# facebookresearch/EgoT2

Measured on AMD Instinct MI355X. Metric: clips/sec fwd+bwd, 3-task TTM translator (B=256,T=15,d=128), higher is better.
Workload: dtype f32 (operands split exactly into 3 bf16 parts; 6 bf16 MFMA products per K-block, f32 accumulate); 1 GPU; configs[1]: TTM 3-task translator, 1 layer d=128 h=4 d_ff=2048, B=256/GPU T=15 S=45, synthetic N(0,1) features, random-init weights, train mode dropout=0.5 (+0.1 on PE), weighted CE (evaluated in the forward's head epilogue), fwd+bwd; global_batch=256, parallelism=dp1, impl=auto, workgroups_per_clip=1, launch=one hipGraph replay per step, deterministic=False, compute_is_module_default=True, loss=weighted CE in the forward's head epilogue (egx_ce)

## Files before the change

egot2_amd/_lib.py:

```python
from __future__ import annotations

import ctypes as C
import os

_PKG = os.path.dirname(os.path.abspath(__file__))
LIB_PATH = os.environ.get("EGX_LIB") or os.path.join(_PKG, "libegot2x.so")

EGX_ABI_VERSION = 18
EGX_MAX_SEGMENTS = 8
EGX_F32, EGX_BF16, EGX_F32_SPLIT = 0, 1, 2
EGX_IMPL_AUTO, EGX_IMPL_GENERIC, EGX_IMPL_FUSED, EGX_IMPL_WIDE, EGX_IMPL_TILED = 0, 1, 2, 3, 4

_fp = C.c_void_p


class Segment(C.Structure):
    _fields_ = [("feat", _fp), ("T", C.c_int), ("d_in", C.c_int), ("proj_w", _fp), ("proj_b", _fp),
                ("add_vec", _fp), ("pos", _fp), ("pos_stride", C.c_int), ("feat_bf16", C.c_int), ("pool", C.c_int)]


class SegmentGrads(C.Structure):
    _fields_ = [("proj_w", _fp), ("proj_b", _fp), ("add_vec", _fp), ("pos", _fp), ("feat", _fp)]


# ... 67 lines not shown
    _fields_ = [(n, _fp) for n in _DEC_LAYER_FIELDS]


class DecLayerGrads(C.Structure):
    _fields_ = [(n, _fp) for n in _DEC_LAYER_FIELDS]


SIGNATURES = {
    "egx_abi_version": (C.c_int, []),
    "egx_last_error": (C.c_char_p, []),
    "egx_launch_count": (C.c_longlong, [C.c_int]),
    "egx_tuning_reload": (None, []),
    "egx_weight_cache_bytes": (C.c_size_t, [C.POINTER(Config), C.POINTER(Segment)]),
    "egx_encoder_workspace": (C.c_int, [C.POINTER(Config), C.POINTER(Segment), C.c_int,
                                        C.POINTER(C.c_size_t), C.POINTER(C.c_size_t)]),
    "egx_encoder_uses_fused": (C.c_int, [C.POINTER(Config), C.POINTER(Segment), C.c_int]),
    "egx_encoder_token_ce_ok": (C.c_int, [C.POINTER(Config), C.POINTER(Segment), C.c_int]),
    "egx_encoder_impl": (C.c_int, [C.POINTER(Config), C.POINTER(Segment), C.c_int]),
    "egx_encoder_slices": (C.c_int, [C.POINTER(Config), C.POINTER(Segment), C.c_int]),
    "egx_wide_gemm_scratch": (C.c_size_t, [C.c_int, C.c_int, C.c_int, C.c_int]),
    "egx_wide_gemm": (C.c_int, [C.c_int, _fp, _fp, _fp, _fp, C.c_int, C.c_int, C.c_int, _fp, C.c_int, _fp, _fp, _fp]),
    "egx_wide_attention_fwd": (C.c_int, [_fp, _fp, _fp, C.c_int, C.c_int, C.c_int, C.c_int, C.c_float, C.c_uint64, _fp]),
    "egx_wide_attention_bwd": (C.c_int, [_fp, _fp, _fp, _fp, _fp, _fp, C.c_int, C.c_int, C.c_int, C.c_int, C.c_float, C.c_uint64, _fp]),
    "egx_encoder_fwd": (C.c_int, [C.POINTER(Config), C.POINTER(Segment), _fp, _fp, C.POINTER(Layer), C.c_int,
                                  _fp, _fp, _fp, C.c_int, C.c_uint64, _fp]),
    "egx_encoder_bwd": (C.c_int, [C.POINTER(Config), C.POINTER(Segment), _fp, _fp, C.POINTER(Layer), C.c_int,
                                  _fp, _fp, _fp, C.POINTER(SegmentGrads), _fp, _fp, C.POINTER(LayerGrads),
                                  C.c_int, C.c_uint64, _fp]),
    "egx_translator_workspace": (C.c_int, [C.POINTER(Config), C.POINTER(Segment), C.c_int,
                                           C.POINTER(C.c_size_t), C.POINTER(C.c_size_t)]),
    "egx_translator_fwd": (C.c_int, [C.POINTER(Config), C.POINTER(Segment), _fp, _fp, C.POINTER(Layer), C.POINTER(Head),
                                     C.c_int, _fp, _fp, _fp, _fp, C.c_int, C.c_uint64, _fp]),
    "egx_ragged_workspace": (C.c_int, [C.POINTER(Config), C.POINTER(Segment), C.c_int, _fp, C.POINTER(C.c_size_t)]),
    "egx_ragged_fwd": (C.c_int, [C.POINTER(Config), C.POINTER(Segment), _fp, _fp, _fp, C.POINTER(Layer), C.POINTER(Head), C.c_int,
                                 _fp, _fp, _fp, _fp]),
    "egx_ragged_train_workspace": (C.c_int, [C.POINTER(Config), C.POINTER(Segment), C.c_int, _fp, C.POINTER(C.c_size_t),
                                             C.POINTER(C.c_size_t)]),
    "egx_ragged_train_fwd": (C.c_int, [C.POINTER(Config), C.POINTER(Segment), _fp, _fp, _fp, C.POINTER(Layer), C.POINTER(Head), C.c_int,
                                       _fp, _fp, _fp, _fp, C.c_int, C.c_uint64, _fp]),
    "egx_ragged_bwd": (C.c_int, [C.POINTER(Config), C.POINTER(Segment), _fp, _fp, _fp, C.POINTER(Layer), C.POINTER(Head), C.c_int,
                                 _fp, _fp, _fp, _fp, C.POINTER(SegmentGrads), _fp, _fp, C.POINTER(LayerGrads), C.POINTER(HeadGrads),
                                 C.c_int, C.c_uint64, _fp]),
    "egx_ragged_encode_workspace": (C.c_int, [C.POINTER(Config), C.POINTER(Segment), C.c_int, _fp, C.POINTER(C.c_size_t)]),
    "egx_ragged_encode": (C.c_int, [C.POINTER(Config), C.POINTER(Segment), _fp, _fp, _fp, C.POINTER(Layer), C.c_int, _fp, C.c_int, _fp, _fp]),
    "egx_ragged_encode_train_workspace": (C.c_int, [C.POINTER(Config), C.POINTER(Segment), C.c_int, _fp, C.POINTER(C.c_size_t),
                                                    C.POINTER(C.c_size_t)]),
    "egx_ragged_encode_train_fwd": (C.c_int, [C.POINTER(Config), C.POINTER(Segment), _fp, _fp, _fp, C.POINTER(Layer), C.c_int, _fp, C.c_int, _fp,
                                              C.c_int, C.c_uint64, _fp]),
    "egx_ragged_encode_bwd": (C.c_int, [C.POINTER(Config), C.POINTER(Segment), _fp, _fp, C.POINTER(Layer), C.c_int, _fp, C.c_int, _fp, _fp,
                                        C.POINTER(SegmentGrads), _fp, _fp, C.POINTER(LayerGrads), C.c_int, C.c_uint64, _fp]),
    "egx_translator_bwd": (C.c_int, [C.POINTER(Config), C.POINTER(Segment), _fp, _fp, C.POINTER(Layer), C.POINTER(Head),
                                     C.c_int, _fp, _fp, _fp, C.POINTER(SegmentGrads), _fp, _fp, C.POINTER(LayerGrads),
                                     C.POINTER(HeadGrads), C.c_int, C.c_uint64, _fp]),
    "egx_small_attention_fwd": (C.c_int, [_fp, C.c_int, _fp, C.c_int, _fp, C.c_int, _fp, C.c_int, C.c_int, C.c_int, C.c_int,
                                          C.c_int, C.c_int, C.c_int, C.c_float, C.c_uint64, C.c_uint32, _fp]),
    "egx_small_attention_bwd": (C.c_int, [_fp, C.c_int, _fp, C.c_int, _fp, C.c_int, _fp, C.c_int, _fp, _fp, _fp, C.c_int,
                                          C.c_int, C.c_int, C.c_int, C.c_int, C.c_int, C.c_float, C.c_uint64, C.c_uint32, _fp]),
    "egx_target_attention_fwd": (C.c_int, [_fp, C.c_int, _fp, C.c_int, _fp, C.c_int, _fp, C.c_int, C.c_int, C.c_int, C.c_int,
                                           C.c_int, C.c_int, C.c_int, C.c_float, C.c_uint64, C.c_uint32, _fp]),
    "egx_target_attention_bwd": (C.c_int, [_fp, C.c_int, _fp, C.c_int, _fp, C.c_int, _fp, C.c_int, _fp, _fp, _fp, C.c_int,
                                           C.c_int, C.c_int, C.c_int, C.c_int, C.c_int, C.c_float, C.c_uint64, C.c_uint32, _fp]),
    "egx_embed_pos_fwd": (C.c_int, [_fp, _fp, _fp, C.c_int, C.c_float, _fp, C.c_int, C.c_int, C.c_int, C.c_int, C.c_float,
                                    C.c_uint64, _fp]),
    "egx_embed_pos_bwd": (C.c_int, [_fp, _fp, _fp, C.c_float, C.c_int, C.c_int, C.c_int, C.c_int, C.c_float, C.c_uint64, _fp]),
    "egx_decoder_workspace": (C.c_int, [C.POINTER(DecConfig), C.c_int, C.POINTER(C.c_size_t), C.POINTER(C.c_size_t)]),
    "egx_decoder_fwd": (C.c_int, [C.POINTER(DecConfig), _fp, _fp, _fp, _fp, C.c_int, C.POINTER(DecLayer), _fp, _fp, C.c_int, _fp, _fp,
                                  _fp, C.c_int, C.c_uint64, _fp]),
    "egx_decoder_ragged_workspace": (C.c_int, [C.POINTER(DecConfig), C.c_int, _fp, C.POINTER(C.c_size_t)]),
    "egx_decoder_ragged_fwd": (C.c_int, [C.POINTER(DecConfig), _fp, _fp, _fp, _fp, _fp, C.c_int, C.POINTER(DecLayer), _fp, _fp, C.c_int, _fp,
                                         _fp, _fp]),
    "egx_decoder_ragged_train_workspace": (C.c_int, [C.POINTER(DecConfig), C.c_int, _fp, C.POINTER(C.c_size_t), C.POINTER(C.c_size_t)]),
    "egx_decoder_ragged_train_fwd": (C.c_int, [C.POINTER(DecConfig), _fp, _fp, _fp, _fp, _fp, C.c_int, C.POINTER(DecLayer), _fp, _fp, C.c_int,
                                               _fp, _fp, _fp, C.c_int, C.c_uint64, _fp]),
    "egx_decoder_ragged_bwd": (C.c_int, [C.POINTER(DecConfig), _fp, _fp, C.POINTER(DecLayer), _fp, C.c_int, _fp, _fp, _fp, _fp, _fp,
                                         C.POINTER(DecLayerGrads), _fp, _fp, _fp, C.c_size_t, C.c_int, C.c_uint64, _fp]),
    "egx_decoder_generate_workspace": (C.c_int, [C.POINTER(DecConfig), C.c_int, C.c_int, C.POINTER(C.c_size_t)]),
    "egx_decoder_generate": (C.c_int, [C.POINTER(DecConfig), _fp, _fp, _fp, _fp, C.c_int, C.POINTER(DecLayer), _fp, _fp, C.c_int, C.c_int, _fp,
                                       _fp, _fp, _fp]),
    "egx_decoder_beam_workspace": (C.c_int, [C.POINTER(DecConfig), C.c_int, C.c_int, C.c_int, C.POINTER(C.c_size_t)]),
    "egx_decoder_beam": (C.c_int, [C.POINTER(DecConfig), _fp, _fp, _fp, _fp, C.c_int, C.POINTER(DecLayer), _fp, _fp, C.c_int, C.c_int, C.c_int,
                                   _fp, _fp, _fp, _fp, _fp, _fp, _fp, _fp]),
    "egx_decoder_generate_sched": (C.c_int, [C.POINTER(DecConfig), _fp, _fp, _fp, _fp, C.c_int, C.POINTER(DecLayer), _fp, _fp, C.c_int, C.c_int,
                                             _fp, _fp, _fp, _fp, C.c_int, C.POINTER(C.c_int), _fp]),
    "egx_decoder_beam_sched": (C.c_int, [C.POINTER(DecConfig), _fp, _fp, _fp, _fp, C.c_int, C.POINTER(DecLayer), _fp, _fp, C.c_int, C.c_int,
                                         C.c_int, _fp, _fp, _fp, _fp, _fp, _fp, _fp, _fp, C.c_int, C.POINTER(C.c_int), _fp]),
    "egx_cross_attention_weights": (C.c_int, [_fp, C.c_int, _fp, C.c_int, C.c_int, _fp, C.c_int, C.c_int, C.c_int, C.c_int, C.c_int, _fp, C.c_int,
                                              _fp]),
    "egx_decoder_cross_weights": (C.c_int, [C.POINTER(DecConfig), C.c_int, _fp, _fp, _fp, _fp]),
    "egx_decoder_generate_attn": (C.c_int, [C.POINTER(DecConfig), _fp, _fp, _fp, _fp, C.c_int, C.POINTER(DecLayer), _fp, _fp, C.c_int, C.c_int,
                                            _fp, _fp, _fp, _fp, C.c_int, C.POINTER(C.c_int), _fp, _fp]),
    "egx_decoder_forced_workspace": (C.c_int, [C.POINTER(DecConfig), C.c_int, C.c_int, C.c_int, C.POINTER(C.c_size_t)]),
    "egx_decoder_forced": (C.c_int, [C.POINTER(DecConfig), _fp, _fp, _fp, _fp, _fp, C.c_int, C.POINTER(DecLayer), _fp, _fp, C.c_int, C.c_int,
                                     C.c_int, _fp, _fp, _fp, _fp]),
    "egx_decoder_bwd": (C.c_int, [C.POINTER(DecConfig), _fp, C.POINTER(DecLayer), _fp, C.c_int, _fp, _fp, _fp, _fp, _fp,
                                  C.POINTER(DecLayerGrads), _fp, _fp, _fp, C.c_size_t, C.c_int, C.c_uint64, _fp]),
    "egx_comm_unique_id": (C.c_int, [_fp]),
    "egx_comm_create": (C.c_int, [_fp, C.c_int, C.c_int, C.POINTER(C.c_void_p)]),
    "egx_comm_size": (C.c_int, [_fp]),
    "egx_allreduce": (C.c_int, [_fp, _fp, C.c_size_t, C.c_int, C.c_int, _fp]),
    "egx_comm_destroy": (C.c_int, [_fp]),
    "egx_comm_library": (C.c_char_p, []),
    "egx_relu_mask": (C.c_int, [_fp, _fp, C.c_size_t, _fp]),
    "egx_dropout": (C.c_int, [_fp, C.c_int, C.c_int, C.c_float, C.c_uint64, C.c_uint32, _fp]),
    "egx_pool_pack": (C.c_int, [_fp, C.c_int, C.c_int, C.c_int, C.c_int, C.c_int, C.c_int, C.c_int, C.c_int, C.c_int, C.c_int,
                                _fp, C.c_int, C.c_longlong, _fp]),
    "egx_weighted_ce": (C.c_int, [_fp, _fp, _fp, C.c_int, C.c_int, _fp, _fp, _fp]),
# ... 104 lines not shown
```

egot2_amd/csrc/common.h:

```cpp
#pragma once
#include <hip/hip_runtime.h>
#include <stdint.h>
#include <stdio.h>
#include <string>

namespace egx {

typedef float f32x4 __attribute__((ext_vector_type(4)));
typedef short bf16x8 __attribute__((ext_vector_type(8)));

void set_error(const char* fmt, ...);
void count_launch();

#define EGX_CHECK(cond, ...)                         \
    do {                                             \
        if (!(cond)) {                               \
            ::egx::set_error(__VA_ARGS__);           \
            return 1;                                \
        }                                            \
    } while (0)

#define EGX_HIP(expr)                                                                    \
    do {                                                                                 \
        hipError_t _e = (expr);                                                          \
        if (_e != hipSuccess) {                                                          \
            ::egx::set_error("%s failed: %s (%s:%d)", #expr, hipGetErrorString(_e),      \
                             __FILE__, __LINE__);                                        \
            return 1;                                                                    \
        }                                                                                \
    } while (0)

#define EGX_LAUNCH_CHECK()                                                               \
    do {                                                                                 \
        ::egx::count_launch();                                                           \
        hipError_t _e = hipGetLastError();                                               \
        if (_e != hipSuccess) {                                                          \
            ::egx::set_error("kernel launch failed: %s (%s:%d)", hipGetErrorString(_e),  \
                             __FILE__, __LINE__);                                        \
            return 1;                                                                    \
        }                                                                                \
    } while (0)

struct Tuning {
    int ffn_cut = -1;
    bool has_slices = false; int slices_cap = 0;
    bool has_drop = false; long slice_drop = 0;
    int dec_group = -1;
    int wide_tile = 0;
    int dec_side = 1;
};
const Tuning& tuning();

static inline int cdiv(int a, int b) { return (a + b - 1) / b; }
static inline size_t align_up(size_t x, size_t a) { return (x + a - 1) / a * a; }

__device__ __forceinline__ unsigned short f2bf(float x) {
    __bf16 h = (__bf16)x;
    return __builtin_bit_cast(unsigned short, h);
}

__device__ __forceinline__ uint32_t pack_bf16x2(float a, float b) {
    typedef float f32x2_ __attribute__((ext_vector_type(2)));
    typedef __bf16 bf16x2_ __attribute__((ext_vector_type(2)));
    f32x2_ v = {a, b};
    return __builtin_bit_cast(uint32_t, __builtin_convertvector(v, bf16x2_));
}

template <typename T>
__device__ __forceinline__ T wave_sum(T v) {
#pragma unroll
    for (int o = 32; o > 0; o >>= 1) v += __shfl_xor(v, o, 64);
    return v;
}
__device__ __forceinline__ float wave_max(float v) {
#pragma unroll
    for (int o = 32; o > 0; o >>= 1) v = fmaxf(v, __shfl_xor(v, o, 64));
    return v;
}
__device__ __forceinline__ int wave_max(int v) {
#pragma unroll
    for (int o = 32; o > 0; o >>= 1) v = max(v, __shfl_xor(v, o, 64));
    return v;
}
struct WaveBest { float v; int i; };
__device__ __forceinline__ bool argmax_better(float va, int ia, float vb, int ib) {
    const bool na = va != va, nb = vb != vb;
    if (na != nb) return na;
    if (na || va == vb) return ia < ib;
    return va > vb;
}
__device__ __forceinline__ WaveBest wave_argmax(float v, int i) {
#pragma unroll
    for (int o = 32; o > 0; o >>= 1) {
        const float vo = __shfl_xor(v, o, 64);
        const int io = __shfl_xor(i, o, 64);
        if (argmax_better(vo, io, v, i)) { v = vo; i = io; }
    }
    WaveBest b;
    b.v = v; b.i = i;
    return b;
}
// ... 63 lines not shown
```

egot2_amd/csrc/encoder.hip:

```cpp
#include <stdarg.h>
#include <string.h>
#include <stdlib.h>
#include <vector>

#include "../../include/egot2x.h"
#include "common.h"
#include "kernels.h"
#include "fused.h"
#include "fused_host.h"
#include "wide.h"
#include "wide_host.h"

namespace egx {

static thread_local char g_err[1024] = "";

static long long g_launches = 0;
void count_launch() { ++g_launches; }
void set_error(const char* fmt, ...) {
    va_list ap;
    va_start(ap, fmt);
    vsnprintf(g_err, sizeof(g_err), fmt, ap);
    va_end(ap);
}
// ... 33 lines not shown
    }
    size_t d = pl.d, N = pl.N;
    size_t cur = 0;
    for (int i = 0; i < pl.nseg; ++i) {
        size_t rows = (size_t)B * segs[i].T;
        pl.seg_pre[i] = take(cur, rows * d * 4);
        pl.seg_stats[i] = take(cur, rows * 2 * 4);
    }
    for (int l = 0; l < pl.L; ++l) {
        LayerOff& o = pl.layer[l];
        o.x_in = take(cur, N * d * 4);
        o.qkv = take(cur, N * 3 * d * 4);
        o.lse = take(cur, (size_t)B * pl.H * S * 4);
        o.attn_o = take(cur, N * d * 4);
        o.res1 = take(cur, N * d * 4);
        o.stats1 = take(cur, N * 2 * 4);
        o.x1 = take(cur, N * d * 4);
        o.hid = take(cur, N * (size_t)pl.dff * 4);
        o.res2 = take(cur, N * d * 4);
        o.stats2 = take(cur, N * 2 * 4);
    }
    pl.saved_bytes = cur;

    size_t sc = 0;
    pl.s_dA = take(sc, N * d * 4);
    pl.s_dB = take(sc, N * d * 4);
    pl.s_dqkv = take(sc, N * 3 * d * 4);
    pl.s_dhid = take(sc, N * (size_t)pl.dff * 4);
    size_t slab = 0;
    auto upd = [&](int M, int Nn, int K) { slab = size_max(slab, gemm_scratch_bytes(2, M, Nn, K)); };
    upd(3 * pl.d, pl.d, (int)N);
    upd(pl.d, pl.d, (int)N);
    upd(pl.dff, pl.d, (int)N);
    upd(pl.d, pl.dff, (int)N);
    for (int i = 0; i < pl.nseg; ++i)
        if (segs[i].proj_w) upd(pl.d, segs[i].d_in, B * segs[i].T);
    pl.slab_bytes = slab;
    pl.s_slab = take(sc, slab);
    pl.det_bytes = cfg->deterministic ? generic_det_scratch_bytes(B, pl.d, pl.dff) : 0;
    pl.s_det = take(sc, pl.det_bytes);
    pl.scratch_bytes = sc;
    return 0;
}

static Tuning g_tuning;
static bool g_tuning_loaded = false;
static void tuning_load() {
    Tuning t;
    if (const char* e = getenv("EGX_FFN_CUT")) t.ffn_cut = e[0] != '0' ? 1 : 0;
    if (const char* e = getenv("EGX_FFN_SLICES")) { t.has_slices = true; t.slices_cap = atoi(e); }
    if (const char* e = getenv("EGX_SLICE_DROP")) { t.has_drop = true; t.slice_drop = strtol(e, nullptr, 16); }
    if (const char* e = getenv("EGX_DEC_GROUP")) t.dec_group = atoi(e);
    if (const char* e = getenv("EGX_WIDE_TILE")) t.wide_tile = atoi(e);
    if (const char* e = getenv("EGX_DEC_SIDE")) t.dec_side = e[0] == '0' ? 0 : e[0] == '2' ? 2 : 1;
    g_tuning = t;
    g_tuning_loaded = true;
}
const Tuning& tuning() { if (!g_tuning_loaded) tuning_load(); return g_tuning; }

static bool use_tiled(const egx_config* cfg, const egx_segment* segs, const Plan& pl, bool* err) {
    *err = false;
    const bool ok = tiled_ok(cfg, segs, pl);
    if (cfg->impl == EGX_IMPL_TILED) {
        if (!ok) { set_error("tiled implementation does not support this configuration (needs d=128, h=4, 48 < S <= %d, compute bf16 or f32s, d_ff%%128==0, projected segments, <=4 layers)", TILED_MAX_S); *err = true; }
        return ok;
    }
    return cfg->impl == EGX_IMPL_AUTO && ok;
}

static bool use_fused(const egx_config* cfg, const egx_segment* segs, const Plan& pl, bool* err) {
    *err = false;
    bool ok = fused_ok(cfg, segs, pl);
    if (cfg->impl == EGX_IMPL_FUSED) {
        if (!ok) { set_error("fused implementation does not support this configuration (needs d=128, h=4 or 8, S<=48, d_ff%%128==0, projected segments, <=%d layers)", FUSED_MAX_LAYERS); *err = true; }
        return ok;
    }
    return cfg->impl == EGX_IMPL_AUTO && ok;
}

static bool use_wide(const egx_config* cfg, const egx_segment* segs, const Plan& pl, bool* err) {
    *err = false;
    const bool ok = wide_ok(cfg, segs, pl.B);
    if (cfg->impl == EGX_IMPL_WIDE) {
        if (!ok) { set_error("wide implementation does not support this configuration (needs compute = bf16, d_model >= 256, d_model / d_ff / projected d_in multiples of 128, S <= 128 with head dim 32 / 64 / 96 / 128, S <= 480 with head dim 32 / 64 or S <= 16 with head dim 256 / 512; d_model <= 2048)"); *err = true; }
        return ok;
    }
    return cfg->impl == EGX_IMPL_AUTO && ok && !fused_ok(cfg, segs, pl);
}

static int linear_nt(const float* x, const float* W, const float* bias, float* y, int M, int N, int K, int relu,
                     const Drop& dr, const float* residual, int compute, hipStream_t st) {
    GemmParams g;
    g.A = x; g.B = W; g.C = y;
    g.M = M; g.N = N; g.K = K;
    g.lda = K; g.ldb = K; g.ldc = N;
    g.bias = bias;
    g.relu = relu;
    g.drop_key = dr.key; g.drop_thresh = dr.thresh; g.drop_inv_keep = dr.inv_keep;
    g.residual = residual; g.ldr = N;
    return gemm(0, g, compute, 0, nullptr, 0, st);
}

int linear_dx(const float* dy, const float* W, float* dx, int M, int N, int K, const float* mask, float mask_scale,
              const float* residual, int compute, hipStream_t st, void* slab, size_t slab_bytes) {
    GemmParams g;
    g.A = dy; g.B = W; g.C = dx;
// ... 197 lines not shown
        const float* pre = sg.feat;
        if (sg.proj_w) {
            float* po = fptr(saved, pl.seg_pre[i]);
            Drop df = make_drop(training, cfg->p_feat, seed, (uint32_t)i, SITE_FEAT);
            if (linear_nt(sg.feat, sg.proj_w, sg.proj_b, po, rows, d, sg.d_in, 0, df, nullptr, comp, st)) return 1;
            pre = po;
        }
        LnFwdParams lp;
        lp.x = pre; lp.w = ln_w; lp.b = ln_b; lp.eps = cfg->ln_eps;
        lp.stats = fptr(saved, pl.seg_stats[i]);
        lp.y = x0; lp.rows = rows; lp.d = d;
        lp.T = sg.T; lp.S = S; lp.off = pl.seg_off[i];
        lp.add_vec = sg.add_vec; lp.pos = sg.pos; lp.pos_stride = sg.pos_stride;
        Drop dp = make_drop(training, cfg->p_pos, seed, 0, SITE_POS);
        lp.drop_key = dp.key; lp.drop_thresh = dp.thresh; lp.drop_inv_keep = dp.inv_keep;
        if (layernorm_fwd(lp, st)) return 1;
    }

    for (int l = 0; l < pl.L; ++l) {
        const LayerOff& o = pl.layer[l];
        const egx_layer& w = layers[l];
        const float* x_in = cfptr(saved, o.x_in);
        float* x_out = (l + 1 < pl.L) ? fptr(saved, pl.layer[l + 1].x_in) : tokens_out;
        Drop none;
        if (linear_nt(x_in, w.in_proj_w, w.in_proj_b, fptr(saved, o.qkv), N, 3 * d, d, 0, none, nullptr, comp, st)) return 1;
        Drop da = make_drop(training, cfg->p_drop, seed, (uint32_t)l, SITE_ATTN);
        if (attention_fwd(cfptr(saved, o.qkv), fptr(saved, o.attn_o), fptr(saved, o.lse), B, S, pl.H, d, da.key, da.thresh,
                          da.inv_keep, st)) return 1;
        Drop d1 = make_drop(training, cfg->p_drop, seed, (uint32_t)l, SITE_RES1);
        if (linear_nt(cfptr(saved, o.attn_o), w.out_proj_w, w.out_proj_b, fptr(saved, o.res1), N, d, d, 0, d1, x_in, comp, st)) return 1;
        LnFwdParams l1;
        l1.x = cfptr(saved, o.res1); l1.w = w.norm1_w; l1.b = w.norm1_b; l1.eps = cfg->ln_eps;
        l1.stats = fptr(saved, o.stats1); l1.y = fptr(saved, o.x1); l1.rows = N; l1.d = d;
        if (layernorm_fwd(l1, st)) return 1;
        Drop dh = make_drop(training, cfg->p_drop, seed, (uint32_t)l, SITE_FFN);
        if (linear_nt(cfptr(saved, o.x1), w.lin1_w, w.lin1_b, fptr(saved, o.hid), N, pl.dff, d, 1, dh, nullptr, comp, st)) return 1;
        Drop d2 = make_drop(training, cfg->p_drop, seed, (uint32_t)l, SITE_RES2);
        if (linear_nt(cfptr(saved, o.hid), w.lin2_w, w.lin2_b, fptr(saved, o.res2), N, d, pl.dff, 0, d2, cfptr(saved, o.x1), comp, st)) return 1;
        LnFwdParams l2;
        l2.x = cfptr(saved, o.res2); l2.w = w.norm2_w; l2.b = w.norm2_b; l2.eps = cfg->ln_eps;
        l2.stats = fptr(saved, o.stats2); l2.y = x_out; l2.rows = N; l2.d = d;
        if (layernorm_fwd(l2, st)) return 1;
    }
    if (with_head) {
        if (pool_head_fwd(tokens_out, B, S, d, head->ln_w, head->ln_b, cfg->ln_eps, head->W, head->b, head->n_out,
                          head_pooled, logits_out, st)) return 1;
        if (ce) return weighted_ce(logits_out, ce->target, ce->class_weight, B, head->n_out, ce->loss, ce->d_logits, st);
    }
    return 0;
}

static int encoder_fwd_impl(const egx_config* cfg, const egx_segment* segs, const float* ln_w, const float* ln_b,
                            const egx_layer* layers, const egx_head* head, int B, float* tokens_out, float* logits_out,
                            void* saved, void* scratch, int training, uint64_t seed, void* stream) {
    (void)scratch;
    Plan pl;
    if (make_plan(cfg, segs, B, pl)) return 1;
    EGX_CHECK(saved && ln_w && ln_b, "null pointer argument");
    EGX_CHECK(pl.L == 0 || layers, "null layers");
    hipStream_t st = (hipStream_t)stream;
    const bool with_head = head && head->W;
    EGX_CHECK(with_head ? (logits_out != nullptr) : (tokens_out != nullptr), "null output pointer");
    if (check_ce(cfg->ce, with_head, " (egx_translator_fwd)")) return 1;
    EGX_CHECK(!cfg->weight_cache_valid || cfg->weight_cache, "weight_cache_valid without a weight_cache");
    const egx_token_ce* tce = cfg->token_ce;
    if (tce) {
        EGX_CHECK(!with_head && token_ce_ok(cfg, segs, pl), "egx_config.token_ce: not on this configuration (egx_encoder_token_ce_ok)");
        EGX_CHECK(tce->W && tce->target && tce->logits && tce->loss && tce->d_logits && tce->C >= 1 && tce->C <= 8,
                  "egx_config.token_ce: W, target, logits, loss, d_logits and 1 <= C <= 8 must be set");
    }
    if (check_head(head)) return 1;
    if (training && !cfg->seed_ptr && (cfg->p_drop > 0.f || cfg->p_pos > 0.f || cfg->p_feat > 0.f)) {
        hipStreamCaptureStatus cs = hipStreamCaptureStatusNone;
        if (hipStreamIsCapturing(st, &cs) != hipSuccess) (void)hipGetLastError();
        EGX_CHECK(cs == hipStreamCaptureStatusNone, "training-mode dropout (p > 0) with a host seed cannot be captured in a hipGraph: every replay would "
                  "repeat the same masks; pass egx_config.seed_ptr (model.enable_device_seed()), capture with p = 0, or launch eagerly");
    }
    bool ferr, terr = false, werr;
    const bool fused = use_fused(cfg, segs, pl, &ferr);
    const bool tiled = !fused && !ferr && use_tiled(cfg, segs, pl, &terr);
    if (fused || tiled) return fused_path_fwd(cfg, segs, pl, tiled, ln_w, ln_b, layers, head, tokens_out, logits_out, saved, training, seed, st);
    if (ferr || terr) return 1;
    EGX_CHECK(cfg->out_tokens == 0 || cfg->out_tokens == pl.S, "out_tokens is implemented by the fused per-clip kernels only (egx_encoder_impl() == EGX_IMPL_FUSED)");
    if (use_wide(cfg, segs, pl, &werr)) return wide_path_fwd(cfg, segs, pl, ln_w, ln_b, layers, head, tokens_out, logits_out, saved, training, seed, st);
    if (werr) return 1;
    return generic_fwd(cfg, segs, pl, ln_w, ln_b, layers, head, tokens_out, logits_out, saved, training, seed, st);
}

static int wide_path_bwd(const egx_config* cfg, const egx_segment* segs, const Plan& pl, const float* ln_w, const egx_layer* layers, const egx_head* head,
                         const float* d_tokens, const float* d_logits, const void* saved, void* scratch, const egx_segment_grads* seg_grads, float* d_ln_w,
                         float* d_ln_b, const egx_layer_grads* layer_grads, const egx_head_grads* head_grads, int training, uint64_t seed, hipStream_t st) {
    const int B = pl.B;
    const bool with_head = head && head->W;
    EGX_CHECK(layers && layer_grads, "null layers / layer_grads");
    if (cfg->bwd_stage == 2) return 0;
    size_t wsv = 0, wsc = 0;
    wide_workspace(cfg, segs, B, &wsv, &wsc);
    const float* dtok = d_tokens;
    bool zeroed = false;
    if (with_head) {
        const float* extra = cfptr(saved, align_up(wsv, 256));
        const float* pooled = extra + (size_t)pl.N * pl.d;
        float* dt = fptr(scratch, align_up(wsc, 256));
        if (cfg->zero_buf && cfg->zero_bytes) { EGX_HIP(hipMemsetAsync(cfg->zero_buf, 0, cfg->zero_bytes, st)); zeroed = true; }
        if (pool_head_bwd(d_logits, pooled, B, pl.S, pl.d, head->ln_w, head->ln_b, cfg->ln_eps, head->W, head->n_out, dt,
                          head_grads ? head_grads->ln_w : nullptr, head_grads ? head_grads->ln_b : nullptr,
                          head_grads ? head_grads->W : nullptr, head_grads ? head_grads->b : nullptr, st)) return 1;
        dtok = dt;
    }
    egx_config c2 = *cfg;
    if (zeroed) { c2.zero_buf = nullptr; c2.zero_bytes = 0; }
    return wide_encoder_bwd(&c2, segs, ln_w, layers, B, dtok, saved, scratch, seg_grads, d_ln_w, d_ln_b, layer_grads, training, seed, st);
}

static int generic_bwd(const egx_config* cfg, const egx_segment* segs, const Plan& pl, const float* ln_w, const egx_layer* layers, const egx_head* head,
                       float* d_tokens, const float* d_logits, const void* saved, void* scratch, const egx_segment_grads* seg_grads, float* d_ln_w,
                       float* d_ln_b, const egx_layer_grads* layer_grads, const egx_head_grads* head_grads, int training, uint64_t seed, hipStream_t st) {
    const int B = pl.B;
    const bool with_head = head && head->W;
    EGX_CHECK(pl.L == 0 || (layers && layer_grads), "null layers / layer_grads");
    if (cfg->bwd_stage == 2) return 0;
    const int d = pl.d, S = pl.S, comp = cfg->compute, dff = pl.dff;
    const int N = (int)pl.N;
    if (cfg->zero_buf && cfg->zero_bytes) EGX_HIP(hipMemsetAsync(cfg->zero_buf, 0, cfg->zero_bytes, st));
    DetScope det_scope(cfg->deterministic ? (char*)scratch + pl.s_det : nullptr, pl.det_bytes);
    if (with_head) {
        const float* tk = cfptr(saved, align_up(pl.saved_bytes, 256));
        const float* pooled = tk + (size_t)N * d;
        d_tokens = fptr(scratch, align_up(pl.scratch_bytes, 256));
        if (pool_head_bwd(d_logits, pooled, B, S, d, head->ln_w, head->ln_b, cfg->ln_eps, head->W, head->n_out, d_tokens,
                          head_grads ? head_grads->ln_w : nullptr, head_grads ? head_grads->ln_b : nullptr,
                          head_grads ? head_grads->W : nullptr, head_grads ? head_grads->b : nullptr, st)) return 1;
    }
    float* dA = fptr(scratch, pl.s_dA);
// ... 34 lines not shown
        if (d1.thresh) {
            EGX_HIP(hipMemcpyAsync(dBm, dA, (size_t)N * d * 4, hipMemcpyDeviceToDevice, st));
            if (apply_dropout_mask(dBm, N, d, d1.key, d1.thresh, d1.inv_keep, st)) return 1;
            dbr = dBm;
        }
        if (gw.out_proj_b && colsum_accum(dbr, N, d, d, gw.out_proj_b, st)) return 1;
        if (gw.out_proj_w && linear_dw(dbr, cfptr(saved, o.attn_o), gw.out_proj_w, N, d, d, comp, slab, pl.slab_bytes, st)) return 1;
        if (linear_dx(dbr, w.out_proj_w, g, N, d, d, nullptr, 1.f, nullptr, comp, st)) return 1;
        Drop da = make_drop(training, cfg->p_drop, seed, (uint32_t)l, SITE_ATTN);
        if (attention_bwd(cfptr(saved, o.qkv), cfptr(saved, o.attn_o), cfptr(saved, o.lse), g, dqkv, B, S, pl.H, d, da.key,
                          da.thresh, da.inv_keep, st)) return 1;
        if (gw.in_proj_b && colsum_accum(dqkv, N, 3 * d, 3 * d, gw.in_proj_b, st)) return 1;
        if (gw.in_proj_w && linear_dw(dqkv, cfptr(saved, o.x_in), gw.in_proj_w, N, 3 * d, d, comp, slab, pl.slab_bytes, st)) return 1;
        if (linear_dx(dqkv, w.in_proj_w, g, N, 3 * d, d, nullptr, 1.f, dA, comp, st)) return 1;
    }

    Drop dp = make_drop(training, cfg->p_pos, seed, 0, SITE_POS);
    for (int i = 0; i < pl.nseg; ++i) {
        const egx_segment& sg = segs[i];
        egx_segment_grads sgr;
        memset(&sgr, 0, sizeof(sgr));
        if (seg_grads) sgr = seg_grads[i];
        int rows = B * sg.T;
        if (sgr.pos && pos_grad_accum(g, B, S, pl.seg_off[i], sg.T, d, sgr.pos, sg.pos_stride, dp.key, dp.thresh, dp.inv_keep, st)) return 1;
        bool need_dx = (sg.proj_w && (sgr.proj_w || sgr.proj_b || sgr.feat)) || (!sg.proj_w && sgr.feat);
        bool need_any = need_dx || d_ln_w || d_ln_b || sgr.add_vec;
        if (!need_any) continue;
        float* dseg = (!sg.proj_w && sgr.feat) ? sgr.feat : dA;
        LnBwdParams bp;
        bp.dy = g;
        bp.pre = sg.proj_w ? cfptr(saved, pl.seg_pre[i]) : sg.feat;
        bp.stats = cfptr(saved, pl.seg_stats[i]);
        bp.w = ln_w; bp.dx = dseg; bp.dw = d_ln_w; bp.db = d_ln_b; bp.dadd = sgr.add_vec;
        bp.rows = rows; bp.d = d; bp.T = sg.T; bp.S = S; bp.off = pl.seg_off[i];
        bp.drop_key = dp.key; bp.drop_thresh = dp.thresh; bp.drop_inv_keep = dp.inv_keep;
        if (sg.proj_w) {
            Drop df = make_drop(training, cfg->p_feat, seed, (uint32_t)i, SITE_FEAT);
            bp.out_drop_key = df.key; bp.out_drop_thresh = df.thresh; bp.out_drop_inv_keep = df.inv_keep;
        }
        if (layernorm_bwd(bp, st)) return 1;
        if (sg.proj_w) {
            if (sgr.proj_b && colsum_accum(dseg, rows, d, d, sgr.proj_b, st)) return 1;
            if (sgr.proj_w && linear_dw(dseg, sg.feat, sgr.proj_w, rows, d, sg.d_in, comp, slab, pl.slab_bytes, st)) return 1;
            if (sgr.feat && linear_dx(dseg, sg.proj_w, sgr.feat, rows, d, sg.d_in, nullptr, 1.f, nullptr, comp, st)) return 1;
        }
    }
    return 0;
}

static int encoder_bwd_impl(const egx_config* cfg, const egx_segment* segs, const float* ln_w, const float* ln_b,
                            const egx_layer* layers, const egx_head* head, int B, float* d_tokens, const float* d_logits,
                            const void* saved, void* scratch, const egx_segment_grads* seg_grads, float* d_ln_w,
                            float* d_ln_b, const egx_layer_grads* layer_grads, const egx_head_grads* head_grads,
                            int training, uint64_t seed, void* stream) {
    (void)ln_b;
    Plan pl;
    if (make_plan(cfg, segs, B, pl)) return 1;
    const bool with_head = head && head->W;
    EGX_CHECK((with_head ? (const void*)d_logits : cfg->token_ce ? (const void*)cfg->token_ce->d_logits : (const void*)d_tokens) && saved && scratch && ln_w, "null pointer argument");
    hipStream_t st = (hipStream_t)stream;
    bool ferr, terr = false, werr;
    const bool fused = use_fused(cfg, segs, pl, &ferr);
    const bool tiled = !fused && !ferr && use_tiled(cfg, segs, pl, &terr);
    if (fused || tiled) return fused_path_bwd(cfg, segs, pl, tiled, ln_w, ln_b, layers, head, d_tokens, d_logits, saved, scratch, seg_grads, d_ln_w, d_ln_b,
                                              layer_grads, head_grads, training, seed, st);
    if (ferr || terr) return 1;
    if (use_wide(cfg, segs, pl, &werr)) return wide_path_bwd(cfg, segs, pl, ln_w, layers, head, d_tokens, d_logits, saved, scratch, seg_grads, d_ln_w, d_ln_b,
                                                             layer_grads, head_grads, training, seed, st);
    if (werr) return 1;
    return generic_bwd(cfg, segs, pl, ln_w, layers, head, d_tokens, d_logits, saved, scratch, seg_grads, d_ln_w, d_ln_b, layer_grads, head_grads, training, seed, st);
}

extern "C" {

int egx_encoder_fwd(const egx_config* cfg, const egx_segment* segs, const float* ln_w, const float* ln_b,
                    const egx_layer* layers, int B, float* tokens_out, void* saved, void* scratch, int training,
                    uint64_t seed, void* stream) {
    return encoder_fwd_impl(cfg, segs, ln_w, ln_b, layers, nullptr, B, tokens_out, nullptr, saved, scratch, training, seed, stream);
}

int egx_encoder_bwd(const egx_config* cfg, const egx_segment* segs, const float* ln_w, const float* ln_b,
                    const egx_layer* layers, int B, float* d_tokens, const void* saved, void* scratch,
                    const egx_segment_grads* seg_grads, float* d_ln_w, float* d_ln_b,
                    const egx_layer_grads* layer_grads, int training, uint64_t seed, void* stream) {
    return encoder_bwd_impl(cfg, segs, ln_w, ln_b, layers, nullptr, B, d_tokens, nullptr, saved, scratch, seg_grads, d_ln_w,
                            d_ln_b, layer_grads, nullptr, training, seed, stream);
}

int egx_translator_workspace(const egx_config* cfg, const egx_segment* segs, int B, size_t* saved_bytes, size_t* scratch_bytes) {
    Plan pl;
    if (make_plan(cfg, segs, B, pl)) return 1;
    size_t sv = 0, sc = 0;
    if (egx_encoder_workspace(cfg, segs, B, &sv, &sc)) return 1;
    size_t wsv = 0, wsc = 0;
    if (wide_ok(cfg, segs, B)) wide_workspace(cfg, segs, B, &wsv, &wsc);
    size_t extra_sv = align_up(size_max(pl.saved_bytes, wsv), 256) + (pl.N + (size_t)B) * pl.d * 4 + 256;
    size_t extra_sc = align_up(size_max(pl.scratch_bytes, wsc), 256) + pl.N * pl.d * 4 + 256;
    if (saved_bytes) *saved_bytes = size_max(sv, extra_sv);
    if (scratch_bytes) *scratch_bytes = size_max(sc, extra_sc);
    return 0;
}

int egx_translator_fwd(const egx_config* cfg, const egx_segment* segs, const float* ln_w, const float* ln_b,
                       const egx_layer* layers, const egx_head* head, int B, float* logits_out, float* tokens_out,
                       void* saved, void* scratch, int training, uint64_t seed, void* stream) {
    EGX_CHECK(head && head->W, "egx_translator_fwd needs a head (use egx_encoder_fwd otherwise)");
    return encoder_fwd_impl(cfg, segs, ln_w, ln_b, layers, head, B, tokens_out, logits_out, saved, scratch, training, seed, stream);
}

int egx_translator_bwd(const egx_config* cfg, const egx_segment* segs, const float* ln_w, const float* ln_b,
                       const egx_layer* layers, const egx_head* head, int B, const float* d_logits, const void* saved,
                       void* scratch, const egx_segment_grads* seg_grads, float* d_ln_w, float* d_ln_b,
                       const egx_layer_grads* layer_grads, const egx_head_grads* head_grads, int training,
                       uint64_t seed, void* stream) {
    EGX_CHECK(head && head->W, "egx_translator_bwd needs a head (use egx_encoder_bwd otherwise)");
    return encoder_bwd_impl(cfg, segs, ln_w, ln_b, layers, head, B, nullptr, d_logits, saved, scratch, seg_grads, d_ln_w,
                            d_ln_b, layer_grads, head_grads, training, seed, stream);
}

int egx_pool_head_fwd(const float* tokens, int B, int S, int d, const float* ln_w, const float* ln_b, float ln_eps,
                      const float* W, const float* b, int n_out, float* pooled_saved, float* out, void* stream) {
    EGX_CHECK(tokens && pooled_saved && out, "null pointer argument");
    return pool_head_fwd(tokens, B, S, d, ln_w, ln_b, ln_eps, W, b, n_out, pooled_saved, out, (hipStream_t)stream);
}

int egx_pool_head_bwd(const float* d_out, const float* pooled_saved, int B, int S, int d, const float* ln_w,
                      const float* ln_b, float ln_eps, const float* W, int n_out, float* d_tokens, float* d_ln_w,
                      float* d_ln_b, float* d_W, float* d_b, void* stream) {
    EGX_CHECK(d_out && pooled_saved && d_tokens, "null pointer argument");
    return pool_head_bwd(d_out, pooled_saved, B, S, d, ln_w, ln_b, ln_eps, W, n_out, d_tokens, d_ln_w, d_ln_b, d_W, d_b,
                         (hipStream_t)stream);
}

int egx_linear_fwd(const float* x, const float* W, const float* b, float* y, int M, int N, int K, int relu, int compute,
                   void* stream) {
    EGX_CHECK(x && W && y, "null pointer argument");
    Drop none;
    return linear_nt(x, W, b, y, M, N, K, relu, none, nullptr, compute, (hipStream_t)stream);
}
int egx_linear_residual_fwd(const float* x, const float* W, const float* b, const float* residual, float* y, int M, int N, int K,
                            int compute, void* stream) {
    EGX_CHECK(x && W && y && residual, "null pointer argument");
    Drop none;
    return linear_nt(x, W, b, y, M, N, K, 0, none, residual, compute, (hipStream_t)stream);
}
int egx_gelu_fwd(const float* z, float* h, size_t n, void* stream) { return gelu_fwd(z, h, n, (hipStream_t)stream); }
int egx_gelu_bwd(const float* z, const float* dh, float* dz, size_t n, void* stream) { return gelu_bwd(z, dh, dz, n, (hipStream_t)stream); }

size_t egx_colsum_ordered_scratch(int M, int N) { return colsum_part_bytes(M, N); }
int egx_colsum_ordered(const float* dy, int M, int N, float* db, void* scratch, size_t scratch_bytes, void* stream) {
    EGX_CHECK(dy && db, "egx_colsum_ordered: null pointer argument");
    EGX_CHECK(scratch_bytes >= colsum_part_bytes(M, N) && (scratch || !colsum_part_bytes(M, N)),
              "egx_colsum_ordered: scratch of %zu bytes, egx_colsum_ordered_scratch(%d, %d) = %zu", scratch_bytes, M, N, colsum_part_bytes(M, N));
    return colsum_accum_ordered(dy, M, N, N, db, scratch, scratch_bytes, (hipStream_t)stream);
}

size_t egx_linear_bwd_scratch(int M, int N, int K) { return size_max(gemm_scratch_bytes(2, N, K, M), gemm_scratch_bytes(1, M, K, N)); }

int egx_linear_bwd(const float* dy, const float* x, const float* W, float* dx, float* dW, float* db, int M, int N, int K,
                   int compute, void* scratch, void* stream) {
    hipStream_t st = (hipStream_t)stream;
    EGX_CHECK(dy, "null dy");
    if (db && colsum_accum(dy, M, N, N, db, st)) return 1;
    if (dW) {
        EGX_CHECK(x && scratch, "linear_bwd: dW needs x and scratch");
        if (linear_dw(dy, x, dW, M, N, K, compute, scratch, gemm_scratch_bytes(2, N, K, M), st)) return 1;
    }
    if (dx) {
        EGX_CHECK(W, "linear_bwd: dx needs W");
        if (linear_dx(dy, W, dx, M, N, K, nullptr, 1.f, nullptr, compute, st, scratch, scratch ? egx_linear_bwd_scratch(M, N, K) : 0)) return 1;
    }
    return 0;
// ... 191 lines not shown
```

egot2_amd/csrc/ffn_cut.hip:

```cpp
#include <stdlib.h>
#include "common.h"
#include "kernels.h"
#include "fused.h"
#include "fused_dev.h"

namespace egx {

__device__ unsigned long long g_cstamps[32];
#ifdef EGX_STAMPS
#define CSTAMP_INIT() unsigned long long ct_prev = __builtin_amdgcn_s_memtime(), ct_acc[8] = {0, 0, 0, 0, 0, 0, 0, 0}
#define CSTAMP(k) do { __builtin_amdgcn_sched_barrier(0); unsigned long long t_ = __builtin_amdgcn_s_memtime(); ct_acc[k] += t_ - ct_prev; ct_prev = t_; __builtin_amdgcn_sched_barrier(0); } while (0)
#define CSTAMP_FLUSH(base) do { if (blockIdx.x == 0 && (threadIdx.x == 0 || threadIdx.x == 256)) for (int k_ = 0; k_ < 8; ++k_) g_cstamps[(base) + (threadIdx.x >> 8) * 8 + k_] = ct_acc[k_]; } while (0)
#define ASTAMP(i) do { if (blockIdx.x == 0 && threadIdx.x == 0) g_cstamps[i] = __builtin_amdgcn_s_memtime(); } while (0)
#else
#define ASTAMP(i) do { } while (0)
#define CSTAMP_INIT() do { } while (0)
#define CSTAMP(k) do { } while (0)
#define CSTAMP_FLUSH(base) do { } while (0)
#endif
int debug_read_cstamps(unsigned long long* out) {
    return hipMemcpyFromSymbol(out, HIP_SYMBOL(g_cstamps), sizeof(unsigned long long) * 32) == hipSuccess ? 0 : 1;
}
#ifdef EGX_DIAG_NOLOAD
#define RING_REFILL(slot, k, hb, hbn) do { } while (0)
#else
#define RING_REFILL(slot, k, hb, hbn) ring[slot] = frag_load(((k) + D) & 15, (k) + D < 16 ? (hb) : (hbn))
#endif

namespace {
constexpr int CT = 512;
constexpr int CNT = 3;
constexpr int CSP = CNT * 16;
constexpr int CBLK = CSP * LDX;
constexpr int CPS = CSP * LDXH;

template <int CM> struct RingDepth { static constexpr int v = 4; };
template <> struct RingDepth<CM_BF16> { static constexpr int v = 16; };

template <int CM>
__device__ __forceinline__ Frag<CM> operand_frag(const unsigned short* planes, const float* xf, int row, int k0, int q) {
    if constexpr (CM == CM_SPLIT) {
        return load_split_frag(planes, CPS, row, k0, q);
    } else if constexpr (CM == CM_BF16) {
        const unsigned short* b = planes + row * LDXH + k0 + 4 * q;
        const uint2 lo = *reinterpret_cast<const uint2*>(b), hi = *reinterpret_cast<const uint2*>(b + 16);
        Frag<CM_BF16> f;
        f.v = __builtin_bit_cast(bf16x8, (u32x4){lo.x, lo.y, hi.x, hi.y});
        return f;
    } else {
        return load_frag<CM>(xf + row * LDX + k0, q);
    }
}

// ... 38 lines not shown
        *reinterpret_cast<uint2*>(plane + row * LDXH + c) = make_uint2(pack_bf16x2(v[0], v[1]), pack_bf16x2(v[2], v[3]));
    }
}
__device__ __forceinline__ void block_to_split_planes(unsigned short* planes, const float* blk) {
    const int row = threadIdx.x >> 2, c0 = (threadIdx.x & 3) * 32;
    if (row < CSP) {
        float g[32];
        uint32_t h[16], m[16], lo[16];
        load32(blk + row * LDX + c0, g);
        split32(g, h, m, lo);
        store_parts32(planes + row * LDXH + c0, (size_t)CPS, h, m, lo);
    }
}

template <int CM, bool FWD>
__device__ __forceinline__ void cut_walk(int wave, int nit, int& j_begin, int& n_mine, int shift_code = 0) {
    const int shift = shift_code ? shift_code - 1 : (CM == CM_BF16 ? 0 : (FWD ? nit / 4 : nit / 8));
    const int n_old = nit + shift;
    j_begin = wave < 4 ? 0 : n_old;
    n_mine = wave < 4 ? n_old : 2 * nit - n_old;
}
constexpr int CP_FLOATS = 1024 + 8 * FD;
constexpr int CP_HEAD_ROWS = 8;
__device__ __forceinline__ int cut_rot(int rot_mode, int clip, int nit) {
    return rot_mode == 0 ? (int)((clip * 11u + (clip >> 3) * 5u) % (unsigned)nit)
         : rot_mode == 4 ? (int)(((unsigned)(clip >> 3) & 3u) % (unsigned)nit)
         : rot_mode == 5 ? (int)(((unsigned)(clip >> 3) & 7u) % (unsigned)nit) : 0;
}

__device__ __forceinline__ void reduce_partials8(f32x4 (&y)[8][CNT], float* blk0, int wave, int r, int q) {
    if (wave >= 4) {
        float* mine = blk0 + (wave - 4) * CBLK;
#pragma unroll
        for (int i = 0; i < 8; ++i)
#pragma unroll
            for (int t = 0; t < CNT; ++t)
                *reinterpret_cast<f32x4*>(mine + (t * 16 + r) * LDX + i * 16 + 4 * q) = y[i][t];
    }
    __syncthreads();
    if (wave < 4) {
        float* mine = blk0 + wave * CBLK;
#pragma unroll
        for (int i = 0; i < 8; ++i)
#pragma unroll
            for (int t = 0; t < CNT; ++t) {
                f32x4* a = reinterpret_cast<f32x4*>(mine + (t * 16 + r) * LDX + i * 16 + 4 * q);
                *a = y[i][t] + *a;
            }
    }
    __syncthreads();
}
}

template <int CM>
__global__ __launch_bounds__(CT) void ffn_fwd_kernel(FusedFwdParams p, int l) {
    extern __shared__ __attribute__((aligned(16))) float lds[];
    float* X1 = lds;
    float* R = lds + CBLK;
    unsigned short* XP = reinterpret_cast<unsigned short*>(R);
    constexpr int NPL = CM == CM_SPLIT ? 3 : 1;
    constexpr int D = RingDepth<CM>::v;
    const int tid = threadIdx.x, wave = tid >> 6, lane = tid & 63, r = lane & 15, q = lane >> 4;
    const int clip = blockIdx.x, S = p.S;
    const size_t tokbase = (size_t)clip * S;
    const FusedLayer& w = p.layer[l];
    const bool dev_seed = p.seed_ptr != nullptr;
    const uint64_t seed_dev = dev_seed ? *p.seed_ptr : 0ull;
    const uint64_t k_ffn = dev_seed ? site_key(seed_dev, l, SITE_FFN) : w.ffn_key;
    const uint64_t k_res2 = dev_seed ? site_key(seed_dev, l, SITE_RES2) : w.res2_key;

    ASTAMP(16);
    Touched tch = {{0, 0, 0, 0}};
    if (p.touch.n) tch = touch_lines<CT>(p.touch, blockIdx.x, gridDim.x, tid);
    const int nhb = p.d_ff / 32;
    int j_begin_, n_mine_;
    cut_walk<CM, true>(wave, nhb / 8, j_begin_, n_mine_, p.rot_mode >> 8);
    const int nit = __builtin_amdgcn_readfirstlane(n_mine_), j_begin = __builtin_amdgcn_readfirstlane(j_begin_);
    const int pair_s = __builtin_amdgcn_readfirstlane(wave & 3);
    const int rot = cut_rot(p.rot_mode & 255, clip, nit);
    auto hb_of = [&](int it) { int j = it + rot; if (j >= nit) j -= nit; return pair_s + 4 * (j_begin + j); };
    float* CP = lds + 5 * CBLK;
    const bool cp_hd = p.head.n_out > 0 && l + 1 == p.n_layers;
    const int cp_g = tid >> 5, cp_c4 = (tid & 31) << 2;
    f32x4 cp_v, cp_w;
    float cp_b;
    {
        const float* src = cp_g == 0 ? w.norm2_w : cp_g == 1 ? w.norm2_b : (cp_g == 3 && cp_hd) ? p.head.ln_w : (cp_g == 4 && cp_hd) ? p.head.ln_b : w.lin2_b;
        cp_v = *reinterpret_cast<const f32x4*>(src + cp_c4);
        const int nb = cp_hd ? p.head.n_out : 0, nw = cp_hd && p.head.n_out <= CP_HEAD_ROWS ? p.head.n_out * 32 : 0;
        cp_b = nb ? p.head.b[min(max(tid - 160, 0), nb - 1)] : 0.f;
        cp_w = *reinterpret_cast<const f32x4*>(nw ? p.head.W + (size_t)min(max(tid - 256, 0), nw - 1) * 4 : w.lin2_b);
    }
    auto cp_store = [&] {
        if (cp_g < 3 || (cp_g < 5 && cp_hd)) *reinterpret_cast<f32x4*>(CP + cp_g * FD + cp_c4) = cp_v;
        if (cp_hd) {
            if (tid >= 160 && tid < 160 + p.head.n_out) CP[5 * FD + (tid - 160)] = cp_b;
            if (p.head.n_out <= CP_HEAD_ROWS && tid >= 256 && tid < 256 + p.head.n_out * 32) *reinterpret_cast<f32x4*>(CP + 1024 + (tid - 256) * 4) = cp_w;
        }
    };
    auto frag_load = [&](int k, int hb) -> WRaw<CM> {
        return k < 8 ? load_w<CM>(w.lin1_wp, hb * 2 + (k & 1), FD / 32, k >> 1, lane) : load_w<CM>(w.lin2_wp, k - 8, nhb, hb, lane);
    };
    WRaw<CM> ring[D];
    float4 b1r[2];
    {
        const int hb0 = hb_of(0);
#pragma unroll
        for (int k = 0; k < D; ++k) ring[k] = frag_load(k, hb0);
// ... 130 lines not shown
                    for (int e = 0; e < 4; ++e) hacc[i][t][e] += bv[i][e];
        }
        uint32_t dead = 0;
#pragma unroll
        for (int k = 2 * CNT * 4 - 1; k >= 0; --k) {
            const int i = k / (CNT * 4), t = (k / 4) % CNT, e = k & 3;
            dead = __builtin_amdgcn_alignbit(dead, __float_as_uint(hacc[i][t][e]), 31);
        }
        p.relu_bits[bits_base + (size_t)hb * 64] = ~dead & ((1u << (2 * CNT * 4)) - 1u);
#pragma unroll
        for (int i = 0; i < 2; ++i)
#pragma unroll
            for (int t = 0; t < CNT; ++t)
#pragma unroll
                for (int e = 0; e < 4; ++e) hacc[i][t][e] = __int_as_float(max(__float_as_int(hacc[i][t][e]), 0));
        Frag<CM> hbq[CNT];
#pragma unroll
        for (int t = 0; t < CNT; ++t) hbq[t] = chain_frag<CM>(hacc[0][t], hacc[1][t]);
#ifndef EGX_DIAG_NOSTORE
        {
            char* hb_base = hid_base + (size_t)hb * 2 * (HTILE_ELEMS * ESZ);
#pragma unroll
            for (int t = 0; t < CNT; ++t) {
                if constexpr (CM == CM_BF16) {
                    const u32x4 u = __builtin_bit_cast(u32x4, hbq[t].v);
                    store_hid_tile_bf16(hb_base + (size_t)t * nht * (HTILE_ELEMS * ESZ), u, lane, S - t * 16);
                } else {
#pragma unroll
                    for (int i = 0; i < 2; ++i)
                        store_hid_tile<CM>(hb_base + ((size_t)t * nht + i) * (HTILE_ELEMS * ESZ), hacc[i][t], lane, S - t * 16);
                }
            }
        }
#endif
        __builtin_amdgcn_sched_barrier(0);
        CSTAMP(3);
#pragma unroll
        for (int k = 8; k < 16; ++k) {
            pin(ring[k % D]);
            if (k == 8) { CSTAMP(4); }
            Frag<CM> a = w_frag<CM>(ring[k % D]);
#pragma unroll
            for (int t = 0; t < CNT; ++t) mma<CM>(y[k - 8][t], a, hbq[t]);
            __builtin_amdgcn_sched_barrier(0);
            RING_REFILL(k % D, k, hb, hbn);
            __builtin_amdgcn_sched_barrier(0);
        }
    }
    CSTAMP(5);
    CSTAMP_FLUSH(0);
    ASTAMP(18);
    __syncthreads();
    ASTAMP(19);
    reduce_partials8(y, R, wave, r, q);
    ASTAMP(20);

    for (int i = tid; i < S * (FD / 4); i += CT) {
        const int row = i >> 5, c = (i & 31) << 2, o = row * LDX + c;
        const f32x4 a0 = *reinterpret_cast<const f32x4*>(R + o), a1 = *reinterpret_cast<const f32x4*>(R + CBLK + o);
        const f32x4 a2 = *reinterpret_cast<const f32x4*>(R + 2 * CBLK + o), a3 = *reinterpret_cast<const f32x4*>(R + 3 * CBLK + o);
        f32x4 f = ((a0 + a1) + (a2 + a3)) + *reinterpret_cast<const f32x4*>(CP + 2 * FD + c);
        if (w.res_thresh) {
            float m4[4];
            drop_scale4(k_res2, (uint32_t)(tokbase + row), (uint32_t)c, w.res_thresh, w.drop_inv, m4);
            f = f * f32x4{m4[0], m4[1], m4[2], m4[3]};
        }
        *reinterpret_cast<f32x4*>(X1 + o) = f + *reinterpret_cast<const f32x4*>(X1 + o);
    }
    __syncthreads();
    ASTAMP(21);
    const bool last = l + 1 == p.n_layers;
    float* Y = R;
    ln_rows(X1, S, CP, CP + FD, p.eps, [&](int row, int c0, float (&x)[32], float (&yv)[32]) {
        if (last && p.tokens_out && row < p.out_T) store32(p.tokens_out + ((size_t)clip * p.out_T + row) * FD + c0, yv);
        store32(Y + row * LDX + c0, yv);
    }, [&] { rows_from_lds(p.saved_res + ((size_t)(2 * l + 1) * p.B + clip) * S * FD, X1, S); });
    __syncthreads();
    ASTAMP(22);
    if (!last) {
        rows_from_lds(p.xin_out + ((size_t)(l + 1) * p.B + clip) * S * FD, Y, S);
        return;
    }
    if (p.head.n_out > 0) {
        float* pooled = X1;
        const FusedCe ce{p.ce_target, p.ce_weight, p.ce_loss, p.ce_dlogits, p.ce_B, nullptr};
        CeReq rq;
        if (ce.target) { ce_request_labels<CT>(ce, tid, rq); ce_request_weights(ce, p.head.n_out, rq); }
        if (tid < FD) pooled[tid] = colsum_lds(Y, 0, S, tid) * (1.f / (float)S);
        if (ce.target) ce_weight_partials<CT>(ce, p.head.n_out, tid, rq, pooled + 256);
        __syncthreads();
        if (wave == 0) {
            float2 x = *reinterpret_cast<float2*>(pooled + 2 * lane);
            float mean = wave_sum(x.x + x.y) * (1.f / FD);
            float dx = x.x - mean, dy = x.y - mean;
            float rstd = rsqrtf(wave_sum(dx * dx + dy * dy) * (1.f / FD) + p.eps);
            float2 lw = *reinterpret_cast<const float2*>(CP + 3 * FD + 2 * lane);
            float2 lb = *reinterpret_cast<const float2*>(CP + 4 * FD + 2 * lane);
            float y0 = dx * rstd * lw.x + lb.x, y1 = dy * rstd * lw.y + lb.y;
            const bool w_lds = p.head.n_out <= CP_HEAD_ROWS;
            float zmine = 0.f;
            for (int o = 0; o < p.head.n_out; ++o) {
                float2 wv = w_lds ? *reinterpret_cast<const float2*>(CP + 1024 + o * FD + 2 * lane) : *reinterpret_cast<const float2*>(p.head.W + (size_t)o * FD + 2 * lane);
                float sdot = wave_sum(y0 * wv.x + y1 * wv.y) + CP[5 * FD + o];
                if (lane == 0) p.logits_out[(size_t)clip * p.head.n_out + o] = sdot;
                zmine = lane == o ? sdot : zmine;
            }
            if (ce.target) ce_clip<CT>(ce, p.head.n_out, clip, lane, zmine, pooled + 256, true);
        }
    }
    ASTAMP(23);
}

template <int CM>
__global__ __launch_bounds__(CT) void ffn_bwd_kernel(FusedBwdParams p, int l) {
    extern __shared__ __attribute__((aligned(16))) float lds[];
    float* B1 = lds;
    float* Gs = lds + 1 * CBLK;
    float* B2 = lds + 2 * CBLK;
    float* B3 = lds + 3 * CBLK;
    float* B4 = lds + 4 * CBLK;
    unsigned short* GP = reinterpret_cast<unsigned short*>(B3);
    constexpr int D = RingDepth<CM>::v;
    const int tid = threadIdx.x, wave = tid >> 6, lane = tid & 63, r = lane & 15, q = lane >> 4;
    const int clip = blockIdx.x, S = p.S;
    const size_t tok0 = (size_t)clip * S;
    const FusedBwdLayer& w = p.layer[l];
    const bool dev_seed = p.seed_ptr != nullptr;
    const uint64_t seed_dev = dev_seed ? *p.seed_ptr : 0ull;
    const uint64_t k_res2 = dev_seed ? site_key(seed_dev, l, SITE_RES2) : w.res2_key;
    const bool last = l + 1 == p.n_layers;

    ASTAMP(24);
    Touched tch = {{0, 0, 0, 0}};
    if (p.touch.n) tch = touch_lines<CT>(p.touch, blockIdx.x, gridDim.x, tid);
    if (p.zero_buf) {
        const size_t n4 = p.zero_n / 4, per = (n4 + gridDim.x - 1) / gridDim.x;
        const size_t b0 = (size_t)blockIdx.x * per, b1 = b0 + per < n4 ? b0 + per : n4;
        for (size_t k = b0 + threadIdx.x; k < b1; k += CT) reinterpret_cast<float4*>(p.zero_buf)[k] = make_float4(0, 0, 0, 0);
    }
    float* part = p.partials + (size_t)clip * p.P;
    float* pl = part + l * FUSED_P_LAYER;

    const int nhb = p.d_ff / 32;
    int j_begin_, n_mine_;
    cut_walk<CM, false>(wave, nhb / 8, j_begin_, n_mine_, p.rot_mode >> 8);
    const int nit = __builtin_amdgcn_readfirstlane(n_mine_), j_begin = __builtin_amdgcn_readfirstlane(j_begin_);
    const int pair_s = __builtin_amdgcn_readfirstlane(wave & 3);
    const int rot = cut_rot(p.rot_mode & 255, clip, nit);
    auto hb_of = [&](int it) { int j = it + rot; if (j >= nit) j -= nit; return pair_s + 4 * (j_begin + j); };
    float* CP = lds + 5 * CBLK;
    const bool cp_hd = p.head.n_out > 0 && last;
    const int cp_g = tid >> 5, cp_c4 = (tid & 31) << 2;
    f32x4 cp_v, cp_w;
    float cp_b;
    {
        const float* src = cp_g == 1 ? w.norm2_b : (cp_g == 3 && cp_hd) ? p.head.ln_w : (cp_g == 4 && cp_hd) ? p.head.ln_b : w.norm2_w;
        cp_v = *reinterpret_cast<const f32x4*>(src + cp_c4);
        const int nb = cp_hd ? p.head.n_out : 0, nw = cp_hd && p.head.n_out <= CP_HEAD_ROWS ? p.head.n_out * 32 : 0;
        cp_b = nb ? p.d_logits[(size_t)clip * p.head.n_out + min(max(tid - 160, 0), nb - 1)] : 0.f;
        if (nb && p.d_logits_scale) cp_b *= *p.d_logits_scale;
        cp_w = *reinterpret_cast<const f32x4*>(nw ? p.head.W + (size_t)min(max(tid - 256, 0), nw - 1) * 4 : w.norm2_w);
    }
    auto cp_store = [&] {
        if (cp_g < 2 || ((cp_g == 3 || cp_g == 4) && cp_hd)) *reinterpret_cast<f32x4*>(CP + cp_g * FD + cp_c4) = cp_v;
        if (cp_hd) {
            if (tid >= 160 && tid < 160 + p.head.n_out) CP[5 * FD + 64 + (tid - 160)] = cp_b;
            if (p.head.n_out <= CP_HEAD_ROWS && tid >= 256 && tid < 256 + p.head.n_out * 32) *reinterpret_cast<f32x4*>(CP + 1024 + (tid - 256) * 4) = cp_w;
        }
    };
    auto frag_load = [&](int k, int hb) -> WRaw<CM> {
        return k < 8 ? load_w<CM>(w.lin2_wtp, hb * 2 + (k & 1), FD / 32, k >> 1, lane) : load_w<CM>(w.lin1_wtp, k - 8, nhb, hb, lane);
    };
    const uint32_t* relu_bits = p.relu_bits + ((size_t)l * p.B + clip) * (size_t)nhb * 64 + lane;
    WRaw<CM> ring[D];
    uint32_t relu_word;
    {
        const int hb0 = hb_of(0);
#pragma unroll
        for (int k = 0; k < D; ++k) ring[k] = frag_load(k, hb0);
        relu_word = relu_bits[(size_t)hb0 * 64];
    }
    const float* res2 = p.saved_res + ((size_t)(2 * l + 1) * p.B + clip) * S * FD;
    const bool head_bwd = last && p.head.n_out > 0;
    {
        constexpr int XR = CSP * (FD / 4) / CT;
        f32x4 rr[XR], dr[XR];
        const f32x4* rs = reinterpret_cast<const f32x4*>(res2);
        const int ndy_rows = head_bwd ? 0 : (last ? p.out_T : S);
        const f32x4* ds = head_bwd ? rs : reinterpret_cast<const f32x4*>(last ? p.d_tokens + (size_t)clip * p.out_T * FD : p.dxin + tok0 * FD);
        const int nx = S * (FD / 4), nd = ndy_rows * (FD / 4);
#pragma unroll
        for (int k = 0; k < XR; ++k) {
            const int i = tid + CT * k;
            rr[k] = rs[i < nx ? i : nx - 1];
            dr[k] = ds[i < nd ? i : (nd > 0 ? nd - 1 : 0)];
        }
        for (int i = tid; i < 5 * CBLK / 4; i += CT) reinterpret_cast<f32x4*>(lds)[i] = f32x4{0, 0, 0, 0};
        cp_store();
        __syncthreads();
#pragma unroll
        for (int k = 0; k < XR; ++k) {
            const int i = tid + CT * k, row = i >> 5, c = (i & 31) << 2;
            if (i < nx) {
                *reinterpret_cast<f32x4*>(B1 + row * LDX + c) = rr[k];
                if (head_bwd) *reinterpret_cast<f32x4*>(Gs + row * LDX + c) = rr[k];
            }
            if (i < nd) *reinterpret_cast<f32x4*>(Gs + row * LDX + c) = dr[k];
        }
        touch_sink(tch);
    }
    ASTAMP(25);
    if (head_bwd) {
        float* hp = part + p.head_off;
        __syncthreads();
        ln_rows(Gs, S, CP, CP + FD, p.eps, [&](int row, int c0, float (&x)[32], float (&y)[32]) { store32(Gs + row * LDX + c0, y); });
        __syncthreads();
        float* pooled = B2;
        if (tid < FD) pooled[tid] = colsum_lds(Gs, 0, S, tid) * (1.f / (float)S);
        __syncthreads();
        if (wave == 0) {
            float2 x = *reinterpret_cast<float2*>(pooled + 2 * lane);
            float mean = wave_sum(x.x + x.y) * (1.f / FD);
            float xh0 = x.x - mean, xh1 = x.y - mean;
            float rstd = rsqrtf(wave_sum(xh0 * xh0 + xh1 * xh1) * (1.f / FD) + p.eps);
            xh0 *= rstd; xh1 *= rstd;
            float2 lw = *reinterpret_cast<const float2*>(CP + 3 * FD + 2 * lane);
            float2 lb = *reinterpret_cast<const float2*>(CP + 4 * FD + 2 * lane);
            float y0 = xh0 * lw.x + lb.x, y1 = xh1 * lw.y + lb.y;
            float d0 = 0.f, d1 = 0.f;
            const bool w_lds = p.head.n_out <= CP_HEAD_ROWS;
            for (int o = 0; o < p.head.n_out; ++o) {
                float go = CP[5 * FD + 64 + o];
                float2 wv = w_lds ? *reinterpret_cast<const float2*>(CP + 1024 + o * FD + 2 * lane) : *reinterpret_cast<const float2*>(p.head.W + (size_t)o * FD + 2 * lane);
                d0 += go * wv.x; d1 += go * wv.y;
                *reinterpret_cast<float2*>(hp + 256 + FUSED_HEAD_MAX_OUT + o * FD + 2 * lane) = make_float2(go * y0, go * y1);
                if (lane == 0) hp[256 + o] = go;
            }
            *reinterpret_cast<float2*>(hp + 2 * lane) = make_float2(d0 * xh0, d1 * xh1);
            *reinterpret_cast<float2*>(hp + 128 + 2 * lane) = make_float2(d0, d1);
            float g0 = d0 * lw.x, g1 = d1 * lw.y;
            float s1 = wave_sum(g0 + g1) * (1.f / FD);
            float s2 = wave_sum(g0 * xh0 + g1 * xh1) * (1.f / FD);
            float inv_s = 1.f / (float)S;
            *reinterpret_cast<float2*>(pooled + 128 + 2 * lane) =
                make_float2(rstd * (g0 - s1 - xh0 * s2) * inv_s, rstd * (g1 - s1 - xh1 * s2) * inv_s);
        }
        __syncthreads();
        f32x4 dp[1];
        {
            const int c = (tid & 31) << 2;
            dp[0] = *reinterpret_cast<const f32x4*>(pooled + 128 + c);
        }
        __syncthreads();
        for (int i = tid; i < S * (FD / 4); i += CT) {
            const int row = i >> 5, c = (i & 31) << 2;
            *reinterpret_cast<f32x4*>(Gs + row * LDX + c) = dp[0];
        }
        if (tid < 64) *reinterpret_cast<f32x4*>(B2 + 4 * tid) = f32x4{0, 0, 0, 0};
    }
    __syncthreads();
    ASTAMP(26);
    ln_bwd_rows(S, CP, p.eps,
        [&](int row, int c0, float (&dy)[32], float (&x)[32]) { load32(Gs + row * LDX + c0, dy); load32(B1 + row * LDX + c0, x); },
        [&](int row, int c0, float (&dy)[32], float (&dx)[32], float (&dyx)[32]) {
            store32(B1 + row * LDX + c0, dx);
            store32(B3 + row * LDX + c0, dyx);
            if (w.res_thresh) {
                const uint32_t orow = (uint32_t)(tok0 + row);
#pragma unroll
                for (int j = 0; j < 32; ++j) dx[j] *= drop_scale(k_res2, orow, (uint32_t)(c0 + j), w.res_thresh, w.drop_inv);
            }
            store32(B2 + row * LDX + c0, dx);
        });
    __syncthreads();
    if (tid < 128) pl[0 + tid] = colsum_lds(B3, 0, S, tid);
    else if (tid < 256) pl[128 + (tid - 128)] = colsum_lds(Gs, 0, S, tid - 128);
    else if (tid < 384) pl[256 + (tid - 256)] = colsum_lds(B2, 0, S, tid - 256);
    if (!(CM != CM_F32 && p.xg_planes)) rows_from_lds(w.g2_out + tok0 * FD, B2, S);
    __syncthreads();
    if constexpr (CM == CM_SPLIT) block_to_split_planes(GP, B2);
    else if constexpr (CM == CM_BF16) block_to_plane(GP, B2);
    __syncthreads();
    if (CM != CM_F32 && p.xg_planes) {
        if constexpr (CM == CM_SPLIT) {
            const size_t plane = (size_t)p.B * CSP * FD;
            planes_from_lds<3>(reinterpret_cast<unsigned short*>(w.g2_out) + (size_t)clip * CSP * FD, plane, GP);
        } else {
            planes_from_lds<1>(reinterpret_cast<unsigned short*>(w.g2_out) + (size_t)clip * CSP * FD, 0, GP);
        }
    }

    ASTAMP(27);
    f32x4 dxa[8][CNT];
#pragma unroll
    for (int i = 0; i < 8; ++i)
#pragma unroll
        for (int t = 0; t < CNT; ++t) dxa[i][t] = f32x4{0, 0, 0, 0};
    constexpr int ESZ = CM == CM_BF16 ? 2 : 4;
    const int nht = p.d_ff / 16;
    char* const dhid_base = (char*)p.dhid_out + ((size_t)l * p.B + clip) * CNT * nht * (size_t)(HTILE_ELEMS * ESZ);
    for (int it = 0; it < nit; ++it) {
        const int hb = hb_of(it);
        const int hbn = hb_of(it + 1 < nit ? it + 1 : it);
        __builtin_amdgcn_sched_barrier(0);
        f32x4 dacc[2][CNT];
#pragma unroll
        for (int i = 0; i < 2; ++i)
#pragma unroll
            for (int t = 0; t < CNT; ++t) dacc[i][t] = f32x4{0, 0, 0, 0};
        Frag<CM> gb[CNT];
#pragma unroll
        for (int k = 0; k < 8; ++k) {
// ... 19 lines not shown
#pragma unroll
            for (int t = 0; t < CNT; ++t)
#pragma unroll
                for (int e = 0; e < 4; ++e) {
                    const int k = (i * CNT + t) * 4 + e;
                    const int32_t m = ((int32_t)(bits << (31 - k))) >> 31;
                    dacc[i][t][e] = __uint_as_float(__float_as_uint(dacc[i][t][e]) & (uint32_t)m);
                }
        Frag<CM> dq_[CNT];
#pragma unroll
        for (int t = 0; t < CNT; ++t) dq_[t] = chain_frag<CM>(dacc[0][t], dacc[1][t]);
        {
            char* hb_base = dhid_base + (size_t)hb * 2 * (HTILE_ELEMS * ESZ);
#pragma unroll
            for (int t = 0; t < CNT; ++t) {
                if constexpr (CM == CM_BF16) {
                    const u32x4 u = __builtin_bit_cast(u32x4, dq_[t].v);
                    store_hid_tile_bf16(hb_base + (size_t)t * nht * (HTILE_ELEMS * ESZ), u, lane, S - t * 16);
                } else {
#pragma unroll
                    for (int i = 0; i < 2; ++i)
                        store_hid_tile<CM>(hb_base + ((size_t)t * nht + i) * (HTILE_ELEMS * ESZ), dacc[i][t], lane, S - t * 16);
                }
            }
        }
        __builtin_amdgcn_sched_barrier(0);
#pragma unroll
        for (int k = 8; k < 16; ++k) {
            pin(ring[k % D]);
            Frag<CM> a = w_frag<CM>(ring[k % D]);
#pragma unroll
            for (int t = 0; t < CNT; ++t) mma<CM>(dxa[k - 8][t], a, dq_[t]);
            __builtin_amdgcn_sched_barrier(0);
            RING_REFILL(k % D, k, hb, hbn);
            __builtin_amdgcn_sched_barrier(0);
        }
    }
    ASTAMP(28);
    __syncthreads();
    ASTAMP(29);
    reduce_partials8(dxa, Gs, wave, r, q);
    ASTAMP(30);
    {
        f32x4* dst = reinterpret_cast<f32x4*>(p.dy1 + tok0 * FD);
        for (int i = tid; i < S * (FD / 4); i += CT) {
            const int o = (i >> 5) * LDX + ((i & 31) << 2);
            const f32x4 a0 = *reinterpret_cast<const f32x4*>(Gs + o), a1 = *reinterpret_cast<const f32x4*>(B2 + o);
            const f32x4 a2 = *reinterpret_cast<const f32x4*>(B3 + o), a3 = *reinterpret_cast<const f32x4*>(B4 + o);
            dst[i] = (((a0 + a1) + a2) + a3) + *reinterpret_cast<const f32x4*>(B1 + o);
        }
    }
    ASTAMP(31);
}

bool ffn_cut_supported(int d_ff) { return d_ff % 256 == 0 && d_ff >= 256; }
size_t ffn_cut_lds_bytes() { return (size_t)(5 * CBLK + CP_FLOATS) * sizeof(float); }

template <int CM>
static int launch_cut_fwd(const FusedFwdParams& p, int l, hipStream_t st) {
    const size_t lds = ffn_cut_lds_bytes();
    static bool attr_set = false;
    if (!attr_set) {
        EGX_HIP(hipFuncSetAttribute(reinterpret_cast<const void*>(&ffn_fwd_kernel<CM>), hipFuncAttributeMaxDynamicSharedMemorySize, (int)lds));
        attr_set = true;
    }
    timing_begin(TIMER_FFN_FWD, st);
    hipLaunchKernelGGL((ffn_fwd_kernel<CM>), dim3(p.B), dim3(CT), lds, st, p, l);
    timing_end(TIMER_FFN_FWD, st);
    EGX_LAUNCH_CHECK();
    return 0;
}
template <int CM>
static int launch_cut_bwd(const FusedBwdParams& p, int l, hipStream_t st) {
    const size_t lds = ffn_cut_lds_bytes();
    static bool attr_set = false;
    if (!attr_set) {
        EGX_HIP(hipFuncSetAttribute(reinterpret_cast<const void*>(&ffn_bwd_kernel<CM>), hipFuncAttributeMaxDynamicSharedMemorySize, (int)lds));
        attr_set = true;
    }
    timing_begin(TIMER_FFN_BWD, st);
    hipLaunchKernelGGL((ffn_bwd_kernel<CM>), dim3(p.B), dim3(CT), lds, st, p, l);
    timing_end(TIMER_FFN_BWD, st);
    EGX_LAUNCH_CHECK();
    return 0;
}

int ffn_cut_forward(const FusedFwdParams& p, int l, int compute, hipStream_t st) {
    EGX_CHECK(ffn_cut_supported(p.d_ff) && p.S <= CSP && l >= 0 && l < p.n_layers, "ffn_cut_forward: d_ff=%d S=%d layer %d", p.d_ff, p.S, l);
    EGX_CHECK(p.x1f_out && p.xin_out && p.saved_res && p.relu_bits && p.hid_out, "ffn_cut_forward: missing buffers");
    return compute == CM_BF16 ? launch_cut_fwd<CM_BF16>(p, l, st) : compute == CM_SPLIT ? launch_cut_fwd<CM_SPLIT>(p, l, st) : launch_cut_fwd<CM_F32>(p, l, st);
}
int ffn_cut_backward(const FusedBwdParams& p, int l, int compute, hipStream_t st) {
    EGX_CHECK(ffn_cut_supported(p.d_ff) && p.S <= CSP && l >= 0 && l < p.n_layers, "ffn_cut_backward: d_ff=%d S=%d layer %d", p.d_ff, p.S, l);
    EGX_CHECK(p.dy1 && p.saved_res && p.relu_bits && p.dhid_out && p.partials && (l + 1 == p.n_layers || p.dxin), "ffn_cut_backward: missing buffers");
    return compute == CM_BF16 ? launch_cut_bwd<CM_BF16>(p, l, st) : compute == CM_SPLIT ? launch_cut_bwd<CM_SPLIT>(p, l, st) : launch_cut_bwd<CM_F32>(p, l, st);
}

}
```

egot2_amd/csrc/fused.h:

```cpp
#pragma once
#include "common.h"

namespace egx {

constexpr int FUSED_MAX_SEG = 4;
constexpr int FUSED_MAX_LAYERS = 6;

constexpr int TOUCH_MAX = 4;
struct TouchList { const void* base[TOUCH_MAX]; unsigned lines[TOUCH_MAX]; int n; };
static inline void touch_add(TouchList& t, const void* base, size_t bytes) {
    if (base && bytes >= 128 && t.n < TOUCH_MAX) { t.base[t.n] = base; t.lines[t.n] = (unsigned)(bytes >> 7); ++t.n; }
}

struct FusedSeg {
    const float* feat;
    const void* proj_wp;
    const float* proj_b;
    const float* add_vec;
    const float* pos;
    int T, d_in, off, pos_stride;
    int row0, Tfull;
    int seg_id, pad_;
};

// ... 114 lines not shown
    const float* norm1_w; const float* norm1_b; const float* norm2_w; const float* norm2_b;
    uint64_t attn_key, res1_key, ffn_key, res2_key;
    uint32_t attn_thresh, res_thresh, ffn_thresh;
    float drop_inv;
    float* x1_out; float* g2_out; float* attn_o_out; float* g1_out; float* x_in_out; float* dqkv_out;
};

constexpr int FUSED_P_LAYER = 1152;
static inline int fused_partial_len(int L, int nseg) { return L * FUSED_P_LAYER + 256 + nseg * 256; }

struct FusedBwdParams {
    FusedSeg seg[FUSED_MAX_SEG];
    float* dseg_out[FUSED_MAX_SEG];
    FusedBwdLayer layer[FUSED_MAX_LAYERS];
    const float* ln_w; const float* ln_b;
    float eps;
    int nseg, n_layers, B, S, d_ff;
    int rot_mode;
    const float* d_tokens;
    int out_T;
    FusedHead head; const float* d_logits; int head_off;
    const float* pooled;
    const float* saved_pre;
    const float* saved_res;
    const float* saved_qkv;
    const uint32_t* relu_bits;
    int xg_planes;
    void* dhid_out;
    float* zero_buf; size_t zero_n;
    float* partials; int P;
    uint64_t pos_key; uint32_t pos_thresh; float pos_inv;
    const uint64_t* seed_ptr;
    uint64_t feat_key[FUSED_MAX_SEG]; uint32_t feat_thresh; float feat_inv;
    int n_heads;
    float* dx0_out;
    int tpc, S_clip; size_t Ntok;
    int tiled, l_front, l_back;
    float* datt;
    float* dres;
    int n_slices; float* xchg; unsigned* xflags; int slice_drop;
    int cut, cut_layer;
    float* dy1;
    float* dxin;
    const float* d_logits_scale;
    const float* tce_W; const float* tce_dlogits; int tce_C;
    TouchList touch;
    const int* rtab; int B_clips; const int* rseg;
};
int fused_backward(const FusedBwdParams& p, int compute, hipStream_t st);
bool ffn_cut_supported(int d_ff);
size_t ffn_cut_lds_bytes();
int ffn_cut_forward(const FusedFwdParams& p, int l, int compute, hipStream_t st);
int ffn_cut_backward(const FusedBwdParams& p, int l, int compute, hipStream_t st);

struct SmallDwProblem {
    const float* G; const float* X; float* out;
    int R, C, K, ldg, ldx, first_block, splits;
};
constexpr int SMALL_DW_MAX = 8;
struct SmallDwParams {
    SmallDwProblem pr[SMALL_DW_MAX];
    int n, per;
    float* slabs;
};
int small_dw(SmallDwParams& p, int compute, hipStream_t st, void* slabs = nullptr, size_t slab_bytes = 0, bool reduce_here = true);
int seed_advance(uint64_t* seed, hipStream_t st);

struct PartialDst { float* dst; int off, len; };
constexpr int PARTIAL_MAX_DST = 64;
struct ReducePartialsParams {
    PartialDst d[PARTIAL_MAX_DST];
    int n, B, P;
    const float* partials;
};
int reduce_partials(const ReducePartialsParams& rp, hipStream_t st, bool deterministic = false);
struct SmallDwTail { SlabReduce red; ReducePartialsParams rp; unsigned slab_blocks; int rp_units, chunks; uint64_t* seed_advance;  TouchList touch;  };
int tail_reduce(const SmallDwParams* sp, const SlabReduce* red, const ReducePartialsParams* rp, uint64_t* seed_advance_ptr, const TouchList* touch, hipStream_t st);

enum { TIMER_FUSED_FWD = 0, TIMER_FUSED_BWD = 1, TIMER_FFN_DW = 2, TIMER_FFN_FWD = 3, TIMER_FFN_BWD = 4, TIMER_WIDE_GEMM = 5,
       TIMER_WIDE_ATTN_FWD = 6, TIMER_WIDE_ATTN_BWD = 7, TIMER_COUNT = 8 };
void timing_enable(int on);
void timing_begin(int which, hipStream_t st);
void timing_end(int which, hipStream_t st);
int timing_read(int which, double* total_ms, int* count);

struct TiledAttnParams {
    const float* qkv;
    float* attn_o;
    float* lse;
    const float* d_o;
    float* delta;
    float* dqkv;
    int B, S, tpc;
    uint64_t drop_key; uint32_t drop_thresh; float drop_inv;
    const uint64_t* seed_ptr; int layer;
    const int* rtab;
};
constexpr int TILED_MAX_S = 512;
constexpr int RAGGED_REC = 16;
enum { RG_TILE0 = 0, RG_S = 1, RG_TOK0 = 2, RG_OUT0 = 3, RG_OUTN = 4, RG_T = 5 , RG_OFF = 9  };
static_assert(RG_OFF + FUSED_MAX_SEG <= RAGGED_REC, "ragged clip record");
int upload_words(int* dst, const int* src, size_t n, hipStream_t st);
int ragged_rows(float* padded, float* packed, const int* rtab, const int* rseg, int B, int T_pad, int C, int k, int to_packed, hipStream_t st);
int tiled_attn_fwd(const TiledAttnParams& p, int compute, hipStream_t st);
int tiled_attn_bwd(const TiledAttnParams& p, int compute, hipStream_t st);

bool fused_supported(int d_model, int n_heads, int d_ff, int S, int nseg, const int* d_in, const int* T, const bool* has_proj);
size_t fused_lds_bytes(int NT);
long long slices_stolen_fwd(int reset);
long long slices_stolen_bwd(int reset);
int debug_read_stamps(unsigned long long* out, int n);
int debug_read_bstamps(unsigned long long* out, int n);
int fused_forward(const FusedFwdParams& p, int compute, hipStream_t st);

}
```

egot2_amd/csrc/fused.hip:

```cpp
#include "common.h"
#include "kernels.h"
#include "fused.h"
#include "fused_dev.h"
#include <stdlib.h>
#include <string.h>
#include <type_traits>
#include <vector>

namespace egx {

__global__ __launch_bounds__(64) void pack_weights_kernel(PackParams pp) {
    int blk = blockIdx.x;
    if (pp.seed_advance && blk == 0 && threadIdx.x == 0)
        *pp.seed_advance = *pp.seed_advance * 6364136223846793005ull + 1442695040888963407ull;
    if (pp.zero_words)
        for (int i = blk * 64 + threadIdx.x; i < pp.n_zero; i += gridDim.x * 64) pp.zero_words[i] = 0u;
    if (pp.zero_word2 && blk == 0 && threadIdx.x == 0) *pp.zero_word2 = 0.f;
    if (pp.zero_ctl && blk == 0 && threadIdx.x < 8) pp.zero_ctl[threadIdx.x] = 0u;
    if (pp.n == 0) return;
    int di = 0;
    while (di + 1 < pp.n && blk >= pp.d[di + 1].first_block) ++di;
    const PackDesc& d = pp.d[di];
    int local = blk - d.first_block;
    int nkb = d.K / 32;
// ... 1021 lines not shown
            float* tacc = reinterpret_cast<float*>(p.tce_ticket + 1);
            atomicAdd(tacc, l);
            __threadfence();
            const unsigned mine = 1u + ((unsigned)cn << 12);
            const unsigned old = atomicAdd(p.tce_ticket, mine);
            if ((old & 4095u) == (unsigned)p.B - 1u) {
                __threadfence();
                *p.tce_loss = atomicExch(tacc, 0.f);
                if (p.tce_correct) *p.tce_correct = (float)((old + mine) >> 12);
                atomicExch(p.tce_ticket, 0u);
            }
        }
        STAMP(14);
    }

    if (!TILED && p.head.n_out > 0) {
        float* pooled = X1;
        const FusedCe ce{p.ce_target, p.ce_weight, p.ce_loss, p.ce_dlogits, p.ce_B, p.ce_ticket};
        CeReq rq;
        if (ce.target) { ce_request_labels<256>(ce, tid, rq); ce_request_weights(ce, p.head.n_out, rq); }
        if (tid < FD) pooled[tid] = colsum_lds(Xs, 0, S, tid) * (1.f / (float)S);
        if (ce.target) ce_weight_partials<256>(ce, p.head.n_out, tid, rq, pooled + 256);
        __syncthreads();
        if (wave == 0) {
            float2 x = *reinterpret_cast<float2*>(pooled + 2 * lane);
            float mean = wave_sum(x.x + x.y) * (1.f / FD);
            float dx = x.x - mean, dy = x.y - mean;
            float rstd = rsqrtf(wave_sum(dx * dx + dy * dy) * (1.f / FD) + p.eps);
            float2 lw = *reinterpret_cast<const float2*>(p.head.ln_w + 2 * lane);
            float2 lb = *reinterpret_cast<const float2*>(p.head.ln_b + 2 * lane);
            float y0 = dx * rstd * lw.x + lb.x, y1 = dy * rstd * lw.y + lb.y;
            float zmine = 0.f;
            for (int o = 0; o < p.head.n_out; ++o) {
                float2 wv = *reinterpret_cast<const float2*>(p.head.W + (size_t)o * FD + 2 * lane);
                float sdot = wave_sum(y0 * wv.x + y1 * wv.y) + p.head.b[o];
                if (lane == 0) p.logits_out[(size_t)clip * p.head.n_out + o] = sdot;
                zmine = lane == o ? sdot : zmine;
            }
            if (ce.target) ce_clip<256>(ce, p.head.n_out, clip, lane, zmine, pooled + 256, slice == 0);
        }
    }
}

namespace {
struct TimerSlot { std::vector<hipEvent_t> a, b; int n = 0; };
TimerSlot g_timers[TIMER_COUNT];
int g_timing_on = 0;
constexpr int TIMER_MAX_EVENTS = 4096;
}
void timing_enable(int on) {
    g_timing_on = on;
    for (int i = 0; i < TIMER_COUNT; ++i) g_timers[i].n = 0;
}
void timing_begin(int which, hipStream_t st) {
    if (!g_timing_on) return;
    TimerSlot& t = g_timers[which];
    if (t.n >= TIMER_MAX_EVENTS) return;
    if ((int)t.a.size() <= t.n) {
        hipEvent_t ea, eb;
        (void)hipEventCreate(&ea); (void)hipEventCreate(&eb);
        t.a.push_back(ea); t.b.push_back(eb);
    }
    (void)hipEventRecord(t.a[t.n], st);
}
void timing_end(int which, hipStream_t st) {
    if (!g_timing_on) return;
    TimerSlot& t = g_timers[which];
    if (t.n < (int)t.a.size() && t.n < TIMER_MAX_EVENTS) { (void)hipEventRecord(t.b[t.n], st); ++t.n; }
}
int timing_read(int which, double* total_ms, int* count) {
    if (which < 0 || which >= TIMER_COUNT) return 1;
    TimerSlot& t = g_timers[which];
    double tot = 0;
    for (int i = 0; i < t.n; ++i) {
        float ms = 0.f;
        if (hipEventSynchronize(t.b[i]) != hipSuccess || hipEventElapsedTime(&ms, t.a[i], t.b[i]) != hipSuccess) return 1;
        tot += ms;
    }
    if (total_ms) *total_ms = tot;
    if (count) *count = t.n;
    return 0;
}

size_t fused_lds_bytes(int NT) {
    int SP = NT * 16;
    return (size_t)(4 * SP * LDX + FD * LDV) * sizeof(float) + FUSED_MAX_SEG * sizeof(FusedSeg) + 16 + 21 * FD * sizeof(float);
}

bool fused_supported(int d_model, int n_heads, int d_ff, int S, int nseg, const int* d_in, const int* T, const bool* has_proj) {
    if (d_model != FD || (n_heads != FH && n_heads != 2 * FH)) return false;
    if (d_ff % 128 != 0 || d_ff < 128) return false;
    if (S < 1 || S > 48) return false;
    for (int i = 0; i < nseg; ++i) {
        if (!has_proj[i]) return false;
        if (d_in[i] % 128 != 0) return false;
        if (T[i] < 1) return false;
    }
    return true;
}

template <int CM, bool TILED, int DH>
static int launch_fwd(const FusedFwdParams& p, hipStream_t st) {
    EGX_CHECK(p.S <= 48, "fused: S=%d unsupported", p.S);
    const size_t lds = fused_lds_bytes(3);
    static bool attr_set = false;
    if (!attr_set) {
// ... 80 lines not shown
```

egot2_amd/csrc/fused_bwd.hip:

```cpp
#include <stdlib.h>
#include <string.h>
#include <type_traits>
#include "common.h"
#include "kernels.h"
#include "fused.h"
#ifdef EGX_STAMPS
namespace egx { extern __device__ unsigned long long g_bstamps[32]; }
#define LNB_STAMP(base, k) do { if ((base) >= 0 && blockIdx.x == 0 && threadIdx.x == 0) { __builtin_amdgcn_sched_barrier(0); egx::g_bstamps[(base) + (k)] = __builtin_amdgcn_s_memtime(); __builtin_amdgcn_sched_barrier(0); } } while (0)
#endif
#include "fused_dev.h"

namespace egx {

template <int CM, int HT>
__global__ __launch_bounds__(256, HT == 1 ? 2 : 1) void ffn_dw_kernel(FfnDwParams p) {
    extern __shared__ __attribute__((aligned(16))) float lds[];
    constexpr int TILE = 32 * LDX;
    const int tid = threadIdx.x, lane = tid & 63, wave = tid >> 6;
    const int r = lane & 15, q = lane >> 4;
    const int hg = blockIdx.x, split = blockIdx.y;
    const int htile0 = (hg * 4 + wave) * HT;
    const int nkb_total = (p.N + 31) / 32;
    const int kb_beg = split * p.kb_per_split;
    const int kb_end = min(nkb_total, kb_beg + p.kb_per_split);
// ... 1110 lines not shown
}
__device__ unsigned long long g_bstamps[32];
#ifdef EGX_STAMPS
#define BSTAMP(i) do { if (blockIdx.x == 0 && threadIdx.x == 0) g_bstamps[i] = __builtin_amdgcn_s_memtime(); } while (0)
#else
#define BSTAMP(i) do { } while (0)
#endif
int debug_read_bstamps(unsigned long long* out, int n) {
    return hipMemcpyFromSymbol(out, HIP_SYMBOL(g_bstamps), sizeof(unsigned long long) * (n > 32 ? 32 : n)) == hipSuccess ? 0 : 1;
}

template <int CM, bool TILED, int DH, bool SLICED = false, bool CUT = false, bool RAGGED = false>
__global__ __launch_bounds__(256, 1) void fused_bwd_kernel(FusedBwdParams p) {
    static_assert(!(TILED && SLICED), "the tiled launches are not sliced");
    static_assert(!RAGGED || TILED, "ragged batches run the tiled launches");
    static_assert(!(CUT && (TILED || SLICED)), "the cut launches are neither tiled nor sliced");
    constexpr int HPW = FDH / DH, NHEAD = FH * HPW, NCT = DH / 16;
    constexpr int NT = 3;
    constexpr int SP = NT * 16;
    constexpr int BLK = SP * LDX;
    extern __shared__ __attribute__((aligned(16))) float lds[];
    float* Gs = lds;
    float* B1 = lds + 1 * BLK;
    float* B2 = lds + 2 * BLK;
    float* B3 = lds + 3 * BLK;
    float* B4 = lds + 4 * BLK;
    float* B5 = lds + 5 * BLK;
    float* stat = lds + 6 * BLK;
    float* PSB = stat + NHEAD * 3 * SP;

    const int tid = threadIdx.x, wave = tid >> 6;
    int lane = tid & 63, r = lane & 15, q = lane >> 4;
    int clip_ = blockIdx.x, slice_ = 0;
    if constexpr (SLICED) slice_map(p.n_slices, clip_, slice_);
    const int clip = clip_, slice = slice_;
    const int n_slices = SLICED ? p.n_slices : 1;
    int S, c_real, t0;
    size_t tok0;
    const int* rrec = nullptr;
    if constexpr (RAGGED) {
        c_real = p.rtab[(size_t)p.B_clips * RAGGED_REC + clip];
        rrec = p.rtab + (size_t)c_real * RAGGED_REC;
        t0 = (clip - rrec[RG_TILE0]) * 48;
        S = min(48, rrec[RG_S] - t0);
        tok0 = (size_t)rrec[RG_TOK0] + t0;
    } else if constexpr (TILED) {
        c_real = clip / p.tpc;
        t0 = (clip - c_real * p.tpc) * 48;
        S = min(48, p.S_clip - t0);
        tok0 = (size_t)c_real * p.S_clip + t0;
    } else {
        c_real = clip; t0 = 0; S = p.S; tok0 = (size_t)clip * S;
    }
    if (!CUT && p.zero_buf) {
        const size_t n4 = p.zero_n / 4, per = (n4 + gridDim.x - 1) / gridDim.x;
        const size_t b0 = (size_t)blockIdx.x * per, b1 = b0 + per < n4 ? b0 + per : n4;
        for (size_t k = b0 + threadIdx.x; k < b1; k += 256) reinterpret_cast<float4*>(p.zero_buf)[k] = make_float4(0, 0, 0, 0);
    }
    if constexpr (SLICED) { if (clip >= p.B || ((p.slice_drop >> slice) & 1)) return; }

    BSTAMP(12);
    float* part = p.partials + (size_t)clip * p.P;
#define EGX_PHASE()                                              \
    do {                                                         \
        int t_ = threadIdx.x;                                    \
        asm volatile("" : "+v"(t_));                             \
        lane = t_ & 63; r = lane & 15; q = lane >> 4;            \
    } while (0)

    const bool dev_seed = p.seed_ptr != nullptr;
    const uint64_t seed_dev = dev_seed ? *p.seed_ptr : 0ull;
    const uint64_t pos_key = dev_seed ? site_key(seed_dev, 0, SITE_POS) : p.pos_key;
    constexpr int BPF = SP * (FD / 4) / 256;
    static_assert(SP * (FD / 4) % 256 == 0, "a block must divide among the threads");
    auto blk_request = [&](f32x4 (&v)[BPF], const float* src) {
        int t_ = threadIdx.x;
        asm volatile("" : "+v"(t_));
        const f32x4* s4 = reinterpret_cast<const f32x4*>(src);
        const int n = S * (FD / 4);
#pragma unroll
        for (int k = 0; k < BPF; ++k) { const int i = t_ + 256 * k; v[k] = s4[i < n ? i : n - 1]; }
    };
    auto blk_store = [&](const f32x4 (&v)[BPF], float* dst, float* dst2) {
        int t_ = threadIdx.x;
        asm volatile("" : "+v"(t_));
#pragma unroll
        for (int k = 0; k < BPF; ++k) {
            const int i = t_ + 256 * k, row = i >> 5, c = (i & 31) << 2;
            if (i < S * (FD / 4)) {
                *reinterpret_cast<f32x4*>(dst + row * LDX + c) = v[k];
                if (dst2) *reinterpret_cast<f32x4*>(dst2 + row * LDX + c) = v[k];
            }
        }
    };
    f32x4 pf_a[BPF], pf_b[BPF];
    auto res_ptr = [&](int slot) -> const float* {
        return TILED ? p.saved_res + ((size_t)slot * p.Ntok + tok0) * FD : p.saved_res + ((size_t)slot * p.B + clip) * S * FD;
    };
    const int l_first = CUT ? p.cut_layer : TILED ? p.l_back : p.n_layers - 1;
    Touched tch = {{0, 0, 0, 0}};
    if constexpr (!TILED) { if (p.touch.n) tch = touch_lines<256>(p.touch, blockIdx.x, gridDim.x, tid); }
    blk_request(pf_a, CUT ? p.dy1 + tok0 * FD : l_first >= 0 ? res_ptr(2 * l_first + 1) : p.saved_pre + tok0 * FD);
    blk_request(pf_b, l_first >= 0 ? res_ptr(2 * l_first) : p.saved_pre + tok0 * FD);
    const int ps_g = tid >> 5, ps_c = (tid & 31) << 2;
    const f32x4 ln0_v = *reinterpret_cast<const f32x4*>(p.ln_w + ps_c);
    f32x4 n1_v = *reinterpret_cast<const f32x4*>(p.layer[l_first >= 0 ? l_first : 0].norm1_w + ps_c);
    static_assert((6 * BLK) % 4 == 0, "the blocks are zeroed in 16-byte pieces");
// ... 961 lines not shown
```

egot2_amd/csrc/fused_dev.h:

```cpp
#pragma once
#include "common.h"
#include "fused.h"

namespace egx {

constexpr int FD = 128;
constexpr int FH = 4;
constexpr int FDH = 32;
constexpr int LDX = FD + 4;
constexpr int LDV = 64 + 4;

enum { CM_F32 = 0, CM_BF16 = 1, CM_SPLIT = 2 };
typedef uint32_t u32x4 __attribute__((ext_vector_type(4)));

template <int CM> struct Frag { float v[8]; };
template <> struct Frag<CM_BF16> { bf16x8 v; };
template <> struct Frag<CM_SPLIT> { bf16x8 p[3]; };

__device__ __forceinline__ uint32_t pack_bf16(float a, float b) { return pack_bf16x2(a, b); }

__device__ __forceinline__ void split_pair(float x, float y, uint32_t& h, uint32_t& m, uint32_t& l) {
    typedef float f32x2 __attribute__((ext_vector_type(2)));
    h = pack_bf16(x, y);
    f32x2 v = {x, y};
// ... 247 lines not shown
#pragma unroll
    for (int k = 0; k < TOUCH_MAX; ++k) {
        const int kk = k < tl.n ? k : 0;
        const unsigned nl = tl.lines[kk], per = (nl + (unsigned)nblocks - 1) / (unsigned)nblocks;
        unsigned i = (unsigned)block * per + (unsigned)tid;
        i = (i < nl && (unsigned)tid < per) ? i : nl - 1;
        t.v[k] = *reinterpret_cast<const uint32_t*>(reinterpret_cast<const char*>(tl.base[kk]) + ((size_t)i << 7));
    }
    return t;
}
__device__ __forceinline__ void touch_sink(const Touched& t) {
#pragma unroll
    for (int k = 0; k < TOUCH_MAX; ++k) asm volatile("" :: "v"(t.v[k]));
}

struct FusedCe {
    const int64_t* target;
    const float* class_weight;
    float* loss;
    float* d_logits;
    int B;
    unsigned* ticket;
};
struct CeReq { int64_t y[2]; float w[2]; };
template <int NTHREADS>
__device__ __forceinline__ void ce_request_labels(const FusedCe& ce, int tid, CeReq& rq) {
#pragma unroll
    for (int k = 0; k < 2; ++k) { const int i = tid + k * NTHREADS; rq.y[k] = ce.target[i < ce.B ? i : ce.B - 1]; }
}
__device__ __forceinline__ void ce_request_weights(const FusedCe& ce, int n_out, CeReq& rq) {
#pragma unroll
    for (int k = 0; k < 2; ++k) {
        const int64_t y = rq.y[k];
        const int yc = (y >= 0 && y < n_out) ? (int)y : 0;
        rq.w[k] = ce.class_weight ? ce.class_weight[yc] : 1.f;
    }
}
template <int NTHREADS>
__device__ __forceinline__ void ce_weight_partials(const FusedCe& ce, int n_out, int tid, const CeReq& rq, float* red) {
    float s = 0.f;
#pragma unroll
    for (int k = 0; k < 2; ++k) {
        const int i = tid + k * NTHREADS;
        s += (i < ce.B && rq.y[k] >= 0 && rq.y[k] < n_out) ? rq.w[k] : 0.f;
    }
    for (int i = tid + 2 * NTHREADS; i < ce.B; i += NTHREADS) {
        const int64_t y = ce.target[i];
        if (y >= 0 && y < n_out) s += ce.class_weight ? ce.class_weight[y] : 1.f;
    }
    s = wave_sum(s);
    if ((tid & 63) == 0) red[tid >> 6] = s;
}
template <int NTHREADS>
__device__ __forceinline__ void ce_clip(const FusedCe& ce, int n_out, int clip, int lane, float z, const float* red, bool add_loss) {
    float wtot = 0.f;
#pragma unroll
    for (int w = 0; w < NTHREADS / 64; ++w) wtot += red[w];
    const int64_t y = ce.target[clip];
    const bool valid = y >= 0 && y < n_out;
    const float wy = valid ? (ce.class_weight ? ce.class_weight[y] : 1.f) : 0.f;
    const float zl = lane < n_out ? z : -INFINITY;
    const float m = wave_max(zl);
    const float e = lane < n_out ? __expf(zl - m) : 0.f;
    const float s = wave_sum(e);
    const float zy = __shfl(zl, valid ? (int)y : 0, 64);
    const float k = wy / wtot;
    if (lane < n_out) ce.d_logits[(size_t)clip * n_out + lane] = valid ? k * (e / s - (lane == (int)y ? 1.f : 0.f)) : 0.f;
    if (lane == 0 && add_loss) {
        float term = valid ? k * (m + __logf(s) - zy) : 0.f;
        if (wtot == 0.f && clip == 0) term = __builtin_nanf("");
        if (!ce.ticket) {
            atomicAdd(ce.loss, term);
        } else {
            float* acc = reinterpret_cast<float*>(ce.ticket + 1);
            atomicAdd(acc, term);
            __threadfence();
            if (atomicInc(ce.ticket, (unsigned)ce.B - 1u) == (unsigned)ce.B - 1u) {
                __threadfence();
                *ce.loss = atomicExch(acc, 0.f);
            }
        }
    }
}


template <class Fn, class Hook>
__device__ __forceinline__ void ln_rows(const float* buf, int S, const float* __restrict__ w, const float* __restrict__ b,
                                        float eps, Fn&& fn, Hook&& after_w) {
    const int row = threadIdx.x >> 2, part = threadIdx.x & 3;
    const int c0 = part * 32;
    f32x4 wq[8], bq[8];
#pragma unroll
    for (int j = 0; j < 8; ++j) {
        wq[j] = *reinterpret_cast<const f32x4*>(w + c0 + 4 * j);
        bq[j] = *reinterpret_cast<const f32x4*>(b + c0 + 4 * j);
    }
    after_w();
    if (row < S) {
        float x[32], y[32];
        float s = 0.f;
#pragma unroll
        for (int j = 0; j < 8; ++j) {
            float4 v = *reinterpret_cast<const float4*>(buf + row * LDX + c0 + 4 * j);
            x[4 * j] = v.x; x[4 * j + 1] = v.y; x[4 * j + 2] = v.z; x[4 * j + 3] = v.w;
            s += (v.x + v.y) + (v.z + v.w);
        }
        float mean = quad_sum(s) * (1.f / FD);
        float ss = 0.f;
#pragma unroll
        for (int j = 0; j < 32; ++j) { float t = x[j] - mean; ss += t * t; }
        float rstd = rsqrtf(quad_sum(ss) * (1.f / FD) + eps);
#pragma unroll
        for (int j = 0; j < 8; ++j) {
#pragma unroll
            for (int e = 0; e < 4; ++e) y[4 * j + e] = (x[4 * j + e] - mean) * rstd * wq[j][e] + bq[j][e];
        }
        fn(row, c0, x, y);
    } else {
        (void)quad_sum(0.f);
        (void)quad_sum(0.f);
// ... 320 lines not shown
```

egot2_amd/csrc/fused_host.h:

```cpp
#pragma once
#include "../../include/egot2x.h"
#include "common.h"

namespace egx {

struct LayerOff {
    size_t x_in, qkv, lse, attn_o, res1, stats1, x1, hid, res2, stats2;
};
struct Plan {
    int B = 0, S = 0, d = 0, H = 0, dff = 0, L = 0, nseg = 0;
    int vB = 0, tpc = 1;
    size_t N = 0;
    int seg_off[EGX_MAX_SEGMENTS];
    size_t seg_pre[EGX_MAX_SEGMENTS], seg_stats[EGX_MAX_SEGMENTS];
    LayerOff layer[64];
    size_t saved_bytes = 0;
    size_t s_dA = 0, s_dB = 0, s_dqkv = 0, s_dhid = 0, s_slab = 0, slab_bytes = 0, s_det = 0, det_bytes = 0;
    size_t scratch_bytes = 0;
};
int make_plan(const egx_config* cfg, const egx_segment* segs, int B, Plan& pl);

static inline size_t size_max(size_t a, size_t b) { return a > b ? a : b; }
static inline size_t take(size_t& cur, size_t bytes) {
    size_t o = cur;
    cur = align_up(cur + bytes, 256);
    return o;
}
static inline float* fptr(void* base, size_t off) { return (float*)((char*)base + off); }
static inline const float* cfptr(const void* base, size_t off) { return (const float*)((const char*)base + off); }

struct Drop {
    uint64_t key = 0;
    uint32_t thresh = 0;
    float inv_keep = 1.f;
};
static inline Drop make_drop(int training, float p, uint64_t seed, uint32_t layer, uint32_t site) {
    Drop dr;
    if (training && p > 0.f) {
        dr.key = site_key(seed, layer, site);
        dr.thresh = drop_threshold(p);
        dr.inv_keep = p < 1.f ? 1.f / (1.f - p) : 0.f;
    }
    return dr;
}
int linear_dx(const float* dy, const float* W, float* dx, int M, int N, int K, const float* mask, float mask_scale,
              const float* residual, int compute, hipStream_t st, void* slab = nullptr, size_t slab_bytes = 0);

bool packed_feats(const egx_segment* segs, int nseg);
bool fused_ok(const egx_config* cfg, const egx_segment* segs, const Plan& pl);
bool tiled_ok(const egx_config* cfg, const egx_segment* segs, const Plan& pl);
int fused_slices(const Plan& pl, int compute);
bool fused_token_ce_ok(const egx_config* cfg, const Plan& pl);
size_t fused_weight_cache_bytes(const egx_config* cfg, const egx_segment* segs, const Plan& pl);
void fused_workspace(const egx_config* cfg, const egx_segment* segs, const Plan& pl, size_t* saved, size_t* scratch);
int check_head(const egx_head* head);
int check_ce(const egx_ce* ce, bool with_head, const char* entry);
int fused_path_fwd(const egx_config* cfg, const egx_segment* segs, const Plan& pl, bool tiled, const float* ln_w, const float* ln_b,
                   const egx_layer* layers, const egx_head* head, float* tokens_out, float* logits_out, void* saved, int training,
                   uint64_t seed, hipStream_t st);
int fused_path_bwd(const egx_config* cfg, const egx_segment* segs, const Plan& pl, bool tiled, const float* ln_w, const float* ln_b,
                   const egx_layer* layers, const egx_head* head, float* d_tokens, const float* d_logits, const void* saved, void* scratch,
                   const egx_segment_grads* seg_grads, float* d_ln_w, float* d_ln_b, const egx_layer_grads* layer_grads,
                   const egx_head_grads* head_grads, int training, uint64_t seed, hipStream_t st);

}
```

egot2_amd/csrc/fused_host.hip:

```cpp
#include <string.h>
#include <vector>

#include "../../include/egot2x.h"
#include "common.h"
#include "kernels.h"
#include "fused.h"
#include "fused_host.h"

namespace egx {

bool packed_feats(const egx_segment* segs, int nseg) {
    for (int i = 0; i < nseg; ++i)
        if (segs[i].feat_bf16 || segs[i].pool > 1) return true;
    return false;
}
bool fused_ok(const egx_config* cfg, const egx_segment* segs, const Plan& pl) {
    if (pl.nseg > FUSED_MAX_SEG || pl.L > FUSED_MAX_LAYERS || pl.L < 1) return false;
    if (packed_feats(segs, pl.nseg)) return false;
    int d_in[EGX_MAX_SEGMENTS], T[EGX_MAX_SEGMENTS];
    bool hp[EGX_MAX_SEGMENTS];
    for (int i = 0; i < pl.nseg; ++i) { d_in[i] = segs[i].d_in; T[i] = segs[i].T; hp[i] = segs[i].proj_w != nullptr; }
    return fused_supported(pl.d, pl.H, pl.dff, pl.S, pl.nseg, d_in, T, hp);
}
static size_t fused_mask_words(const Plan& pl) { return (size_t)pl.L * pl.vB * (pl.dff / 32) * 64; }
// ... 186 lines not shown
    }
    s.bytes = cur;
    return s;
}

struct Packer {
    PackParams& pk;
    bool cache_hit;
    const void* operator()(const float* src, void* dst, int R, int K, int ld, int transpose, float scale = 1.f) {
        if (cache_hit) return dst;
        PackDesc& dsc = pk.d[pk.n++];
        dsc.src = src; dsc.dst = dst; dsc.R = R; dsc.K = K; dsc.ld = ld; dsc.transpose = transpose; dsc.scale = scale;
        return dst;
    }
};
static void fill_seg(FusedSeg& fs, const egx_segment& s, int i, const void* proj_wp = nullptr) {
    if (proj_wp) { fs.feat = s.feat; fs.proj_wp = proj_wp; fs.proj_b = s.proj_b; }
    fs.add_vec = s.add_vec; fs.pos = s.pos; fs.T = s.T; fs.d_in = s.d_in; fs.pos_stride = s.pos_stride;
    fs.Tfull = s.T; fs.seg_id = i;
}
static void fill_layer(FusedLayer& fl, const egx_layer& w, const FusedPackLayout::Layer& P, int d, int dff, float ffn_scale, Packer& pack) {
    fl.in_proj_wp = pack(w.in_proj_w, P.in_w, 3 * d, d, d, 0); fl.in_proj_b = w.in_proj_b;
    fl.out_proj_wp = pack(w.out_proj_w, P.out_w, d, d, d, 0); fl.out_proj_b = w.out_proj_b;
    fl.lin1_wp = pack(w.lin1_w, P.lin1_w, dff, d, d, 0, ffn_scale); fl.lin1_b = w.lin1_b;
    fl.lin2_wp = pack(w.lin2_w, P.lin2_w, d, dff, dff, 0); fl.lin2_b = w.lin2_b;
    pack(w.in_proj_w, P.in_wt, d, 3 * d, d, 1);
    pack(w.out_proj_w, P.out_wt, d, d, d, 1);
    pack(w.lin1_w, P.lin1_wt, d, dff, d, 1);
    pack(w.lin2_w, P.lin2_wt, dff, d, dff, 1, ffn_scale);
    fl.norm1_w = w.norm1_w; fl.norm1_b = w.norm1_b; fl.norm2_w = w.norm2_w; fl.norm2_b = w.norm2_b;
}
static void fill_bwd_layer(FusedBwdLayer& fl, const egx_layer& w, const FusedPackLayout::Layer& P) {
    fl.in_proj_wp = P.in_w; fl.in_proj_wtp = P.in_wt; fl.out_proj_wtp = P.out_wt;
    fl.lin1_wp = P.lin1_w; fl.lin2_wtp = P.lin2_wt; fl.lin1_wtp = P.lin1_wt;
    fl.in_proj_b = w.in_proj_b; fl.lin1_b = w.lin1_b;
    fl.norm1_w = w.norm1_w; fl.norm1_b = w.norm1_b; fl.norm2_w = w.norm2_w; fl.norm2_b = w.norm2_b;
}
template <class LayerT>
static void set_layer_drop(LayerT& fl, int training, float p, uint64_t seed, int l) {
    const Drop da = make_drop(training, p, seed, (uint32_t)l, SITE_ATTN);
    fl.attn_key = da.key; fl.attn_thresh = da.thresh; fl.drop_inv = da.inv_keep;
    fl.res_thresh = da.thresh; fl.ffn_thresh = da.thresh;
    fl.res1_key = make_drop(training, p, seed, (uint32_t)l, SITE_RES1).key;
    fl.ffn_key = make_drop(training, p, seed, (uint32_t)l, SITE_FFN).key;
    fl.res2_key = make_drop(training, p, seed, (uint32_t)l, SITE_RES2).key;
}

bool fused_token_ce_ok(const egx_config* cfg, const Plan& pl) {
    if (!cfg->weight_cache || cfg->deterministic) return false;
    if (pl.B > 4095) return false;
    const int ns = fused_slices(pl, cfg->compute);
    return ns == 1 && !use_cut(pl, ns, false, cfg->compute);
}
size_t fused_weight_cache_bytes(const egx_config* cfg, const egx_segment* segs, const Plan& pl) {
    if (pl.d != 128 || pl.nseg > FUSED_MAX_SEG || pl.L > FUSED_MAX_LAYERS || pl.L < 1 || pl.dff % 128 != 0) return 0;
    for (int i = 0; i < pl.nseg; ++i)
        if (!segs[i].proj_w || segs[i].d_in % 128 != 0) return 0;
    return align_up(fused_pack_layout(cfg, segs, pl, nullptr).bytes, 256) + 256;
}
void fused_workspace(const egx_config* cfg, const egx_segment* segs, const Plan& pl, size_t* saved, size_t* scratch) {
    *saved = 0; *scratch = 0;
    if (tiled_ok(cfg, segs, pl)) {
        Plan vp = pl;
        plan_tiled(vp);
        *saved = tiled_saved_bytes(cfg, segs, vp);
        *scratch = fused_bwd_scratch(cfg, segs, vp, FUSED_HEAD_MAX_OUT).bytes;
    }
    if (fused_ok(cfg, segs, pl)) {
        *saved = size_max(*saved, fused_saved_bytes(cfg, segs, pl));
        *scratch = size_max(*scratch, fused_bwd_scratch(cfg, segs, pl, FUSED_HEAD_MAX_OUT).bytes);
    }
}
int check_head(const egx_head* head) {
    EGX_CHECK(!(head && head->W) || (head->ln_w && head->ln_b && head->b && head->n_out >= 1 && head->n_out <= FUSED_HEAD_MAX_OUT),
              "head needs ln_w, ln_b, W, b and 1 <= n_out <= %d", FUSED_HEAD_MAX_OUT);
    return 0;
}
int check_ce(const egx_ce* ce, bool with_head, const char* entry) {
    EGX_CHECK(!ce || with_head, "egx_config.ce: the fused cross entropy needs the pooled head%s", entry);
    EGX_CHECK(!ce || (ce->target && ce->loss && ce->d_logits), "egx_config.ce: target, loss and d_logits must be set");
    return 0;
}

struct TiledView {
    char* base;
    size_t off_attn, off_lse, off_tokens;
    const int* rtab;
    int B_clips, tpc, S_clip;
    bool tiled;
    int rot_mode;
    bool keys;
};
static TiledView uniform_view(const egx_config* cfg, const egx_segment* segs, const Plan& vp, const void* saved, bool tiled) {
    TiledView v;
    memset(&v, 0, sizeof(v));
    v.base = (char*)const_cast<void*>(saved);
    if (tiled) { v.off_attn = tiled_attn_offset(cfg, segs, vp); v.off_lse = tiled_lse_offset(cfg, segs, vp); v.off_tokens = tiled_tokens_offset(cfg, segs, vp); }
    v.B_clips = vp.B; v.tpc = vp.tpc; v.S_clip = vp.S; v.tiled = tiled;
    v.rot_mode = FFN_ROT_XCD_STAGGER;
    v.keys = true;
    return v;
}

static void fill_fwd(FusedFwdParams& fp, PackParams& pk, const FusedPackLayout& PL, const TiledView& v, const egx_config* cfg, const egx_segment* segs,
                     const Plan& vp, const float* ln_w, const float* ln_b, const egx_layer* layers, int training, uint64_t seed) {
    const int d = vp.d;
// ... 174 lines not shown
    fp.w1p = PL.layer[l].lin1_w; fp.w2tp = PL.layer[l].lin2_wt; fp.b1 = layers[l].lin1_b;
    fp.N = (int)vp.N; fp.S = vp.S; fp.d_ff = vp.dff;
    fp.drop_key = bp.layer[l].ffn_key; fp.drop_thresh = bp.layer[l].ffn_thresh; fp.drop_inv = bp.layer[l].drop_inv;
    fp.seed_ptr = cfg->seed_ptr; fp.layer = l;
    const size_t lo = (size_t)l * fused_hid_bytes(vp.vB, vp.dff, comp == EGX_BF16);
    fp.hs = v.base + fused_hid_offset(cfg, segs, vp) + lo;
    fp.dhs = (const char*)scratch + SC.dhid + lo;
    fp.B = vp.vB;
    fp.xg_planes = bp.xg_planes;
    if (fp.xg_planes) fp.x1 = (const float*)(v.base + fused_x1p_offset(cfg, segs, vp) + (size_t)l * vp.vB * FUSED_TOK_PAD * vp.d * plane_elem_bytes(cfg));
    return ffn_dw(fp, comp, gw.lin1_w, gw.lin1_b, gw.lin2_w, (char*)scratch + SC.ffn_slab[l], st, nullptr, cfg->deterministic != 0, &red);
}

struct TailArgs { const SlabReduce* red; const ReducePartialsParams* rp; uint64_t* adv; const TouchList* tl; };
struct SmallDwQueue {
    int comp; hipStream_t st;
    void* slabs; size_t slab_bytes;
    const TailArgs* tail;
    SmallDwParams sp;
    bool first;
    SmallDwQueue(int comp_, hipStream_t st_, void* slabs_, size_t slab_bytes_, const TailArgs* tail_)
        : comp(comp_), st(st_), slabs(slabs_), slab_bytes(slab_bytes_), tail(tail_), first(true) { memset(&sp, 0, sizeof(sp)); }
    int flush() {
        if (sp.n && small_dw(sp, comp, st, slabs, slab_bytes, !tail)) return 1;
        const int rc = (tail && (sp.n || first)) ? tail_reduce(sp.n ? &sp : nullptr, first ? tail->red : nullptr, first ? tail->rp : nullptr,
                                                               first ? tail->adv : nullptr, first ? tail->tl : nullptr, st) : 0;
        first = false;
        memset(&sp, 0, sizeof(sp));
        return rc;
    }
    int add(const float* G, int ldg, const float* X, int ldx, float* out, int R, int Cc, int K) {
        if (!out || K <= 0) return 0;
        if (sp.n == SMALL_DW_MAX && flush()) return 1;
        SmallDwProblem& q = sp.pr[sp.n++];
        q.G = G; q.X = X; q.out = out; q.R = R; q.C = Cc; q.K = K; q.ldg = ldg; q.ldx = ldx;
        return 0;
    }
};
static int small_dw_all(SmallDwQueue& q, const FusedBwdParams& bp, const Plan& vp, const egx_layer_grads* layer_grads, const egx_segment* segs,
                        const egx_segment_grads* seg_grads, const float* const* feat, const size_t* seg_rows) {
    const int d = vp.d, N = (int)vp.N;
    for (int l = 0; l < vp.L; ++l) {
        const egx_layer_grads& gw = layer_grads[l];
        if (q.add(bp.layer[l].g1_out, d, bp.layer[l].attn_o_out, d, gw.out_proj_w, d, d, N)) return 1;
        if (q.add(bp.layer[l].dqkv_out, 3 * d, bp.layer[l].x_in_out, d, gw.in_proj_w, 3 * d, d, N)) return 1;
    }
    for (int i = 0; i < vp.nseg && seg_grads; ++i)
        if (q.add(bp.dseg_out[i], d, feat[i], segs[i].d_in, seg_grads[i].proj_w, d, segs[i].d_in, (int)seg_rows[i])) return 1;
    return q.flush();
}

int fused_path_fwd(const egx_config* cfg, const egx_segment* segs, const Plan& pl, bool tiled, const float* ln_w, const float* ln_b,
                   const egx_layer* layers, const egx_head* head, float* tokens_out, float* logits_out, void* saved, int training,
                   uint64_t seed, hipStream_t st) {
    const int d = pl.d, S = pl.S, B = pl.B, comp = cfg->compute;
    const bool with_head = head && head->W;
    const egx_ce* ce = cfg->ce;
    const egx_token_ce* tce = cfg->token_ce;
    Plan vp = pl;
    if (tiled) plan_tiled(vp);
    const TiledView v = uniform_view(cfg, segs, vp, saved, tiled);
    FusedPackLayout PL = fused_pack_layout(cfg, segs, vp, fused_pack_base(cfg, saved, vp));
    FusedFwdParams fp;
    PackParams pk;
    fill_fwd(fp, pk, PL, v, cfg, segs, vp, ln_w, ln_b, layers, training, seed);
    for (int i = 0; i < pl.nseg; ++i) {
        fp.seg[i].off = pl.seg_off[i]; fp.seg[i].row0 = 0;
        Drop df = make_drop(training, cfg->p_feat, seed, (uint32_t)i, SITE_FEAT);
        fp.feat_key[i] = df.key; fp.feat_thresh = df.thresh; fp.feat_inv = df.inv_keep;
    }
    fp.tokens_out = tokens_out;
    fp.out_T = cfg->out_tokens > 0 ? cfg->out_tokens : S;
    if (tiled) {
        if (!fp.tokens_out) fp.tokens_out = (float*)(v.base + v.off_tokens);
        if (pack_weights(pk, st)) return 1;
        return tiled_forward(fp, v, cfg, vp, head, logits_out, st);
    }
    if (with_head) {
        fp.head.ln_w = head->ln_w; fp.head.ln_b = head->ln_b; fp.head.W = head->W; fp.head.b = head->b; fp.head.n_out = head->n_out;
        fp.logits_out = logits_out;
    }
    fp.n_slices = fused_slices(pl, comp);
    if (fp.n_slices > 1) {
        fp.xchg = (float*)((char*)saved + fused_core_bytes(cfg, segs, vp));
        fp.xflags = (unsigned*)((char*)saved + fused_core_bytes(cfg, segs, vp) + sliced_xchg_bytes(pl, fused_slices_layout(pl)));
        pk.zero_words = fp.xflags; pk.n_zero = (int)sliced_flag_words(pl);
        fp.slice_drop = slice_drop_mask(fp.n_slices);
    }
    fp.x1f_out = (float*)((char*)saved + fused_x1f_offset(cfg, segs, vp));
    const bool cut = use_cut(pl, fp.n_slices, false, comp);
    const bool ce_fused = ce && with_head && !cfg->deterministic;
    if (ce_fused) {
        fp.ce_target = ce->target; fp.ce_weight = ce->class_weight; fp.ce_loss = ce->loss; fp.ce_dlogits = ce->d_logits; fp.ce_B = B;
        if (pk.n || pk.seed_advance || pk.zero_words) pk.zero_word2 = ce->loss;
        else if (cut) fp.zero_word = ce->loss;
        else if (cfg->weight_cache) fp.ce_ticket = (unsigned*)((char*)cfg->weight_cache + align_up(PL.bytes, 256));
        else EGX_HIP(hipMemsetAsync(ce->loss, 0, sizeof(float), st));
    }
    if (tce) {
        fp.tce_W = tce->W; fp.tce_b = tce->b; fp.tce_target = tce->target; fp.tce_cw = tce->class_weight; fp.tce_C = tce->C;
        fp.tce_logits = tce->logits; fp.tce_probs = tce->probs; fp.tce_pred = tce->pred; fp.tce_loss = tce->loss; fp.tce_correct = tce->correct;
        fp.tce_dlogits = tce->d_logits;
        fp.tce_ticket = (unsigned*)((char*)cfg->weight_cache + align_up(PL.bytes, 256)) + 4;
    }
    if (pack_weights(pk, st)) return 1;
    const bool touch = cfg->weight_cache != nullptr;
    const size_t ffn_pb = packed_bytes(pl.dff, d, comp), in_pb = packed_bytes(3 * d, d, comp), out_pb = packed_bytes(d, d, comp);
    if (cut) {
        fp.mode = FUSED_MODE_ATTN;
        for (int l = 0; l < pl.L; ++l) {
            fp.l0 = l;
            memset(&fp.touch, 0, sizeof(fp.touch));
            if (touch) { touch_add(fp.touch, PL.layer[l].lin1_w, ffn_pb); touch_add(fp.touch, PL.layer[l].lin2_w, ffn_pb); }
            if (fused_forward(fp, comp, st)) return 1;
            fp.zero_word = nullptr;
            memset(&fp.touch, 0, sizeof(fp.touch));
            if (touch && l + 1 < pl.L) { touch_add(fp.touch, PL.layer[l + 1].in_w, in_pb); touch_add(fp.touch, PL.layer[l + 1].out_w, out_pb); }
            else if (touch && training) { touch_add(fp.touch, PL.layer[l].lin2_wt, ffn_pb); touch_add(fp.touch, PL.layer[l].lin1_wt, ffn_pb); }
            if (ffn_cut_forward(fp, l, comp, st)) return 1;
        }
    } else {
        if (touch) {
            touch_add(fp.touch, PL.layer[0].lin1_w, ffn_pb); touch_add(fp.touch, PL.layer[0].lin2_w, ffn_pb);
            if (training) { touch_add(fp.touch, PL.layer[pl.L - 1].lin2_wt, ffn_pb); touch_add(fp.touch, PL.layer[pl.L - 1].lin1_wt, ffn_pb); }
        }
        if (fused_forward(fp, comp, st)) return 1;
    }
    if (ce && with_head && !ce_fused) return weighted_ce(logits_out, ce->target, ce->class_weight, B, head->n_out, ce->loss, ce->d_logits, st);
    return 0;
}

int fused_path_bwd(const egx_config* cfg, const egx_segment* segs, const Plan& pl, bool tiled, const float* ln_w, const float* ln_b,
                   const egx_layer* layers, const egx_head* head, float* d_tokens, const float* d_logits, const void* saved, void* scratch,
                   const egx_segment_grads* seg_grads, float* d_ln_w, float* d_ln_b, const egx_layer_grads* layer_grads,
                   const egx_head_grads* head_grads, int training, uint64_t seed, hipStream_t st) {
    const int d = pl.d, S = pl.S, B = pl.B, comp = cfg->compute;
    const bool with_head = head && head->W;
    Plan vp = pl;
    if (tiled) plan_tiled(vp);
    const TiledView v = uniform_view(cfg, segs, vp, saved, tiled);
    FusedPackLayout PL = fused_pack_layout(cfg, segs, vp, fused_pack_base(cfg, saved, vp));
    const egx_token_ce* tce = cfg->token_ce;
    if (tce) {
        EGX_CHECK(!with_head && !tiled && fused_token_ce_ok(cfg, pl), "egx_config.token_ce: not on this configuration (egx_encoder_token_ce_ok)");
        EGX_CHECK(tce->W && tce->d_logits && tce->C >= 1 && tce->C <= 8, "egx_config.token_ce: W, d_logits and 1 <= C <= 8 must be set");
    }
    FusedBwdScratch SC = fused_bwd_scratch(cfg, segs, vp, with_head ? head->n_out : tce ? tce->C : 0);
    FusedBwdParams bp;
    if (fill_bwd(bp, PL, SC, v, cfg, segs, vp, ln_w, ln_b, layers, head, d_logits, d_tokens, scratch, training, seed)) return 1;
    const bool touch = cfg->weight_cache != nullptr && !tiled;
    const size_t ffn_pb = packed_bytes(pl.dff, d, comp), in_pb = packed_bytes(3 * d, d, comp), out_pb = packed_bytes(d, d, comp);
    for (int i = 0; i < pl.nseg; ++i) {
        bp.seg[i].off = pl.seg_off[i]; bp.seg[i].row0 = 0;
        Drop df = make_drop(training, cfg->p_feat, seed, (uint32_t)i, SITE_FEAT);
        bp.feat_key[i] = df.key; bp.feat_thresh = df.thresh; bp.feat_inv = df.inv_keep;
    }
    bool want_pos = false;
    for (int i = 0; i < pl.nseg && seg_grads; ++i) want_pos = want_pos || seg_grads[i].pos;
    bp.dx0_out = want_pos ? fptr(scratch, SC.dx0) : nullptr;
    bp.out_T = cfg->out_tokens > 0 ? cfg->out_tokens : S;
    if (tce) {
        bp.tce_W = tce->W; bp.tce_dlogits = tce->d_logits; bp.tce_C = tce->C;
        bp.d_logits_scale = cfg->d_logits_scale;
        bp.head_off = fused_partial_len(pl.L, pl.nseg);
    }
    const int stage = cfg->bwd_stage;
    EGX_CHECK(stage >= 0 && stage <= 2, "bwd_stage=%d", stage);
    if (stage == 2) bp.zero_buf = nullptr;
    if (!tiled) bp.n_slices = fused_slices(pl, comp);
    if (bp.n_slices > 1 && stage != 2) {
        bp.xchg = fptr(scratch, SC.xchg);
        bp.xflags = (unsigned*)((char*)const_cast<void*>(saved) + fused_core_bytes(cfg, segs, vp) + sliced_xchg_bytes(pl, fused_slices_layout(pl))) + sliced_flag_words(pl);
        EGX_HIP(hipMemsetAsync(bp.xflags, 0, sliced_flag_words(pl) * 4, st));
        bp.slice_drop = slice_drop_mask(bp.n_slices);
    }
    if (stage != 2 && tiled) {
        if (tiled_backward(bp, SC, v, cfg, vp, scratch, st)) return 1;
    } else if (stage != 2 && use_cut(pl, bp.n_slices, tiled, comp)) {
        bp.cut = 1; bp.dy1 = fptr(scratch, SC.dy1); bp.dxin = fptr(scratch, SC.dxin);
        for (int l = pl.L - 1; l >= 0; --l) {
            bp.cut_layer = l;
            memset(&bp.touch, 0, sizeof(bp.touch));
            if (touch) { touch_add(bp.touch, PL.layer[l].out_wt, out_pb); touch_add(bp.touch, PL.layer[l].in_wt, in_pb); }
            if (ffn_cut_backward(bp, l, comp, st)) return 1;
            bp.zero_buf = nullptr;
            memset(&bp.touch, 0, sizeof(bp.touch));
            if (touch && l > 0) { touch_add(bp.touch, PL.layer[l - 1].lin2_wt, ffn_pb); touch_add(bp.touch, PL.layer[l - 1].lin1_wt, ffn_pb); }
            if (fused_backward(bp, comp, st)) return 1;
        }
    } else if (stage != 2) {
        if (touch) { touch_add(bp.touch, PL.layer[pl.L - 1].out_wt, out_pb); touch_add(bp.touch, PL.layer[pl.L - 1].in_wt, in_pb); }
        if (fused_backward(bp, comp, st)) return 1;
    }

    for (int i = 0; i < pl.nseg && seg_grads; ++i)
        EGX_CHECK(!seg_grads[i].feat, "fused backward: feature gradients are not supported (use impl=generic)");
    ReducePartialsParams rp;
    partial_dsts(rp, bp, layer_grads, d_ln_w, d_ln_b, seg_grads, head, head_grads, tce);
    if (bp.dx0_out && stage != 2)
        for (int i = 0; i < pl.nseg; ++i)
            if (seg_grads[i].pos && pos_grad_accum(bp.dx0_out, B, S, pl.seg_off[i], segs[i].T, d, seg_grads[i].pos, segs[i].pos_stride, 0, 0, 1.f, st)) return 1;
    bool rp_pending = stage != 2;
    SlabReduce red;
    red.narr = 0; red.nslab = 0;
    for (int l = 0; l < pl.L && stage != 2; ++l)
        if (launch_ffn_dw(l, bp, PL, SC, v, cfg, segs, vp, layers, layer_grads, scratch, red, st)) return 1;
    uint64_t* adv = (cfg->advance_seed == 2 && cfg->seed_ptr && training && stage != 1) ? const_cast<uint64_t*>(cfg->seed_ptr) : nullptr;
    const float* feat[EGX_MAX_SEGMENTS];
    size_t seg_rows[EGX_MAX_SEGMENTS];
    for (int i = 0; i < pl.nseg; ++i) { feat[i] = segs[i].feat; seg_rows[i] = (size_t)(B * segs[i].T); }
    if (stage == 0) {
        TouchList tl;
        memset(&tl, 0, sizeof(tl));
        if (touch) {
            touch_add(tl, PL.proj[0], (size_t)((const char*)PL.layer[0].in_wt - (const char*)PL.proj[0]));
            touch_add(tl, PL.layer[0].out_w, out_pb);
        }
        const TailArgs tail = {&red, &rp, adv, &tl};
        SmallDwQueue q(comp, st, (char*)scratch + SC.sdw_tiles, SC.sdw_bytes, &tail);
        return small_dw_all(q, bp, vp, layer_grads, segs, seg_grads, feat, seg_rows);
    }
    if (red.narr) {
        if (ffn_dw_reduce(red, rp_pending ? &rp : nullptr, cfg->deterministic != 0, st)) return 1;
        rp_pending = false;
    }
    if (rp_pending && reduce_partials(rp, st, cfg->deterministic != 0)) return 1;
    if (stage != 1) {
        SmallDwQueue q(comp, st, cfg->deterministic ? (char*)scratch + SC.slabs : nullptr, SC.slab_bytes, nullptr);
        if (small_dw_all(q, bp, vp, layer_grads, segs, seg_grads, feat, seg_rows)) return 1;
    }
    if (adv && seed_advance(adv, st)) return 1;
    return 0;
}

}

using namespace egx;

namespace {
struct RaggedPlan {
    Plan vp;
// ... 242 lines not shown
```

egot2_amd/functional.py:

```python
from __future__ import annotations

import ctypes as C
import dataclasses
from dataclasses import dataclass, field
from typing import List, Optional, Sequence

import torch

from . import _lib
from ._lib import (Ce, Config, Head, HeadGrads, Layer, LayerGrads, Segment, SegmentGrads, check, ptr,
                   EGX_F32, EGX_BF16, EGX_F32_SPLIT, EGX_IMPL_AUTO, EGX_IMPL_GENERIC, EGX_IMPL_FUSED, EGX_IMPL_WIDE, EGX_IMPL_TILED)

COMPUTE = {"f32": EGX_F32, "fp32": EGX_F32, "float32": EGX_F32, "bf16": EGX_BF16, "bfloat16": EGX_BF16, "f32s": EGX_F32_SPLIT}
IMPL = {"auto": EGX_IMPL_AUTO, "generic": EGX_IMPL_GENERIC, "fused": EGX_IMPL_FUSED, "wide": EGX_IMPL_WIDE, "tiled": EGX_IMPL_TILED}


@dataclass
class SegmentSpec:
    T: int
    d_in: int
    has_proj: bool
    add_row: Optional[int] = None
    pos_row0: Optional[int] = None
    pool: int = 1
# ... 388 lines not shown

class EncoderFn(torch.autograd.Function):

    @staticmethod
    def forward(ctx, spec: EncoderSpec, task_embed, pos_table, ln_w, ln_b, *rest):
        lib = _load()
        nseg = len(spec.segments)
        nhead = 4 if spec.head_n_out else 0
        if spec.token_ce and (nhead or spec.ce):
            raise _lib.EgxError("EncoderSpec.token_ce cannot be combined with the pooled head")
        if spec.ce and not nhead:
            raise _lib.EgxError("EncoderSpec.ce needs the pooled head (head_n_out > 0)")
        feats, proj, layer_t, head_t, tail = _EncArgs.split(spec, rest)
        feats, proj, layer_t, head_t, ln_w, ln_b, task_embed, pos_table = _dev_params(feats, proj, layer_t, head_t, ln_w, ln_b, task_embed,
                                                                                      pos_table)
        assert len(layer_t) == 12 * spec.n_layers, "layer parameter count mismatch"
        d = spec.d_model
        B = feats[0].shape[0]
        device = feats[0].device
        segs = _segments(spec, feats, proj, task_embed, pos_table, B)
        layers = _layers(layer_t, spec.n_layers)

        nig = ctx.needs_input_grad
        if spec.impl == "auto" and (nig[2] or any(nig[5:5 + nseg])):
            feat_grad = [bool(nig[5 + i]) for i in range(nseg)]
            probe_cfg = spec.config()
            wide_ident_only = (lib.egx_encoder_impl(C.byref(probe_cfg), segs, B) == EGX_IMPL_WIDE
                               and not any(fg and ss.has_proj for fg, ss in zip(feat_grad, spec.segments)))
            if any(feat_grad) and not wide_ident_only:
                spec = dataclasses.replace(spec, impl="generic")
        py_slice = 0
        if spec.out_tokens and nhead:
            raise _lib.EgxError("out_tokens (first-tokens-only output) cannot be combined with the fused pooled head: the head pools "
                                "every token of the clip")
        if spec.out_tokens:
            full = dataclasses.replace(spec, out_tokens=0)
            probe = full.config()
            if nhead or lib.egx_encoder_impl(C.byref(probe), segs, B) != EGX_IMPL_FUSED:
                py_slice, spec = spec.out_tokens, full
        cfg = spec.config()
        sv, sc = C.c_size_t(0), C.c_size_t(0)
        ws = lib.egx_translator_workspace if nhead else lib.egx_encoder_workspace
        check(ws(C.byref(cfg), segs, B, C.byref(sv), C.byref(sc)))
        S = sum(s.T for s in spec.segments)
        saved = _saved_buffer(any(nig), "saved", device, sv.value)
        scratch = _workspace("scratch", device, sc.value)
        seed = _seed64(spec.seed)
        wc, wc_sig = _attach_weight_cache(lib, spec, cfg, segs, proj, layer_t, device)
        keep = tw = tb = None
        if spec.ce:
            loss, ctx.ce_dl, keep = _ce_attach(spec, cfg, tail[0], tail[1], B, device)
        if spec.token_ce:
            keep, tce_out, ctx.tce_dl, tw, tb = _token_ce_attach(lib, spec, cfg, segs, tail, wc is not None and not py_slice, B, S, device)
        if nhead:
            head = _head(head_t, spec.head_n_out)
            tokens = torch.empty((B, spec.head_n_out), dtype=torch.float32, device=device)
            check(lib.egx_translator_fwd(C.byref(cfg), segs, ptr(ln_w), ptr(ln_b), layers, C.byref(head), B, ptr(tokens),
                                         None, ptr(saved), ptr(scratch), int(spec.training), seed, _stream()))
        else:
            tokens = torch.empty((B, spec.out_tokens or S, d), dtype=torch.float32, device=device)
            check(lib.egx_encoder_fwd(C.byref(cfg), segs, ptr(ln_w), ptr(ln_b), layers, B, ptr(tokens), ptr(saved),
                                      ptr(scratch), int(spec.training), seed, _stream()))
            if py_slice:
                tokens = tokens[:, :py_slice].contiguous()
        del keep
        if wc is not None:
            wc.sig = wc_sig
        ctx.wcache_buf = wc.buf if wc is not None else None
        ctx.py_slice, ctx.S, ctx.B = py_slice, S, B
        ctx.spec = spec
        ctx.impl = lib.egx_encoder_impl(C.byref(cfg), segs, B)
        _last_impl[0] = ctx.impl
        _last_slices[0] = lib.egx_encoder_slices(C.byref(cfg), segs, B) if ctx.impl == EGX_IMPL_FUSED else 1
        ctx.saved_buf, ctx.scratch_bytes = saved, sc.value
        _EncArgs.save(ctx, task_embed, pos_table, ln_w, ln_b, feats, proj, layer_t, head_t, [t for t in (tw, tb) if t is not None])
        if spec.token_ce:
            ctx.mark_non_differentiable(*tce_out[1:])
            ctx.set_materialize_grads(False)
            return (tokens,) + tce_out
        if spec.ce:
            ctx.set_materialize_grads(False)
            return tokens, loss
        return tokens

    @staticmethod
    def backward(ctx, d_tokens, d_loss=None, *_aux):
        spec: EncoderSpec = ctx.spec
        dl_scale = None
        if spec.token_ce:
            if d_tokens is not None:
                raise _lib.EgxError("EncoderSpec.token_ce: a gradient through the returned tokens as well as through the fused loss is not supported "
                                    "(compose encoder() and linear_cross_entropy() instead)")
            if d_loss is None:
                return (None,) * len(ctx.needs_input_grad)
            dl_scale = _f32c(d_loss)
            d_tokens = ctx.tce_dl
        if spec.ce:
            up = _ce_upstream(ctx, d_tokens, d_loss)
            if up is None:
                return (None,) * len(ctx.needs_input_grad)
            d_tokens, dl_scale = up
        if ctx.py_slice:
            full = torch.zeros((d_tokens.shape[0], ctx.S, d_tokens.shape[2]), dtype=torch.float32, device=d_tokens.device)
            full[:, :ctx.py_slice] = d_tokens
            d_tokens = full
        lib = _load()
        tensors = _EncArgs.load(ctx)
        task_embed, pos_table, ln_w, ln_b, feats, proj, layer_t, head_t, tce_t = tensors
        B = ctx.B
        device = d_tokens.device
        hook = bucket_hook
        gr = _EncGrads(spec, ctx.needs_input_grad, 5, tensors, device, late=hook is None, bucketed=hook is not None)
        pk = gr.pk
        segs, sgr = _segments(spec, feats, proj, task_embed, pos_table, B, grads=gr.segments())
        layers, lgr = _layers(layer_t, spec.n_layers, gr.layers)

        cfg = spec.config()
        gr.attach(cfg)
        if ctx.wcache_buf is not None:
            cfg.weight_cache = ctx.wcache_buf.data_ptr()
        if dl_scale is not None:
            cfg.d_logits_scale = dl_scale.data_ptr()
        tce_keep = None
        if spec.token_ce:
            tce_keep = _lib.TokenCe(ptr(tce_t[0]), None, None, None, int(spec.token_ce), None, None, None, None, None, ptr(ctx.tce_dl),
                                    *map(ptr, (gr.tail + [None])[:2]))
            cfg.token_ce = C.cast(C.pointer(tce_keep), C.c_void_p)
        announced = set()
        cb_keep = None
        if hook is not None and ctx.impl == EGX_IMPL_WIDE:
            flat_for_cb, spans = pk.flat, dict(pk.rank_span)

            cb_error = []

            def _cb(_user, bucket):
                if cb_error or bucket not in spans or bucket in announced:
                    return
                try:
                    hook(flat_for_cb, spans[bucket][0], spans[bucket][1])
                    announced.add(bucket)
                except BaseException as e:
                    cb_error.append(e)
            cb_keep = _lib.BUCKET_CB(_cb)
            cfg.bucket_cb = C.cast(cb_keep, C.c_void_p)
        defer = bool(spec.defer_small) and ctx.impl == EGX_IMPL_FUSED
        cfg.bwd_stage = 1 if defer else 0
        scratch = _workspace("scratch", device, ctx.scratch_bytes)
        seed = _seed64(spec.seed)
        saved_buf = ctx.saved_buf
        p_lnw, p_lnb, flat_buf = ptr(gr.first[2]), ptr(gr.first[3]), pk.flat
        if head_t:
            head, hg = _head(head_t, spec.head_n_out), gr.head_grads()
            dtok = _f32c(d_tokens)

            def launch(c):
                check(lib.egx_translator_bwd(C.byref(c), segs, ptr(ln_w), ptr(ln_b), layers, C.byref(head), B, ptr(dtok),
                                             ptr(saved_buf), ptr(scratch), sgr, p_lnw, p_lnb, lgr,
                                             C.byref(hg), int(spec.training), seed, _stream()))
        else:
            if spec.token_ce:
                dtok = None
            else:
                dtok = _f32c(d_tokens)
                if dtok.data_ptr() == d_tokens.data_ptr() and ctx.impl == EGX_IMPL_GENERIC:
                    dtok = dtok.clone()

            def launch(c):
                check(lib.egx_encoder_bwd(C.byref(c), segs, ptr(ln_w), ptr(ln_b), layers, B, ptr(dtok), ptr(saved_buf),
                                          ptr(scratch), sgr, p_lnw, p_lnb, lgr, int(spec.training), seed,
                                          _stream()))
        launch(cfg)
        del tce_keep
        if cb_keep is not None and cb_error:
            raise cb_error[0]
        if hook is not None and not defer:
            done = sorted(pk.rank_span[b] for b in announced)
            cur = 0
            for lo, hi in done + [(pk.total, pk.total)]:
                if lo > cur:
                    hook(pk.flat, cur, lo)
                cur = max(cur, hi)
        last_grad_layout.update(flat=pk.flat, late_floats=pk.late_floats if defer else 0)
        if defer:
            cfg2 = spec.config()
            cfg2.bwd_stage = 2
            if ctx.wcache_buf is not None:
                cfg2.weight_cache = ctx.wcache_buf.data_ptr()
            keep = (flat_buf, tensors, dtok, scratch, saved_buf)

            def finish(_keep=keep):
                launch(cfg2)
            _deferred.append(finish)
        return gr.result(2 if spec.ce else 4 - len(gr.tail) if spec.token_ce else 0)


def encoder(spec: EncoderSpec, feats: Sequence[torch.Tensor], task_embed, pos_table, ln_w, ln_b,
            proj: Sequence[torch.Tensor], layer_params: Sequence[torch.Tensor],
            head_params: Sequence[torch.Tensor] = (), ce=None):
    if spec.ce:
        return EncoderFn.apply(spec, task_embed, pos_table, ln_w, ln_b, *feats, *proj, *layer_params, *head_params, ce[0], ce[1])
    return EncoderFn.apply(spec, task_embed, pos_table, ln_w, ln_b, *feats, *proj, *layer_params, *head_params)


def ragged_lengths(lengths, B: int, T_pad: Sequence[int], order: Optional[Sequence[int]] = None) -> torch.Tensor:
    K = len(T_pad)
    t = lengths.detach() if isinstance(lengths, torch.Tensor) else torch.as_tensor(lengths)
    if t.dtype.is_floating_point or t.dtype.is_complex or t.dtype == torch.bool:
        raise ValueError(f"lengths must be integers, got {t.dtype}")
    t = t.to("cpu", torch.int64)
    if t.dim() == 1:
        t = t[:, None].expand(t.shape[0], K)
# ... 1822 lines not shown
```

include/egot2x.h:

```cpp
#ifndef EGOT2X_H
#define EGOT2X_H

#include <stddef.h>
#include <stdint.h>

#ifdef __cplusplus
extern "C" {
#endif

#define EGX_ABI_VERSION 18
#define EGX_MAX_SEGMENTS 8

enum { EGX_F32 = 0, EGX_BF16 = 1, EGX_F32_SPLIT = 2 };
enum { EGX_IMPL_AUTO = 0, EGX_IMPL_GENERIC = 1, EGX_IMPL_FUSED = 2, EGX_IMPL_WIDE = 3, EGX_IMPL_TILED = 4 };

typedef struct egx_segment {
    const float* feat;
    int T;
    int d_in;
    const float* proj_w;
    const float* proj_b;
    const float* add_vec;
    const float* pos;
    int pos_stride;
// ... 228 lines not shown
enum { EGX_LR_CONSTANT = 0, EGX_LR_COSINE_ANNEALING = 1, EGX_LR_WARMUP_COSINE = 2, EGX_LR_WARMUP_LINEAR = 3, EGX_LR_TABLE = 4 };
#define EGX_LR_MAX_GROUPS 16
typedef struct egx_lr_schedule {
    int kind;
    int64_t warmup_steps;
    int64_t t_total;
    int64_t T_max;
    double cycles;
    const double* factors;
    int64_t n;
} egx_lr_schedule;
int egx_lr_update(const egx_lr_schedule* schedule, int64_t* step, const double* base_lr, int n_groups, float* lr_out,
                  void* stream);
int egx_adam_step_dev_lr(float* param, const float* grad, float* exp_avg, float* exp_avg_sq, size_t n, const int64_t* step,
                         const float* lr, float beta1, float beta2, float eps, float weight_decay, int decoupled,
                         float grad_scale, void* stream);
int egx_sgd_step(float* param, const float* grad, float* momentum_buf, size_t n, const int64_t* step, const float* lr_dev,
                 float lr, float momentum, float dampening, float weight_decay, int nesterov, float grad_scale,
                 void* stream);
size_t egx_segmented_ce_scratch(int B, int Z, int H, int n_ks);
int egx_segmented_ce(const float* logits, int ld, const int64_t* target, int B, int Z, int H, const int* col0, const int* C,
                     const int* ks, int n_ks, float* loss, float* loss_terms, int* n_valid, int* correct, float* d_logits,
                     void* scratch, void* stream);
int egx_lta_validate(const float* logits, int ld, const int64_t* labels, int B, int Z, int H, const int* col0, const int* C, int K,
                     uint64_t seed, const uint64_t* seed_ptr, const int64_t* preds_in, int64_t* preds, int* min_dist,
                     int64_t* dist_sum, void* stream);
enum { EGX_KF_BCE = 0, EGX_KF_CE = 1, EGX_KF_METRIC = 2 };
size_t egx_keyframe_scratch(int B);
int egx_keyframe_criterion(const float* logits, int ld, int B, int T, const int* cols, int V, int kind, const float* target,
                           const int64_t* label, const int64_t* state_change, const double* fps, const int64_t* clip_start,
                           const int64_t* clip_end, const int64_t* pnr_frame, float* loss, float* loss_rows, float* d_logits,
                           int* pred, int* label_frame, int* counts, double* dist, double* dist_sum, void* scratch, void* stream);
typedef struct egx_seq_task {
    const float* logits; long long stride_b, stride_s;
    int B, sy;
    const int64_t* target; long long target_stride_b, target_stride_s;
    float ratio;
    float* d_logits;
    const int* word_label;
    const int64_t* labels; long long labels_stride_b, labels_stride_s;
    int* pred;
} egx_seq_task;
size_t egx_sequence_ce_scratch(void);
int egx_sequence_ce(const egx_seq_task* tasks, int T, int V, void* result, void* scratch, void* stream);
size_t egx_segment_ap_scratch(int capacity);
int egx_segment_scores_update(const float* logits, int ld, int B, const int64_t* slots, int slot0, const int64_t* labels, int capacity,
                              void* scratch, void* stream);
int egx_segment_ap(int N, int capacity, void* scratch, float* score, int* order1, int* order0, void* result, void* stream);
size_t egx_view_ensemble_state(int capacity, int H, const int* C, size_t* offsets);
int egx_view_ensemble_update(const float* preds, int ld, int B, int H, const int* col0, const int* C, const int64_t* labels, const void* slots,
                             int slot_bytes, int slot0, int method, int capacity, void* state, void* stream);
int egx_view_ensemble_topk(int n, int capacity, int H, const int* C, const int* ks, int n_ks, void* state, int* rank, int* pred, void* result,
                           void* stream);
int egx_small_attention_fwd(const float* q, int ldq, const float* k, int ldk, const float* v, int ldv, float* o, int ldo,
                            int B, int Sq, int Sk, int H, int dh, int causal, float p_drop, uint64_t seed, uint32_t site,
                            void* stream);
int egx_small_attention_bwd(const float* q, int ldq, const float* k, int ldk, const float* v, int ldv, const float* d_o,
                            int ldo, float* dq, float* dk, float* dv, int B, int Sq, int Sk, int H, int dh, int causal,
                            float p_drop, uint64_t seed, uint32_t site, void* stream);
int egx_embed_pos_fwd(const int64_t* tokens, const float* emb, const float* pe, int pe_stride, float scale, float* out,
                      int B, int sy, int d, int V, float p_drop, uint64_t seed, void* stream);
int egx_embed_pos_bwd(const int64_t* tokens, const float* dy, float* d_emb, float scale, int B, int sy, int d, int V,
                      float p_drop, uint64_t seed, void* stream);
typedef struct egx_dec_config {
    int d_model, n_heads, d_ff, n_layers;
    int vocab;
    int sy, S;
    float ln_eps;
    int compute;
    float p_drop;
    float p_pos;
    const uint64_t* seed_ptr;
} egx_dec_config;
typedef struct egx_dec_layer {
    const float* sa_in_w; const float* sa_in_b; const float* sa_out_w; const float* sa_out_b; const float* norm1_w; const float* norm1_b;
    const float* ca_in_w; const float* ca_in_b; const float* ca_out_w; const float* ca_out_b; const float* norm2_w; const float* norm2_b;
    const float* lin1_w; const float* lin1_b; const float* lin2_w; const float* lin2_b; const float* norm3_w; const float* norm3_b;
} egx_dec_layer;
typedef struct egx_dec_layer_grads {
    float* sa_in_w; float* sa_in_b; float* sa_out_w; float* sa_out_b; float* norm1_w; float* norm1_b;
    float* ca_in_w; float* ca_in_b; float* ca_out_w; float* ca_out_b; float* norm2_w; float* norm2_b;
    float* lin1_w; float* lin1_b; float* lin2_w; float* lin2_b; float* norm3_w; float* norm3_b;
} egx_dec_layer_grads;
int egx_decoder_workspace(const egx_dec_config* cfg, int B, size_t* saved_bytes, size_t* scratch_bytes);
int egx_decoder_fwd(const egx_dec_config* cfg, const int64_t* tokens, const float* memory, const float* emb, const float* pe, int pe_stride,
                    const egx_dec_layer* layers, const float* fc_w, const float* fc_b, int B, float* logits, void* saved, void* scratch,
                    int training, uint64_t seed, void* stream);
int egx_decoder_bwd(const egx_dec_config* cfg, const int64_t* tokens, const egx_dec_layer* layers, const float* fc_w, int B, const float* d_logits,
                    const void* saved, void* scratch, float* d_memory, float* d_emb, const egx_dec_layer_grads* grads, float* d_fc_w,
                    float* d_fc_b, void* zero_buf, size_t zero_bytes, int training, uint64_t seed, void* stream);
int egx_decoder_ragged_workspace(const egx_dec_config* cfg, int B, const int* mem_lengths, size_t* bytes);
int egx_decoder_ragged_fwd(const egx_dec_config* cfg, const int64_t* tokens, const float* memory, const int* mem_lengths, const float* emb,
                           const float* pe, int pe_stride, const egx_dec_layer* layers, const float* fc_w, const float* fc_b, int B,
                           float* logits, void* workspace, void* stream);
int egx_decoder_ragged_train_workspace(const egx_dec_config* cfg, int B, const int* mem_lengths, size_t* saved_bytes, size_t* scratch_bytes);
int egx_decoder_ragged_train_fwd(const egx_dec_config* cfg, const int64_t* tokens, const float* memory, const int* mem_lengths, const float* emb,
                                 const float* pe, int pe_stride, const egx_dec_layer* layers, const float* fc_w, const float* fc_b, int B,
                                 float* logits, void* saved, void* scratch, int training, uint64_t seed, void* stream);
int egx_decoder_ragged_bwd(const egx_dec_config* cfg, const int64_t* tokens, const int* mem_lengths, const egx_dec_layer* layers, const float* fc_w,
                           int B, const float* d_logits, const void* saved, void* scratch, float* d_memory, float* d_emb,
                           const egx_dec_layer_grads* grads, float* d_fc_w, float* d_fc_b, void* zero_buf, size_t zero_bytes, int training,
                           uint64_t seed, void* stream);
int egx_decoder_generate_workspace(const egx_dec_config* cfg, int B, int n_steps, size_t* bytes);
int egx_decoder_generate(const egx_dec_config* cfg, const int64_t* start, const float* memory, const float* emb, const float* pe, int pe_stride,
                         const egx_dec_layer* layers, const float* fc_w, const float* fc_b, int B, int n_steps, int64_t* tokens_out,
                         float* logits_out , void* workspace, void* stream);
// ... 63 lines not shown
```

Measured before the change: 685,600 clips/s.

## Fuse last-layer FFN forward with its backward in one round-trip kernel

Adds a 'round' path for the translator: the last layer's FFN forward kernel, after computing the head and weighted CE in its epilogue, continues straight into the FFN backward for the same clip. It prefetches the backward weight ring and ReLU bits before the forward's final reduction and reuses the pooled activations left in LDS, so the separate FFN backward launch and its reload of the residual and head state are skipped. The backward entry point then omits that kernel. This makes forward and backward share a scratch buffer and become order-coupled, and it is restricted to fused, non-deterministic training with a unit upstream gradient. It also adds a guard against the weight cache being re-packed between the two calls.

Result: no change. 681,300 clips/s (-0.6%).

```diff
diff --git a/egot2_amd/_lib.py b/egot2_amd/_lib.py
--- a/egot2_amd/_lib.py
+++ b/egot2_amd/_lib.py
@@ -143,6 +143,12 @@
     "egx_translator_bwd": (C.c_int, [C.POINTER(Config), C.POINTER(Segment), _fp, _fp, C.POINTER(Layer), C.POINTER(Head),
                                      C.c_int, _fp, _fp, _fp, C.POINTER(SegmentGrads), _fp, _fp, C.POINTER(LayerGrads),
                                      C.POINTER(HeadGrads), C.c_int, C.c_uint64, _fp]),
+    "egx_translator_round_ok": (C.c_int, [C.POINTER(Config), C.POINTER(Segment), C.POINTER(Head), C.c_int, C.c_int]),
+    "egx_translator_fwd_round": (C.c_int, [C.POINTER(Config), C.POINTER(Segment), _fp, _fp, C.POINTER(Layer), C.POINTER(Head),
+                                           C.c_int, _fp, _fp, _fp, _fp, C.c_int, C.c_uint64, _fp]),
+    "egx_translator_bwd_round": (C.c_int, [C.POINTER(Config), C.POINTER(Segment), _fp, _fp, C.POINTER(Layer), C.POINTER(Head),
+                                           C.c_int, _fp, _fp, _fp, C.POINTER(SegmentGrads), _fp, _fp, C.POINTER(LayerGrads),
+                                           C.POINTER(HeadGrads), C.c_int, C.c_uint64, _fp]),
     "egx_small_attention_fwd": (C.c_int, [_fp, C.c_int, _fp, C.c_int, _fp, C.c_int, _fp, C.c_int, C.c_int, C.c_int, C.c_int,
                                           C.c_int, C.c_int, C.c_int, C.c_float, C.c_uint64, C.c_uint32, _fp]),
     "egx_small_attention_bwd": (C.c_int, [_fp, C.c_int, _fp, C.c_int, _fp, C.c_int, _fp, C.c_int, _fp, _fp, _fp, C.c_int,
diff --git a/egot2_amd/csrc/common.h b/egot2_amd/csrc/common.h
--- a/egot2_amd/csrc/common.h
+++ b/egot2_amd/csrc/common.h
@@ -47,6 +47,7 @@
     bool has_drop = false; long slice_drop = 0;
     int dec_group = -1;
     int wide_tile = 0;
+    int ffn_round = 0;
     int dec_side = 1;
 };
 const Tuning& tuning();
diff --git a/egot2_amd/csrc/encoder.hip b/egot2_amd/csrc/encoder.hip
--- a/egot2_amd/csrc/encoder.hip
+++ b/egot2_amd/csrc/encoder.hip
@@ -109,6 +109,7 @@
     if (const char* e = getenv("EGX_SLICE_DROP")) { t.has_drop = true; t.slice_drop = strtol(e, nullptr, 16); }
     if (const char* e = getenv("EGX_DEC_GROUP")) t.dec_group = atoi(e);
     if (const char* e = getenv("EGX_WIDE_TILE")) t.wide_tile = atoi(e);
+    if (const char* e = getenv("EGX_FFN_ROUND")) t.ffn_round = e[0] != '0' ? 1 : 0;
     if (const char* e = getenv("EGX_DEC_SIDE")) t.dec_side = e[0] == '0' ? 0 : e[0] == '2' ? 2 : 1;
     g_tuning = t;
     g_tuning_loaded = true;
@@ -412,8 +413,7 @@
 
 static int encoder_fwd_impl(const egx_config* cfg, const egx_segment* segs, const float* ln_w, const float* ln_b,
                             const egx_layer* layers, const egx_head* head, int B, float* tokens_out, float* logits_out,
-                            void* saved, void* scratch, int training, uint64_t seed, void* stream) {
-    (void)scratch;
+                            void* saved, void* scratch, int training, uint64_t seed, void* stream, bool round = false) {
     Plan pl;
     if (make_plan(cfg, segs, B, pl)) return 1;
     EGX_CHECK(saved && ln_w && ln_b, "null pointer argument");
@@ -439,7 +439,8 @@
     bool ferr, terr = false, werr;
     const bool fused = use_fused(cfg, segs, pl, &ferr);
     const bool tiled = !fused && !ferr && use_tiled(cfg, segs, pl, &terr);
-    if (fused || tiled) return fused_path_fwd(cfg, segs, pl, tiled, ln_w, ln_b, layers, head, tokens_out, logits_out, saved, training, seed, st);
+    EGX_CHECK(!round || (fused && scratch), "egx_translator_fwd_round: not on this configuration (egx_translator_round_ok), or null scratch");
+    if (fused || tiled) return fused_path_fwd(cfg, segs, pl, tiled, ln_w, ln_b, layers, head, tokens_out, logits_out, saved, training, seed, st, round ? scratch : nullptr);
     if (ferr || terr) return 1;
     EGX_CHECK(cfg->out_tokens == 0 || cfg->out_tokens == pl.S, "out_tokens is implemented by the fused per-clip kernels only (egx_encoder_impl() == EGX_IMPL_FUSED)");
     if (use_wide(cfg, segs, pl, &werr)) return wide_path_fwd(cfg, segs, pl, ln_w, ln_b, layers, head, tokens_out, logits_out, saved, training, seed, st);
@@ -580,7 +581,7 @@
                             const egx_layer* layers, const egx_head* head, int B, float* d_tokens, const float* d_logits,
                             const void* saved, void* scratch, const egx_segment_grads* seg_grads, float* d_ln_w,
                             float* d_ln_b, const egx_layer_grads* layer_grads, const egx_head_grads* head_grads,
-                            int training, uint64_t seed, void* stream) {
+                            int training, uint64_t seed, void* stream, bool round = false) {
     (void)ln_b;
     Plan pl;
     if (make_plan(cfg, segs, B, pl)) return 1;
@@ -590,8 +591,9 @@
     bool ferr, terr = false, werr;
     const bool fused = use_fused(cfg, segs, pl, &ferr);
     const bool tiled = !fused && !ferr && use_tiled(cfg, segs, pl, &terr);
+    EGX_CHECK(!round || fused, "egx_translator_bwd_round: not on this configuration (egx_translator_round_ok)");
     if (fused || tiled) return fused_path_bwd(cfg, segs, pl, tiled, ln_w, ln_b, layers, head, d_tokens, d_logits, saved, scratch, seg_grads, d_ln_w, d_ln_b,
-                                              layer_grads, head_grads, training, seed, st);
+                                              layer_grads, head_grads, training, seed, st, round);
     if (ferr || terr) return 1;
     if (use_wide(cfg, segs, pl, &werr)) return wide_path_bwd(cfg, segs, pl, ln_w, layers, head, d_tokens, d_logits, saved, scratch, seg_grads, d_ln_w, d_ln_b,
                                                              layer_grads, head_grads, training, seed, st);
@@ -646,6 +648,30 @@
                             d_ln_b, layer_grads, head_grads, training, seed, stream);
 }
 
+int egx_translator_round_ok(const egx_config* cfg, const egx_segment* segs, const egx_head* head, int B, int training) {
+    Plan pl;
+    if (!cfg || !segs || make_plan(cfg, segs, B, pl)) return 0;
+    bool ferr;
+    return use_fused(cfg, segs, pl, &ferr) && fused_round_ok(cfg, pl, head, training);
+}
+
+int egx_translator_fwd_round(const egx_config* cfg, const egx_segment* segs, const float* ln_w, const float* ln_b,
+                             const egx_layer* layers, const egx_head* head, int B, float* logits_out, float* tokens_out,
+                             void* saved, void* scratch, int training, uint64_t seed, void* stream) {
+    EGX_CHECK(head && head->W, "egx_translator_fwd_round needs a head");
+    return encoder_fwd_impl(cfg, segs, ln_w, ln_b, layers, head, B, tokens_out, logits_out, saved, scratch, training, seed, stream, true);
+}
+
+int egx_translator_bwd_round(const egx_config* cfg, const egx_segment* segs, const float* ln_w, const float* ln_b,
+                             const egx_layer* layers, const egx_head* head, int B, const float* d_logits, const void* saved,
+                             void* scratch, const egx_segment_grads* seg_grads, float* d_ln_w, float* d_ln_b,
+                             const egx_layer_grads* layer_grads, const egx_head_grads* head_grads, int training,
+                             uint64_t seed, void* stream) {
+    EGX_CHECK(head && head->W, "egx_translator_bwd_round needs a head");
+    return encoder_bwd_impl(cfg, segs, ln_w, ln_b, layers, head, B, nullptr, d_logits, saved, scratch, seg_grads, d_ln_w,
+                            d_ln_b, layer_grads, head_grads, training, seed, stream, true);
+}
+
 int egx_pool_head_fwd(const float* tokens, int B, int S, int d, const float* ln_w, const float* ln_b, float ln_eps,
                       const float* W, const float* b, int n_out, float* pooled_saved, float* out, void* stream) {
     EGX_CHECK(tokens && pooled_saved && out, "null pointer argument");
diff --git a/egot2_amd/csrc/ffn_cut.hip b/egot2_amd/csrc/ffn_cut.hip
--- a/egot2_amd/csrc/ffn_cut.hip
+++ b/egot2_amd/csrc/ffn_cut.hip
@@ -1,4 +1,5 @@
 #include <stdlib.h>
+#include <string.h>
 #include "common.h"
 #include "kernels.h"
 #include "fused.h"
@@ -143,8 +144,22 @@
 }
 }
 
-template <int CM>
-__global__ __launch_bounds__(CT) void ffn_fwd_kernel(FusedFwdParams p, int l) {
+struct FfnRoundBwd {
+    FusedBwdLayer lw;
+    FusedHead head; int head_off;
+    int n_layers, B, S, d_ff, rot_mode, xg_planes, P;
+    float eps;
+    float* partials; void* dhid_out; float* dy1;
+    const uint32_t* relu_bits;
+    const uint64_t* seed_ptr;
+    TouchList touch;
+};
+template <int CM> struct RoundCarry { WRaw<CM> ring[RingDepth<CM>::v]; uint32_t relu_word; };
+
+template <int CM> __device__ __forceinline__ void ffn_bwd_request(const FfnRoundBwd& p, const FusedBwdLayer& w, int l, RoundCarry<CM>& rc);
+
+template <int CM, bool ROUND>
+__device__ __forceinline__ void ffn_fwd_body(const FusedFwdParams& p, int l, const FfnRoundBwd* rb, RoundCarry<CM>* rc) {
     extern __shared__ __attribute__((aligned(16))) float lds[];
     float* X1 = lds;
     float* R = lds + CBLK;
@@ -381,6 +396,7 @@
     ASTAMP(18);
     __syncthreads();
     ASTAMP(19);
+    if constexpr (ROUND) ffn_bwd_request<CM>(*rb, rb->lw, l, *rc);
     reduce_partials8(y, R, wave, r, q);
     ASTAMP(20);
 
@@ -411,12 +427,18 @@
         return;
     }
     if (p.head.n_out > 0) {
-        float* pooled = X1;
+        float* pooled = ROUND ? lds + 2 * CBLK : X1;
+        float* ce_red = ROUND ? CP + 5 * FD + 128 : pooled + 256;
         const FusedCe ce{p.ce_target, p.ce_weight, p.ce_loss, p.ce_dlogits, p.ce_B, nullptr};
         CeReq rq;
         if (ce.target) { ce_request_labels<CT>(ce, tid, rq); ce_request_weights(ce, p.head.n_out, rq); }
         if (tid < FD) pooled[tid] = colsum_lds(Y, 0, S, tid) * (1.f / (float)S);
-        if (ce.target) ce_weight_partials<CT>(ce, p.head.n_out, tid, rq, pooled + 256);
+        if (ce.target) ce_weight_partials<CT>(ce, p.head.n_out, tid, rq, ce_red);
+        if constexpr (ROUND) {
+            f32x4* z = reinterpret_cast<f32x4*>(lds + 2 * CBLK);
+            for (int i = 64 + tid; i < 3 * CBLK / 4; i += CT) z[i] = f32x4{0, 0, 0, 0};
+            for (int i = tid; i < (CSP - S) * LDX; i += CT) Y[S * LDX + i] = 0.f;
+        }
         __syncthreads();
         if (wave == 0) {
             float2 x = *reinterpret_cast<float2*>(pooled + 2 * lane);
@@ -434,14 +456,42 @@
                 if (lane == 0) p.logits_out[(size_t)clip * p.head.n_out + o] = sdot;
                 zmine = lane == o ? sdot : zmine;
             }
-            if (ce.target) ce_clip<CT>(ce, p.head.n_out, clip, lane, zmine, pooled + 256, true);
+            if (ce.target) ce_clip<CT>(ce, p.head.n_out, clip, lane, zmine, ce_red, true, ROUND ? CP + 5 * FD + 64 : nullptr);
         }
     }
     ASTAMP(23);
 }
-
 template <int CM>
-__global__ __launch_bounds__(CT) void ffn_bwd_kernel(FusedBwdParams p, int l) {
+__global__ __launch_bounds__(CT) void ffn_fwd_kernel(FusedFwdParams p, int l) { ffn_fwd_body<CM, false>(p, l, nullptr, nullptr); }
+
+struct BwdWalk { int nit, j_begin, pair_s, rot; __device__ __forceinline__ int hb_of(int it) const { int j = it + rot; if (j >= nit) j -= nit; return pair_s + 4 * (j_begin + j); } };
+template <int CM, class P>
+__device__ __forceinline__ BwdWalk bwd_walk(const P& p, int wave, int clip) {
+    int j_begin_, n_mine_;
+    cut_walk<CM, false>(wave, p.d_ff / 32 / 8, j_begin_, n_mine_, p.rot_mode >> 8);
+    BwdWalk k;
+    k.nit = __builtin_amdgcn_readfirstlane(n_mine_); k.j_begin = __builtin_amdgcn_readfirstlane(j_begin_);
+    k.pair_s = __builtin_amdgcn_readfirstlane(wave & 3);
+    k.rot = cut_rot(p.rot_mode & 255, clip, k.nit);
+    return k;
+}
+template <int CM>
+__device__ __forceinline__ WRaw<CM> bwd_frag_load(const FusedBwdLayer& w, int nhb, int k, int hb, int lane) {
+    return k < 8 ? load_w<CM>(w.lin2_wtp, hb * 2 + (k & 1), FD / 32, k >> 1, lane) : load_w<CM>(w.lin1_wtp, k - 8, nhb, hb, lane);
+}
+template <int CM>
+__device__ __forceinline__ void ffn_bwd_request(const FfnRoundBwd& p, const FusedBwdLayer& w, int l, RoundCarry<CM>& rc) {
+    constexpr int D = RingDepth<CM>::v;
+    const int lane = threadIdx.x & 63, nhb = p.d_ff / 32;
+    const BwdWalk wk = bwd_walk<CM>(p, threadIdx.x >> 6, blockIdx.x);
+    const int hb0 = wk.hb_of(0);
+#pragma unroll
+    for (int k = 0; k < D; ++k) rc.ring[k] = bwd_frag_load<CM>(w, nhb, k, hb0, lane);
+    rc.relu_word = (p.relu_bits + ((size_t)l * p.B + blockIdx.x) * (size_t)nhb * 64 + lane)[(size_t)hb0 * 64];
+}
+
+template <int CM, bool ROUND, class P>
+__device__ __forceinline__ void ffn_bwd_body(const P& p, const FusedBwdLayer& w, int l, RoundCarry<CM>* rc) {
     extern __shared__ __attribute__((aligned(16))) float lds[];
     float* B1 = lds;
     float* Gs = lds + 1 * CBLK;
@@ -453,7 +503,6 @@
     const int tid = threadIdx.x, wave = tid >> 6, lane = tid & 63, r = lane & 15, q = lane >> 4;
     const int clip = blockIdx.x, S = p.S;
     const size_t tok0 = (size_t)clip * S;
-    const FusedBwdLayer& w = p.layer[l];
     const bool dev_seed = p.seed_ptr != nullptr;
     const uint64_t seed_dev = dev_seed ? *p.seed_ptr : 0ull;
     const uint64_t k_res2 = dev_seed ? site_key(seed_dev, l, SITE_RES2) : w.res2_key;
@@ -462,22 +511,32 @@
     ASTAMP(24);
     Touched tch = {{0, 0, 0, 0}};
     if (p.touch.n) tch = touch_lines<CT>(p.touch, blockIdx.x, gridDim.x, tid);
+    if constexpr (!ROUND) {
     if (p.zero_buf) {
         const size_t n4 = p.zero_n / 4, per = (n4 + gridDim.x - 1) / gridDim.x;
         const size_t b0 = (size_t)blockIdx.x * per, b1 = b0 + per < n4 ? b0 + per : n4;
         for (size_t k = b0 + threadIdx.x; k < b1; k += CT) reinterpret_cast<float4*>(p.zero_buf)[k] = make_float4(0, 0, 0, 0);
     }
+    }
     float* part = p.partials + (size_t)clip * p.P;
     float* pl = part + l * FUSED_P_LAYER;
 
     const int nhb = p.d_ff / 32;
-    int j_begin_, n_mine_;
-    cut_walk<CM, false>(wave, nhb / 8, j_begin_, n_mine_, p.rot_mode >> 8);
-    const int nit = __builtin_amdgcn_readfirstlane(n_mine_), j_begin = __builtin_amdgcn_readfirstlane(j_begin_);
-    const int pair_s = __builtin_amdgcn_readfirstlane(wave & 3);
-    const int rot = cut_rot(p.rot_mode & 255, clip, nit);
-    auto hb_of = [&](int it) { int j = it + rot; if (j >= nit) j -= nit; return pair_s + 4 * (j_begin + j); };
+    const BwdWalk wk = bwd_walk<CM>(p, wave, clip);
+    const int nit = wk.nit;
+    auto hb_of = [&](int it) { return wk.hb_of(it); };
     float* CP = lds + 5 * CBLK;
+    constexpr int XR = CSP * (FD / 4) / CT;
+    const uint32_t* relu_bits = p.relu_bits + ((size_t)l * p.B + clip) * (size_t)nhb * 64 + lane;
+    auto frag_load = [&](int k, int hb) -> WRaw<CM> { return bwd_frag_load<CM>(w, nhb, k, hb, lane); };
+    WRaw<CM> ring[D];
+    uint32_t relu_word;
+    const bool head_bwd = last && p.head.n_out > 0;
+    if constexpr (ROUND) {
+#pragma unroll
+        for (int k = 0; k < D; ++k) ring[k] = rc->ring[k];
+        relu_word = rc->relu_word;
+    } else {
     const bool cp_hd = p.head.n_out > 0 && last;
     const int cp_g = tid >> 5, cp_c4 = (tid & 31) << 2;
     f32x4 cp_v, cp_w;
@@ -497,12 +556,6 @@
             if (p.head.n_out <= CP_HEAD_ROWS && tid >= 256 && tid < 256 + p.head.n_out * 32) *reinterpret_cast<f32x4*>(CP + 1024 + (tid - 256) * 4) = cp_w;
         }
     };
-    auto frag_load = [&](int k, int hb) -> WRaw<CM> {
-        return k < 8 ? load_w<CM>(w.lin2_wtp, hb * 2 + (k & 1), FD / 32, k >> 1, lane) : load_w<CM>(w.lin1_wtp, k - 8, nhb, hb, lane);
-    };
-    const uint32_t* relu_bits = p.relu_bits + ((size_t)l * p.B + clip) * (size_t)nhb * 64 + lane;
-    WRaw<CM> ring[D];
-    uint32_t relu_word;
     {
         const int hb0 = hb_of(0);
 #pragma unroll
@@ -510,9 +563,7 @@
         relu_word = relu_bits[(size_t)hb0 * 64];
     }
     const float* res2 = p.saved_res + ((size_t)(2 * l + 1) * p.B + clip) * S * FD;
-    const bool head_bwd = last && p.head.n_out > 0;
     {
-        constexpr int XR = CSP * (FD / 4) / CT;
         f32x4 rr[XR], dr[XR];
         const f32x4* rs = reinterpret_cast<const f32x4*>(res2);
         const int ndy_rows = head_bwd ? 0 : (last ? p.out_T : S);
@@ -538,15 +589,18 @@
         }
         touch_sink(tch);
     }
+    }
     ASTAMP(25);
-    if (head_bwd) {
+    if (ROUND || head_bwd) {
         float* hp = part + p.head_off;
+        float* pooled = B2;
+        if constexpr (!ROUND) {
         __syncthreads();
         ln_rows(Gs, S, CP, CP + FD, p.eps, [&](int row, int c0, float (&x)[32], float (&y)[32]) { store32(Gs + row * LDX + c0, y); });
         __syncthreads();
-        float* pooled = B2;
         if (tid < FD) pooled[tid] = colsum_lds(Gs, 0, S, tid) * (1.f / (float)S);
         __syncthreads();
+        }
         if (wave == 0) {
             float2 x = *reinterpret_cast<float2*>(pooled + 2 * lane);
             float mean = wave_sum(x.x + x.y) * (1.f / FD);
@@ -587,6 +641,7 @@
         }
         if (tid < 64) *reinterpret_cast<f32x4*>(B2 + 4 * tid) = f32x4{0, 0, 0, 0};
     }
+    if constexpr (ROUND) touch_sink(tch);
     __syncthreads();
     ASTAMP(26);
     ln_bwd_rows(S, CP, p.eps,
@@ -712,6 +767,15 @@
     }
     ASTAMP(31);
 }
+template <int CM>
+__global__ __launch_bounds__(CT) void ffn_bwd_kernel(FusedBwdParams p, int l) { ffn_bwd_body<CM, false>(p, p.layer[l], l, nullptr); }
+
+template <int CM>
+__global__ __launch_bounds__(CT) void ffn_round_kernel(FusedFwdParams p, FfnRoundBwd b, int l) {
+    RoundCarry<CM> rc;
+    ffn_fwd_body<CM, true>(p, l, &b, &rc);
+    ffn_bwd_body<CM, true>(b, b.lw, l, &rc);
+}
 
 bool ffn_cut_supported(int d_ff) { return d_ff % 256 == 0 && d_ff >= 256; }
 size_t ffn_cut_lds_bytes() { return (size_t)(5 * CBLK + CP_FLOATS) * sizeof(float); }
@@ -745,6 +809,19 @@
     return 0;
 }
 
+template <int CM>
+static int launch_cut_round(const FusedFwdParams& p, const FfnRoundBwd& b, int l, hipStream_t st) {
+    const size_t lds = ffn_cut_lds_bytes();
+    static bool attr_set = false;
+    if (!attr_set) {
+        EGX_HIP(hipFuncSetAttribute(reinterpret_cast<const void*>(&ffn_round_kernel<CM>), hipFuncAttributeMaxDynamicSharedMemorySize, (int)lds));
+        attr_set = true;
+    }
+    hipLaunchKernelGGL((ffn_round_kernel<CM>), dim3(p.B), dim3(CT), lds, st, p, b, l);
+    EGX_LAUNCH_CHECK();
+    return 0;
+}
+
 int ffn_cut_forward(const FusedFwdParams& p, int l, int compute, hipStream_t st) {
     EGX_CHECK(ffn_cut_supported(p.d_ff) && p.S <= CSP && l >= 0 && l < p.n_layers, "ffn_cut_forward: d_ff=%d S=%d layer %d", p.d_ff, p.S, l);
     EGX_CHECK(p.x1f_out && p.xin_out && p.saved_res && p.relu_bits && p.hid_out, "ffn_cut_forward: missing buffers");
@@ -756,4 +833,24 @@
     return compute == CM_BF16 ? launch_cut_bwd<CM_BF16>(p, l, st) : compute == CM_SPLIT ? launch_cut_bwd<CM_SPLIT>(p, l, st) : launch_cut_bwd<CM_F32>(p, l, st);
 }
 
-}
+int ffn_cut_round(const FusedFwdParams& fp, const FusedBwdParams& bp, int l, int compute, hipStream_t st) {
+    EGX_CHECK(ffn_cut_supported(fp.d_ff) && fp.S <= CSP && l >= 0 && l + 1 == fp.n_layers, "ffn_cut_round: d_ff=%d S=%d layer %d of %d", fp.d_ff, fp.S, l, fp.n_layers);
+    EGX_CHECK(fp.x1f_out && fp.xin_out && fp.saved_res && fp.relu_bits && fp.hid_out, "ffn_cut_round: missing forward buffers");
+    EGX_CHECK(fp.head.n_out > 0 && fp.head.n_out <= FUSED_HEAD_MAX_OUT && fp.ce_target && fp.ce_dlogits && fp.logits_out, "ffn_cut_round: needs the pooled head with the fused cross entropy");
+    EGX_CHECK(bp.dy1 && bp.dhid_out && bp.partials && bp.layer[l].g2_out, "ffn_cut_round: missing backward buffers");
+    EGX_CHECK(!bp.d_logits_scale && !bp.zero_buf && bp.d_logits == fp.ce_dlogits, "ffn_cut_round: upstream gradient 1 on the forward's own d_logits, no zero_buf");
+    EGX_CHECK(bp.B == fp.B && bp.S == fp.S && bp.d_ff == fp.d_ff && bp.n_layers == fp.n_layers && bp.head.n_out == fp.head.n_out && bp.relu_bits == fp.relu_bits &&
+              bp.seed_ptr == fp.seed_ptr && bp.rot_mode == fp.rot_mode, "ffn_cut_round: forward and backward blocks disagree");
+    FfnRoundBwd b;
+    memset(&b, 0, sizeof(b));
+    b.lw = bp.layer[l];
+    b.head = bp.head; b.head_off = bp.head_off;
+    b.n_layers = bp.n_layers; b.B = bp.B; b.S = bp.S; b.d_ff = bp.d_ff; b.rot_mode = bp.rot_mode; b.xg_planes = bp.xg_planes; b.P = bp.P;
+    b.eps = bp.eps;
+    b.partials = bp.partials; b.dhid_out = bp.dhid_out; b.dy1 = bp.dy1;
+    b.relu_bits = bp.relu_bits; b.seed_ptr = bp.seed_ptr;
+    b.touch = bp.touch;
+    return compute == CM_BF16 ? launch_cut_round<CM_BF16>(fp, b, l, st) : compute == CM_SPLIT ? launch_cut_round<CM_SPLIT>(fp, b, l, st) : launch_cut_round<CM_F32>(fp, b, l, st);
+}
+
+}
diff --git a/egot2_amd/csrc/fused.h b/egot2_amd/csrc/fused.h
--- a/egot2_amd/csrc/fused.h
+++ b/egot2_amd/csrc/fused.h
@@ -190,6 +190,7 @@
 size_t ffn_cut_lds_bytes();
 int ffn_cut_forward(const FusedFwdParams& p, int l, int compute, hipStream_t st);
 int ffn_cut_backward(const FusedBwdParams& p, int l, int compute, hipStream_t st);
+int ffn_cut_round(const FusedFwdParams& fp, const FusedBwdParams& bp, int l, int compute, hipStream_t st);
 
 struct SmallDwProblem {
     const float* G; const float* X; float* out;
@@ -218,6 +219,7 @@
 enum { TIMER_FUSED_FWD = 0, TIMER_FUSED_BWD = 1, TIMER_FFN_DW = 2, TIMER_FFN_FWD = 3, TIMER_FFN_BWD = 4, TIMER_WIDE_GEMM = 5,
        TIMER_WIDE_ATTN_FWD = 6, TIMER_WIDE_ATTN_BWD = 7, TIMER_COUNT = 8 };
 void timing_enable(int on);
+bool timing_enabled();
 void timing_begin(int which, hipStream_t st);
 void timing_end(int which, hipStream_t st);
 int timing_read(int which, double* total_ms, int* count);
diff --git a/egot2_amd/csrc/fused.hip b/egot2_amd/csrc/fused.hip
--- a/egot2_amd/csrc/fused.hip
+++ b/egot2_amd/csrc/fused.hip
@@ -1097,6 +1097,7 @@
     g_timing_on = on;
     for (int i = 0; i < TIMER_COUNT; ++i) g_timers[i].n = 0;
 }
+bool timing_enabled() { return g_timing_on != 0; }
 void timing_begin(int which, hipStream_t st) {
     if (!g_timing_on) return;
     TimerSlot& t = g_timers[which];
diff --git a/egot2_amd/csrc/fused_bwd.hip b/egot2_amd/csrc/fused_bwd.hip
--- a/egot2_amd/csrc/fused_bwd.hip
+++ b/egot2_amd/csrc/fused_bwd.hip
@@ -1186,7 +1186,7 @@
     } else {
         c_real = clip; t0 = 0; S = p.S; tok0 = (size_t)clip * S;
     }
-    if (!CUT && p.zero_buf) {
+    if (p.zero_buf) {
         const size_t n4 = p.zero_n / 4, per = (n4 + gridDim.x - 1) / gridDim.x;
         const size_t b0 = (size_t)blockIdx.x * per, b1 = b0 + per < n4 ? b0 + per : n4;
         for (size_t k = b0 + threadIdx.x; k < b1; k += 256) reinterpret_cast<float4*>(p.zero_buf)[k] = make_float4(0, 0, 0, 0);
diff --git a/egot2_amd/csrc/fused_dev.h b/egot2_amd/csrc/fused_dev.h
--- a/egot2_amd/csrc/fused_dev.h
+++ b/egot2_amd/csrc/fused_dev.h
@@ -323,7 +323,7 @@
     if ((tid & 63) == 0) red[tid >> 6] = s;
 }
 template <int NTHREADS>
-__device__ __forceinline__ void ce_clip(const FusedCe& ce, int n_out, int clip, int lane, float z, const float* red, bool add_loss) {
+__device__ __forceinline__ void ce_clip(const FusedCe& ce, int n_out, int clip, int lane, float z, const float* red, bool add_loss, float* dl_lds = nullptr) {
     float wtot = 0.f;
 #pragma unroll
     for (int w = 0; w < NTHREADS / 64; ++w) wtot += red[w];
@@ -336,7 +336,9 @@
     const float s = wave_sum(e);
     const float zy = __shfl(zl, valid ? (int)y : 0, 64);
     const float k = wy / wtot;
-    if (lane < n_out) ce.d_logits[(size_t)clip * n_out + lane] = valid ? k * (e / s - (lane == (int)y ? 1.f : 0.f)) : 0.f;
+    const float dl = valid ? k * (e / s - (lane == (int)y ? 1.f : 0.f)) : 0.f;
+    if (lane < n_out) ce.d_logits[(size_t)clip * n_out + lane] = dl;
+    if (dl_lds && lane < n_out) dl_lds[lane] = dl;
     if (lane == 0 && add_loss) {
         float term = valid ? k * (m + __logf(s) - zy) : 0.f;
         if (wtot == 0.f && clip == 0) term = __builtin_nanf("");
diff --git a/egot2_amd/csrc/fused_host.h b/egot2_amd/csrc/fused_host.h
--- a/egot2_amd/csrc/fused_host.h
+++ b/egot2_amd/csrc/fused_host.h
@@ -57,10 +57,11 @@
 int check_ce(const egx_ce* ce, bool with_head, const char* entry);
 int fused_path_fwd(const egx_config* cfg, const egx_segment* segs, const Plan& pl, bool tiled, const float* ln_w, const float* ln_b,
                    const egx_layer* layers, const egx_head* head, float* tokens_out, float* logits_out, void* saved, int training,
-                   uint64_t seed, hipStream_t st);
+                   uint64_t seed, hipStream_t st, void* round_scratch = nullptr);
+bool fused_round_ok(const egx_config* cfg, const Plan& pl, const egx_head* head, int training);
 int fused_path_bwd(const egx_config* cfg, const egx_segment* segs, const Plan& pl, bool tiled, const float* ln_w, const float* ln_b,
                    const egx_layer* layers, const egx_head* head, float* d_tokens, const float* d_logits, const void* saved, void* scratch,
                    const egx_segment_grads* seg_grads, float* d_ln_w, float* d_ln_b, const egx_layer_grads* layer_grads,
-                   const egx_head_grads* head_grads, int training, uint64_t seed, hipStream_t st);
+                   const egx_head_grads* head_grads, int training, uint64_t seed, hipStream_t st, bool ffn_round_done = false);
 
 }
diff --git a/egot2_amd/csrc/fused_host.hip b/egot2_amd/csrc/fused_host.hip
--- a/egot2_amd/csrc/fused_host.hip
+++ b/egot2_amd/csrc/fused_host.hip
@@ -262,6 +262,11 @@
     const int ns = fused_slices(pl, cfg->compute);
     return ns == 1 && !use_cut(pl, ns, false, cfg->compute);
 }
+bool fused_round_ok(const egx_config* cfg, const Plan& pl, const egx_head* head, int training) {
+    if (!tuning().ffn_round || !training || !(head && head->W) || !cfg->ce || cfg->deterministic || cfg->token_ce || cfg->bwd_stage != 0) return false;
+    const int ns = fused_slices(pl, cfg->compute);
+    return ns == 1 && use_cut(pl, ns, false, cfg->compute);
+}
 size_t fused_weight_cache_bytes(const egx_config* cfg, const egx_segment* segs, const Plan& pl) {
     if (pl.d != 128 || pl.nseg > FUSED_MAX_SEG || pl.L > FUSED_MAX_LAYERS || pl.L < 1 || pl.dff % 128 != 0) return 0;
     for (int i = 0; i < pl.nseg; ++i)
@@ -542,11 +547,12 @@
 
 int fused_path_fwd(const egx_config* cfg, const egx_segment* segs, const Plan& pl, bool tiled, const float* ln_w, const float* ln_b,
                    const egx_layer* layers, const egx_head* head, float* tokens_out, float* logits_out, void* saved, int training,
-                   uint64_t seed, hipStream_t st) {
+                   uint64_t seed, hipStream_t st, void* round_scratch) {
     const int d = pl.d, S = pl.S, B = pl.B, comp = cfg->compute;
     const bool with_head = head && head->W;
     const egx_ce* ce = cfg->ce;
     const egx_token_ce* tce = cfg->token_ce;
+    EGX_CHECK(!round_scratch || (!tiled && fused_round_ok(cfg, pl, head, training)), "egx_translator_fwd_round: not on this configuration (egx_translator_round_ok)");
     Plan vp = pl;
     if (tiled) plan_tiled(vp);
     const TiledView v = uniform_view(cfg, segs, vp, saved, tiled);
@@ -607,7 +613,18 @@
             memset(&fp.touch, 0, sizeof(fp.touch));
             if (touch && l + 1 < pl.L) { touch_add(fp.touch, PL.layer[l + 1].in_w, in_pb); touch_add(fp.touch, PL.layer[l + 1].out_w, out_pb); }
             else if (touch && training) { touch_add(fp.touch, PL.layer[l].lin2_wt, ffn_pb); touch_add(fp.touch, PL.layer[l].lin1_wt, ffn_pb); }
-            if (ffn_cut_forward(fp, l, comp, st)) return 1;
+            if (round_scratch && l + 1 == pl.L) {
+                const FusedBwdScratch SC = fused_bwd_scratch(cfg, segs, vp, head->n_out);
+                FusedBwdParams bp;
+                if (fill_bwd(bp, PL, SC, v, cfg, segs, vp, ln_w, ln_b, layers, head, ce->d_logits, nullptr, round_scratch, training, seed)) return 1;
+                bp.out_T = S;
+                bp.zero_buf = nullptr; bp.zero_n = 0; bp.d_logits_scale = nullptr;
+                bp.cut = 1; bp.cut_layer = l; bp.dy1 = fptr(round_scratch, SC.dy1); bp.dxin = fptr(round_scratch, SC.dxin);
+                if (touch) { touch_add(bp.touch, PL.layer[l].out_wt, out_pb); touch_add(bp.touch, PL.layer[l].in_wt, in_pb); }
+                if (timing_enabled()) {
+                    if (ffn_cut_forward(fp, l, comp, st) || ffn_cut_backward(bp, l, comp, st)) return 1;
+                } else if (ffn_cut_round(fp, bp, l, comp, st)) return 1;
+            } else if (ffn_cut_forward(fp, l, comp, st)) return 1;
         }
     } else {
         if (touch) {
@@ -623,9 +640,12 @@
 int fused_path_bwd(const egx_config* cfg, const egx_segment* segs, const Plan& pl, bool tiled, const float* ln_w, const float* ln_b,
                    const egx_layer* layers, const egx_head* head, float* d_tokens, const float* d_logits, const void* saved, void* scratch,
                    const egx_segment_grads* seg_grads, float* d_ln_w, float* d_ln_b, const egx_layer_grads* layer_grads,
-                   const egx_head_grads* head_grads, int training, uint64_t seed, hipStream_t st) {
+                   const egx_head_grads* head_grads, int training, uint64_t seed, hipStream_t st, bool ffn_round_done) {
     const int d = pl.d, S = pl.S, B = pl.B, comp = cfg->compute;
     const bool with_head = head && head->W;
+    EGX_CHECK(!ffn_round_done || (!tiled && with_head && training && !cfg->deterministic && !cfg->token_ce && cfg->bwd_stage == 0 && !cfg->d_logits_scale &&
+                                  fused_slices(pl, comp) == 1 && use_cut(pl, 1, false, comp)),
+              "egx_translator_bwd_round: not on this configuration (egx_translator_round_ok; upstream gradient 1: no d_logits_scale)");
     Plan vp = pl;
     if (tiled) plan_tiled(vp);
     const TiledView v = uniform_view(cfg, segs, vp, saved, tiled);
@@ -672,11 +692,15 @@
             bp.cut_layer = l;
             memset(&bp.touch, 0, sizeof(bp.touch));
             if (touch) { touch_add(bp.touch, PL.layer[l].out_wt, out_pb); touch_add(bp.touch, PL.layer[l].in_wt, in_pb); }
-            if (ffn_cut_backward(bp, l, comp, st)) return 1;
-            bp.zero_buf = nullptr;
+            const bool ffn_done = ffn_round_done && l + 1 == pl.L;
+            if (!ffn_done) {
+                if (ffn_cut_backward(bp, l, comp, st)) return 1;
+                bp.zero_buf = nullptr;
+            }
             memset(&bp.touch, 0, sizeof(bp.touch));
             if (touch && l > 0) { touch_add(bp.touch, PL.layer[l - 1].lin2_wt, ffn_pb); touch_add(bp.touch, PL.layer[l - 1].lin1_wt, ffn_pb); }
             if (fused_backward(bp, comp, st)) return 1;
+            bp.zero_buf = nullptr;
         }
     } else if (stage != 2) {
         if (touch) { touch_add(bp.touch, PL.layer[pl.L - 1].out_wt, out_pb); touch_add(bp.touch, PL.layer[pl.L - 1].in_wt, in_pb); }
diff --git a/egot2_amd/functional.py b/egot2_amd/functional.py
--- a/egot2_amd/functional.py
+++ b/egot2_amd/functional.py
@@ -464,11 +464,18 @@
             loss, ctx.ce_dl, keep = _ce_attach(spec, cfg, tail[0], tail[1], B, device)
         if spec.token_ce:
             keep, tce_out, ctx.tce_dl, tw, tb = _token_ce_attach(lib, spec, cfg, segs, tail, wc is not None and not py_slice, B, S, device)
+        ctx.round_scratch = None
         if nhead:
             head = _head(head_t, spec.head_n_out)
             tokens = torch.empty((B, spec.head_n_out), dtype=torch.float32, device=device)
-            check(lib.egx_translator_fwd(C.byref(cfg), segs, ptr(ln_w), ptr(ln_b), layers, C.byref(head), B, ptr(tokens),
-                                         None, ptr(saved), ptr(scratch), int(spec.training), seed, _stream()))
+            fwd = lib.egx_translator_fwd
+            if (spec.ce and any(nig) and not spec.defer_small and hasattr(lib, "egx_translator_round_ok")
+                    and lib.egx_translator_round_ok(C.byref(cfg), segs, C.byref(head), B, int(spec.training))):
+                fwd = lib.egx_translator_fwd_round
+                scratch = ctx.round_scratch = _saved_buffer(True, "scratch", device, sc.value)
+                ctx.wc, ctx.wc_sig = wc, wc_sig
+            check(fwd(C.byref(cfg), segs, ptr(ln_w), ptr(ln_b), layers, C.byref(head), B, ptr(tokens),
+                      None, ptr(saved), ptr(scratch), int(spec.training), seed, _stream()))
         else:
             tokens = torch.empty((B, spec.out_tokens or S, d), dtype=torch.float32, device=device)
             check(lib.egx_encoder_fwd(C.byref(cfg), segs, ptr(ln_w), ptr(ln_b), layers, B, ptr(tokens), ptr(saved),
@@ -557,7 +564,16 @@
             cfg.bucket_cb = C.cast(cb_keep, C.c_void_p)
         defer = bool(spec.defer_small) and ctx.impl == EGX_IMPL_FUSED
         cfg.bwd_stage = 1 if defer else 0
-        scratch = _workspace("scratch", device, ctx.scratch_bytes)
+        round_scratch, ctx.round_scratch = ctx.round_scratch, None
+        unit = _UNIT_GRAD.get(device.index)
+        round_done = (round_scratch is not None and d_tokens is ctx.ce_dl and dl_scale is not None and unit is not None
+                      and dl_scale.data_ptr() == unit.data_ptr())
+        if round_scratch is not None and ctx.wc is not None and ctx.wc.sig is not None and ctx.wc.sig != ctx.wc_sig:
+            raise _lib.EgxError("the packed-weight cache was re-packed between this forward and its backward (another forward of the module "
+                                "with other weights, mode or dropout); run the backward first, or give that forward no weight cache")
+        if round_done:
+            cfg.d_logits_scale = None
+        scratch = round_scratch if round_scratch is not None else _workspace("scratch", device, ctx.scratch_bytes)
         seed = _seed64(spec.seed)
         saved_buf = ctx.saved_buf
         p_lnw, p_lnb, flat_buf = ptr(gr.first[2]), ptr(gr.first[3]), pk.flat
@@ -565,10 +581,12 @@
             head, hg = _head(head_t, spec.head_n_out), gr.head_grads()
             dtok = _f32c(d_tokens)
 
+            bwd = lib.egx_translator_bwd_round if round_done else lib.egx_translator_bwd
+
             def launch(c):
-                check(lib.egx_translator_bwd(C.byref(c), segs, ptr(ln_w), ptr(ln_b), layers, C.byref(head), B, ptr(dtok),
-                                             ptr(saved_buf), ptr(scratch), sgr, p_lnw, p_lnb, lgr,
-                                             C.byref(hg), int(spec.training), seed, _stream()))
+                check(bwd(C.byref(c), segs, ptr(ln_w), ptr(ln_b), layers, C.byref(head), B, ptr(dtok),
+                          ptr(saved_buf), ptr(scratch), sgr, p_lnw, p_lnb, lgr,
+                          C.byref(hg), int(spec.training), seed, _stream()))
         else:
             if spec.token_ce:
                 dtok = None
diff --git a/include/egot2x.h b/include/egot2x.h
--- a/include/egot2x.h
+++ b/include/egot2x.h
@@ -304,6 +304,15 @@
                              int slot_bytes, int slot0, int method, int capacity, void* state, void* stream);
 int egx_view_ensemble_topk(int n, int capacity, int H, const int* C, const int* ks, int n_ks, void* state, int* rank, int* pred, void* result,
                            void* stream);
+int egx_translator_round_ok(const egx_config* cfg, const egx_segment* segs, const egx_head* head, int B, int training);
+int egx_translator_fwd_round(const egx_config* cfg, const egx_segment* segs, const float* ln_w, const float* ln_b,
+                             const egx_layer* layers, const egx_head* head, int B, float* logits_out, float* tokens_out,
+                             void* saved, void* scratch, int training, uint64_t seed, void* stream);
+int egx_translator_bwd_round(const egx_config* cfg, const egx_segment* segs, const float* ln_w, const float* ln_b,
+                             const egx_layer* layers, const egx_head* head, int B, const float* d_logits, const void* saved,
+                             void* scratch, const egx_segment_grads* seg_grads, float* d_ln_w, float* d_ln_b,
+                             const egx_layer_grads* layer_grads, const egx_head_grads* head_grads, int training,
+                             uint64_t seed, void* stream);
 int egx_small_attention_fwd(const float* q, int ldq, const float* k, int ldk, const float* v, int ldv, float* o, int ldo,
                             int B, int Sq, int Sk, int H, int dh, int causal, float p_drop, uint64_t seed, uint32_t site,
                             void* stream);
```
